# ODD2/DFD-CLIP

Hardware: AMD Instinct MI355X
Metric: 1-sec clips/sec (30x224x224 frames) ViT-B/16 (higher is better)
Workload: dtype bf16

## Files before the change

dfd-clip_amd/blocked.py:

```python
import torch

GROUP_ROWS = 16
TILE_CHANNELS = 64


def padded_rows(m):
    return (int(m) + GROUP_ROWS - 1) // GROUP_ROWS * GROUP_ROWS


def piece_offset(row, channel, ld):
    g, er = divmod(int(row), GROUP_ROWS)
    kt, c = divmod(int(channel), TILE_CHANNELS)
    chunk, e = divmod(c, 8)
    s, eq = chunk & 1, chunk >> 1
    return g * GROUP_ROWS * ld + kt * 1024 + s * 512 + er * 32 + eq * 8 + e


def pack(x, fill=0):
    m, c = x.shape
    assert c % TILE_CHANNELS == 0, "the blocked layout needs whole 64-channel K tiles"
    mp = padded_rows(m)
    xp = torch.full((mp, c), fill, dtype=x.dtype, device=x.device)
    xp[:m] = x
    v = xp.view(mp // GROUP_ROWS, GROUP_ROWS, c // TILE_CHANNELS, 4, 2, 8)
    return v.permute(0, 2, 4, 1, 3, 5).reshape(mp, c).contiguous()


def unpack(b, m=None):
    mp, c = b.shape
    assert mp % GROUP_ROWS == 0 and c % TILE_CHANNELS == 0 and b.is_contiguous()
    v = b.view(mp // GROUP_ROWS, c // TILE_CHANNELS, 2, GROUP_ROWS, 4, 8)
    x = v.permute(0, 3, 1, 4, 2, 5).reshape(mp, c)
    return x[:mp if m is None else m].contiguous()


def fc_channel_perm(n, device=None):
    assert n % TILE_CHANNELS == 0
    c = torch.arange(n, device=device)
    return (c & ~60) | ((c & 12) << 2) | ((c & 48) >> 2)


def lane_channels(eq):
    perm = fc_channel_perm(TILE_CHANNELS)
    return [[int(perm[16 * j + 4 * eq + e]) for e in range(4)] for j in range(4)]
```

dfd-clip_amd/capi.py:

```python
import ctypes
import os
from ctypes import POINTER, Structure, c_char_p, c_double, c_float, c_int, c_int32, c_int64, c_size_t, c_uint, c_uint8, c_uint32, c_uint64, c_void_p

import torch

PKG_DIR = os.path.dirname(os.path.abspath(__file__))
LIB_PATH = os.path.join(PKG_DIR, "libdfdclip_hip.so")

F32, BF16 = 0, 1
EPI_BIAS, EPI_BIAS_QUICKGELU, EPI_BIAS_RESIDUAL, EPI_PATCH_EMBED, EPI_QKV_EXPORT, EPI_RESIDUAL_POS, EPI_BIAS_GELU = range(7)
ABI_VERSION = 17

_DTYPE = {torch.float32: F32, torch.bfloat16: BF16}
FP8 = 2
FP8_MAX = 448.0
FP8_MIN_ROWS = 1024


class DfdError(RuntimeError):
    pass


GEMM_STREAM_OUT = 1
GEMM_SPARE_IF_FREE = 2
GEMM_C_BLOCKED = 4
GEMM_A_BLOCKED = 8


class GemmExtra(Structure):
    _fields_ = [("pos", c_void_p), ("cls", c_void_p), ("k_export", c_void_p), ("v_export", c_void_p),
                ("tokens", c_int32), ("frames_per_clip", c_int32), ("residual", c_void_p), ("qkv_first", c_int32),
                ("drop_rng", c_void_p), ("drop_site", c_uint32), ("drop_p", c_float), ("flags", c_uint32)]


OPTIM_SGD, OPTIM_ADAMW = 0, 1


class OptimExtra(Structure):
    _fields_ = [("kind", c_int32), ("reserved", c_int32), ("beta1", c_double), ("beta2", c_double), ("eps", c_double),
                ("step", c_int64), ("exp_avg_sq", c_void_p)]


class DropoutDesc(Structure):
    _fields_ = [("rng_state", c_void_p), ("site", c_uint32), ("p", c_float)]


class Dropout:
    __slots__ = ("rng", "site", "p")

    def __init__(self, rng, site, p):
        assert rng.is_cuda and rng.dtype == torch.int64 and rng.numel() == 2 and 0.0 <= p < 1.0
        self.rng, self.site, self.p = rng, int(site), float(p)

    def desc(self):
        return DropoutDesc(self.rng.data_ptr(), self.site, self.p)


def _drop(d):
    return ctypes.byref(d.desc()) if d is not None and d.p > 0 else None


SIGNATURES = {
    "dfd_last_error": (c_char_p, []),
    "dfd_abi_version": (c_int, []),
    "dfd_gemm_last_path": (c_int, []),
    "dfd_gemm_set_variant": (c_int, [c_int]),
    "dfd_dropout": (c_int, [c_void_p, c_int, c_void_p, c_int, c_int64, POINTER(DropoutDesc), c_void_p]),
    "dfd_device_check": (c_int, []),
    "dfd_layernorm": (c_int, [c_void_p, c_int64, c_void_p, c_void_p, c_void_p, c_int64, c_int, c_int64, c_int, c_float, c_float, c_void_p]),
    "dfd_layernorm2": (c_int, [c_void_p, c_int64, c_void_p, c_void_p, c_void_p, c_void_p, c_void_p, c_int64, c_int, c_int64, c_int, c_float,
                               c_float, c_void_p]),
    "dfd_add_layernorm": (c_int, [c_void_p, c_int64, c_void_p, c_void_p, c_int64, c_int, c_int, c_void_p, c_void_p, c_void_p, c_int64,
                                  c_int, c_int64, c_int, c_float, c_float, c_void_p]),
    "dfd_patchify": (c_int, [c_void_p, c_void_p, c_int, c_int, c_int, c_int, c_int, c_void_p]),
    "dfd_preprocess_u8": (c_int, [c_void_p, c_int, c_int, c_int, c_int, c_int, c_int, POINTER(c_float), POINTER(c_float),
                                  c_void_p, c_int, c_int, c_int, c_void_p]),
    "dfd_preprocess_geometry": (c_int, [c_int, c_int, c_int, POINTER(c_int), POINTER(c_int), POINTER(c_int), POINTER(c_int)]),
    "dfd_gemm": (c_int, [c_void_p, c_int64, c_void_p, c_int64, c_int, c_void_p, c_int64, c_int, c_void_p, c_int,
                         POINTER(GemmExtra), c_int64, c_int, c_int, c_void_p]),
# ... 123 lines not shown

SWIGLU_SIGNATURES = {
    "dfd_swiglu_fwd": (c_int, [c_void_p, c_int64, c_void_p, c_int64, c_int, c_int64, c_int, c_void_p]),
    "dfd_swiglu_last_path": (c_int, []),
}

KVGATHER_VEC16, KVGATHER_ELEMENT = 1, 2

KVGATHER_SIGNATURES = {
    "dfd_kv_gather_patches": (c_int, [c_void_p, c_void_p, c_int, c_int64, c_int64, c_int64, c_void_p, c_void_p, c_void_p, c_void_p, c_int,
                                      c_int64, c_int, c_int, c_int, c_int, c_void_p]),
    "dfd_kv_gather_last_path": (c_int, []),
}

KVFRAMES_VEC16, KVFRAMES_ELEMENT = 1, 2
KVFRAMES_SRC_ONCE = 1

KVFRAMES_SIGNATURES = {
    "dfd_kv_move_frames": (c_int, [c_void_p, c_void_p, c_void_p, c_void_p, c_int, c_int64, c_int64, c_int64, c_int64, c_int64, c_int64,
                                   c_void_p, c_void_p, c_int, c_int64, c_int, c_int, c_int, c_int, c_int, c_void_p]),
    "dfd_kv_move_last_path": (c_int, []),
}

EMA_SIGNATURES = {
    "dfd_ema_step": (c_int, [c_void_p, c_int, c_int64, c_float, c_float, c_void_p]),
}

class AttentionPlan(Structure):
    _fields_ = [("path", c_int32), ("grid", c_uint32), ("block", c_uint32), ("chunk", c_int32), ("lds", c_uint64)]


class GemmPlan(Structure):
    _fields_ = [("kernel", c_int32), ("epilogue", c_int32), ("tile_rows", c_int32), ("tiles_m", c_int32), ("ntiles", c_int64),
                ("grid", c_uint32), ("grid_y", c_uint32), ("block", c_uint32), ("c_blocked", c_int32), ("a_blocked", c_int32),
                ("dynamic", c_int32)]


class AdapterPlan(Structure):
    _fields_ = [("path", c_int32), ("grid", c_uint32), ("block", c_uint32), ("slabs", c_int32), ("groups_per_slab", c_int32)]


HOOK_SIGNATURES = {
    "dfd_adapter_norm_gelu_last_path": (c_int, []),
    "dfd_adapter_norm_gelu_plan": (c_int, [c_int, c_int, c_int, c_int, c_int, c_int, c_int, c_int, POINTER(AdapterPlan)]),
    "dfd_gemm_last_kernel": (c_int, []),
    "dfd_gemm_plan": (c_int, [c_int, c_int, c_int, c_int64, c_int, c_int, c_int64, c_int64, c_int64, c_uint32, c_int, c_int, c_int, c_uint,
                              c_uint, c_int, POINTER(GemmPlan)]),
    "dfd_attention_set_variant": (c_int, [c_int]),
    "dfd_attention_last_path": (c_int, []),
    "dfd_attention_plan": (c_int, [c_int, c_int, c_int, c_int, c_int64, c_int64, c_int, POINTER(AttentionPlan)]),
    "dfd_gemm_pair_set_variant": (c_int, [c_int]),
    "dfd_gemm_pair_plan": (c_int, [c_int64, c_int, c_int]),
    "dfd_gemm_pair_launches": (c_int64, []),
    "dfd_gemm_at_b_last_path": (c_int, []),
    "dfd_stream_policy_set": (c_uint, [c_uint]),
    "dfd_stream_policy_get": (c_uint, []),
}

(ATTN_ROWS, ATTN_ROWS_CHUNKED, ATTN_ITEM7, ATTN_ITEM9, ATTN_PERSIST7_SHORT, ATTN_PERSIST7, ATTN_XROW,
 ATTN_STREAM) = range(1, 9)

ADP_ROW256, ADP_JOINT_REG, ADP_JOINT, ADP_ROW = range(1, 5)

GEMM_GENERAL, GEMM_TILE, GEMM_PERSISTENT, GEMM_PINGPONG = range(1, 5)
(GEMM_PTR_A, GEMM_PTR_W, GEMM_PTR_C, GEMM_PTR_BIAS, GEMM_PTR_POS, GEMM_PTR_CLS, GEMM_PTR_RESIDUAL, GEMM_PTR_COL_SCALE,
 GEMM_PTR_EXPORT) = (1 << i for i in range(9))

STREAM_DECODER_KV, STREAM_DECODER_WEIGHTS, STREAM_OPTIMIZER, STREAM_ENCODER_ROWS, STREAM_ALL = 1, 2, 4, 8, 15
STREAM_DEFAULT = STREAM_DECODER_KV | STREAM_ENCODER_ROWS

_lib = None


def load_library(path=None):
    global _lib
    if _lib is not None and path is None:
        return _lib
    path = path or LIB_PATH
    if not os.path.exists(path):
        raise DfdError(f"{path} not found: the HIP kernel library is not built and there is no fallback path")
    lib = ctypes.CDLL(path)
    for name, (res, args) in {**SIGNATURES, **EXT_SIGNATURES, **EXPLAIN_SIGNATURES, **AUGMENT_SIGNATURES, **ALIGN_SIGNATURES,
                               **ELASTIC_SIGNATURES, **YUV_SIGNATURES, **SWIGLU_SIGNATURES, **KVGATHER_SIGNATURES,
                               **KVFRAMES_SIGNATURES, **EMA_SIGNATURES, **HOOK_SIGNATURES}.items():
        try:
            fn = getattr(lib, name)
        except AttributeError:
            raise DfdError(f"{path} does not export {name}")
        fn.restype = res
        fn.argtypes = args
    if lib.dfd_abi_version() != ABI_VERSION:
        raise DfdError(f"{path}: ABI version {lib.dfd_abi_version()} != {ABI_VERSION}")
    _lib = lib
    return lib


def _check(rc, what):
    if rc != 0:
        raise DfdError(f"{what} failed ({rc}): {load_library().dfd_last_error().decode()}")


def _stream():
    return c_void_p(torch._C._cuda_getCurrentRawStream(torch._C._cuda_getDevice()))


def _ptr(t):
# ... 251 lines not shown

def kv_move_frames(k, v, k_out, v_out, src_frame=None, dst_frame=None, src_once=False, src_host=None, dst_host=None):
    _dev(k, v, k_out, v_out, src_frame, dst_frame)
    assert k.dtype == v.dtype == k_out.dtype == v_out.dtype and k.dtype in _DTYPE, (k.dtype, v.dtype, k_out.dtype, v_out.dtype)
    assert k.dim() == 4 and k.shape == v.shape and k.stride() == v.stride(), "k and v are two views of one layout"
    assert k_out.dim() == 4 and k_out.shape == v_out.shape and k_out.stride() == v_out.stride(), "k_out and v_out are two views of one layout"
    L, src_frames, P, D = k.shape
    assert (k_out.shape[0], k_out.shape[2], k_out.shape[3]) == (L, P, D), (k.shape, k_out.shape)
    dst_frames = k_out.shape[1]
    assert (k.stride(3) == 1 and k_out.stride(3) == 1) or D <= 1, "rows are dense: unit column stride"
    n_src, _ = _frame_table("src_frame", src_frame, src_host, src_frames)
    n_dst, host = _frame_table("dst_frame", dst_frame, dst_host, dst_frames)
    if n_src is not None and n_dst is not None:
        assert n_src == n_dst, (n_src, n_dst)
    n = n_src if n_src is not None else n_dst
    if n is None:
        assert src_frames == dst_frames, "without a table both sides hold the same frames"
        n = src_frames
    if (src_frame is None and n > src_frames) or (dst_frame is None and n > dst_frames):
        raise DfdError(f"kv_move_frames: {n} frames under an identity table exceed that side (src {src_frames}, dst {dst_frames})")
    if host is not None and len(set(host.tolist())) != host.numel():
        raise DfdError("kv_move_frames: dst_frame names a frame twice: two moves into one frame would race")
    if L == 0 or n == 0 or P == 0 or D == 0:
        return k_out, v_out
    _check(load_library().dfd_kv_move_frames(_ptr(k), _ptr(v), _ptr(k_out), _ptr(v_out), _DTYPE[k.dtype], k.stride(0), k.stride(1),
                                             max(k.stride(2), D), k_out.stride(0), k_out.stride(1), max(k_out.stride(2), D),
                                             _ptr(src_frame), _ptr(dst_frame), L, n, src_frames, dst_frames, P, D,
                                             KVFRAMES_SRC_ONCE if src_once else 0, _stream()), "dfd_kv_move_frames")
    return k_out, v_out


def kv_move_last_path():
    return load_library().dfd_kv_move_last_path()


def profile_gemm(epilogue=None):
    _profile["epilogue"] = epilogue
    _profile["events"] = []
    _profile["base"] = None
    if epilogue is not None:
        _profile["base"] = torch.cuda.Event(enable_timing=True)
        _profile["base"].record()


def profile_gemm_collect():
    base = _profile["base"]
    spans = [(base.elapsed_time(a), base.elapsed_time(b), flops) for a, b, flops in _profile["events"]]
    profile_gemm(None)
    return spans


def gemm(a, w, c, bias=None, epilogue=EPI_BIAS, m=None, pos=None, cls=None, k_export=None, v_export=None, tokens=0,
         frames_per_clip=0, residual=None, qkv_first=0, drop=None, stream_out=False, spare_cus=0, tile_blocks=0, spare_if_free=False,
         c_blocked=False, a_blocked=False):
    _dev(a, w, c, bias, pos, cls, k_export, v_export, residual)
    assert a.dtype == w.dtype and a.stride(1) == 1 and w.stride(1) == 1 and c.stride(1) == 1
    M = a.shape[0] if m is None else m
    N, K = w.shape
    assert a.shape[1] == K
    assert residual is None or (residual.dtype == c.dtype and residual.stride(0) == c.stride(0))
    assert drop is None or epilogue == EPI_RESIDUAL_POS
    assert 0 <= epilogue <= EPI_BIAS_GELU, f"unknown epilogue {epilogue}"
    if c_blocked or a_blocked:
        blk = c if c_blocked else a
        assert blk.shape[0] >= (M + 15) // 16 * 16, "a blocked matrix needs its rows rounded up to 16"
    extra = GemmExtra(_ptr(pos).value, _ptr(cls).value, _ptr(k_export).value, _ptr(v_export).value, tokens, frames_per_clip,
                      _ptr(residual).value, qkv_first, drop.rng.data_ptr() if drop is not None and drop.p > 0 else None,
                      drop.site if drop is not None else 0, drop.p if drop is not None else 0.0, (GEMM_STREAM_OUT if stream_out else 0) | (GEMM_SPARE_IF_FREE if spare_if_free else 0) | ((int(spare_cus) & 0xff) << 8) | ((int(tile_blocks) & 0xf) << 16)
                      | (GEMM_C_BLOCKED if c_blocked else 0) | (GEMM_A_BLOCKED if a_blocked else 0))
    timed = _profile["epilogue"] == epilogue
    if timed:
        e0, e1 = torch.cuda.Event(enable_timing=True), torch.cuda.Event(enable_timing=True)
        e0.record()
    _check(load_library().dfd_gemm(_ptr(a), a.stride(0), _ptr(w), w.stride(0), _DTYPE[a.dtype], _ptr(c), c.stride(0),
                                   _DTYPE[c.dtype], _ptr(bias), epilogue, ctypes.byref(extra), M, N, K, _stream()), "dfd_gemm")
    if timed:
        e1.record()
        _profile["events"].append((e0, e1, 2.0 * M * N * K))
    return c


def gemm_fp8(a, w, c, col_scale, bias=None, epilogue=EPI_BIAS, m=None, out_inv_scale=0.0, pos=None, k_export=None, v_export=None,
             tokens=0, frames_per_clip=0, qkv_first=0, stream_out=False, spare_cus=0, spare_if_free=False):
    _dev(a, w, c, col_scale, bias, pos, k_export, v_export)
    assert a.element_size() == 1 and w.element_size() == 1 and a.stride(1) == 1 and w.stride(1) == 1 and c.stride(1) == 1
    assert col_scale.dtype == torch.float32 and col_scale.is_contiguous()
    M = a.shape[0] if m is None else m
    N, K = w.shape
    assert a.shape[1] == K and col_scale.numel() == N
    c_dtype = FP8 if c.element_size() == 1 else _DTYPE[c.dtype]
    extra = GemmExtra(_ptr(pos).value, None, _ptr(k_export).value, _ptr(v_export).value, tokens, frames_per_clip, None, qkv_first,
                      None, 0, 0.0, (GEMM_STREAM_OUT if stream_out else 0) | (GEMM_SPARE_IF_FREE if spare_if_free else 0) | ((int(spare_cus) & 0xff) << 8))
    timed = _profile["epilogue"] == epilogue
    if timed:
        e0, e1 = torch.cuda.Event(enable_timing=True), torch.cuda.Event(enable_timing=True)
        e0.record()
    _check(load_library().dfd_gemm_fp8(_ptr(a), a.stride(0), _ptr(w), w.stride(0), _ptr(c), c.stride(0), c_dtype, _ptr(col_scale),
                                       _ptr(bias), float(out_inv_scale), epilogue, ctypes.byref(extra), M, N, K, _stream()),
           "dfd_gemm_fp8")
    if timed:
        e1.record()
        _profile["events"].append((e0, e1, 2.0 * M * N * K))
    return c


def gemm_set_variant(variant):
    return load_library().dfd_gemm_set_variant(int(variant))


def gemm_pair_set_variant(variant):
    return load_library().dfd_gemm_pair_set_variant(int(variant))


def gemm_pair_plan(M, D, H):
    return bool(load_library().dfd_gemm_pair_plan(int(M), int(D), int(H)))


def gemm_pair_launches():
    return load_library().dfd_gemm_pair_launches()


def stream_policy_set(mask):
    return load_library().dfd_stream_policy_set(int(mask))


def stream_policy_get():
    return load_library().dfd_stream_policy_get()


def gemm_last_path():
    return load_library().dfd_gemm_last_path()


def gemm_last_kernel():
    return load_library().dfd_gemm_last_kernel()


def gemm_plan(ab_dtype, c_dtype, epilogue, M, N, K, lda=None, ldw=None, ldc=None, flags=0, tokens=0, frames_per_clip=0, qkv_first=0,
              has=0, misaligned=0, n_cu=256):
    out = GemmPlan()
    rc = load_library().dfd_gemm_plan(ab_dtype, c_dtype, epilogue, M, N, K, K if lda is None else lda, K if ldw is None else ldw,
                                      N if ldc is None else ldc, flags, tokens, frames_per_clip, qkv_first, has, misaligned, n_cu,
                                      ctypes.byref(out))
    if rc < 0:
        raise DfdError(f"dfd_gemm_plan failed ({rc}): {load_library().dfd_last_error().decode()}")
    return out


def gemm_at_b_workspace_bytes(R, Ma, Nb, dtype):
    return load_library().dfd_gemm_at_b_workspace(R, Ma, Nb, _DTYPE[dtype])


def gemm_at_b_last_path():
    return load_library().dfd_gemm_at_b_last_path()


def gemm_at_b(a, b, c, workspace):
    _dev(a, b, c, workspace)
    assert a.dtype == b.dtype and a.stride(1) == 1 and b.stride(1) == 1 and c.is_contiguous() and c.dtype == torch.float32
    R, Ma = a.shape
    Nb = b.shape[1]
    assert b.shape[0] == R and tuple(c.shape) == (Ma, Nb)
    assert workspace.numel() * workspace.element_size() >= gemm_at_b_workspace_bytes(R, Ma, Nb, a.dtype)
    _check(load_library().dfd_gemm_at_b(_ptr(a), a.stride(0), _ptr(b), b.stride(0), _DTYPE[a.dtype], _ptr(c), R, Ma, Nb,
                                        _ptr(workspace), _stream()), "dfd_gemm_at_b")
    return c


def adapter_norm_gelu(a, y, weight, bias, frames, patches, x, joint, eps=1e-5):
    _dev(a, y, weight, bias)
    assert (a.dtype == y.dtype or a.dtype == torch.float32) and a.is_contiguous() and y.is_contiguous()
    assert weight.is_contiguous() and bias.is_contiguous()
    _check(load_library().dfd_adapter_norm_gelu(_ptr(a), _DTYPE[a.dtype], _ptr(y), _DTYPE[y.dtype], _ptr(weight), _ptr(bias), frames,
                                                patches, x, int(joint), eps, _stream()), "dfd_adapter_norm_gelu")
    return y


def adapter_norm_gelu_bwd_workspace_bytes(frames, patches, x, joint):
    return load_library().dfd_adapter_norm_gelu_bwd_workspace(frames, patches, x, int(joint))


def adapter_norm_gelu_bwd(a, dy, da, weight, bias, dweight, dbias, workspace, frames, patches, x, joint, eps=1e-5):
    _dev(a, dy, da, weight, bias, dweight, dbias, workspace)
    assert dy.dtype == da.dtype and (a.dtype == dy.dtype or a.dtype == torch.float32)
    assert a.is_contiguous() and dy.is_contiguous() and da.is_contiguous()
    _check(load_library().dfd_adapter_norm_gelu_bwd(_ptr(a), _DTYPE[a.dtype], _ptr(dy), _ptr(da), _DTYPE[dy.dtype], _ptr(weight), _ptr(bias),
                                                    _ptr(dweight), _ptr(dbias), _ptr(workspace), frames, patches, x, int(joint),
                                                    eps, _stream()), "dfd_adapter_norm_gelu_bwd")
    return da


def attention_set_variant(variant):
    return load_library().dfd_attention_set_variant(int(variant))


def attention_last_path():
    return load_library().dfd_attention_last_path()


def attention_plan(dtype, n_frames, tokens, heads, ld_qkv=None, ld_out=None, n_cu=256):
    D = heads * 64
    plan = AttentionPlan()
    rc = load_library().dfd_attention_plan(_DTYPE[dtype], n_frames, tokens, heads, 3 * D if ld_qkv is None else ld_qkv,
                                           D if ld_out is None else ld_out, n_cu, ctypes.byref(plan))
    if rc < 0:
        raise DfdError(f"dfd_attention_plan failed ({rc}): {load_library().dfd_last_error().decode()}")
    return plan


def attention_fwd(qkv, out, n_frames, tokens, heads, head_dim=64):
    _dev(qkv, out)
    assert qkv.dtype == out.dtype and qkv.stride(1) == 1 and out.stride(1) == 1
    _check(load_library().dfd_attention_fwd(_ptr(qkv), qkv.stride(0), _ptr(out), out.stride(0), _DTYPE[qkv.dtype], n_frames,
                                            tokens, heads, head_dim, head_dim ** -0.5, _stream()), "dfd_attention_fwd")
    return out


def linear_rows(x, w, bias, y, epilogue=EPI_BIAS):
    _dev(x, w, bias, y)
    assert x.dtype == torch.float32 and w.dtype == torch.float32 and y.dtype == torch.float32
    assert x.stride(1) == 1 and y.stride(1) == 1 and w.is_contiguous()
    B, K = x.shape
    N = w.shape[0]
    _check(load_library().dfd_linear_rows(_ptr(x), x.stride(0), _ptr(w), _ptr(bias), _ptr(y), y.stride(0), epilogue, B, N, K,
                                          _stream()), "dfd_linear_rows")
    return y


def linear_rows_t_workspace_bytes(B, N, K):
    return load_library().dfd_linear_rows_t_workspace(B, N, K)


def linear_rows_t(x, wt, bias, y, workspace, epilogue=EPI_BIAS, residual=None):
    _dev(x, wt, bias, y, workspace, residual)
    assert residual is None or (residual.dtype == torch.float32 and residual.stride(1) == 1 and residual.shape == y.shape)
    assert x.dtype == torch.float32 and wt.dtype == torch.float32 and y.dtype == torch.float32
    assert x.stride(1) == 1 and y.stride(1) == 1 and wt.is_contiguous()
    B, K = x.shape
    N = wt.shape[1]
    assert wt.shape[0] == K and workspace.numel() * workspace.element_size() >= linear_rows_t_workspace_bytes(B, N, K)
    _check(load_library().dfd_linear_rows_t(_ptr(x), x.stride(0), _ptr(wt), _ptr(bias), _ptr(residual),
                                            residual.stride(0) if residual is not None else 0, _ptr(y), y.stride(0), epilogue, B, N, K,
                                            _ptr(workspace), _stream()), "dfd_linear_rows_t")
    return y


def decoder_attn_workspace_bytes(B, heads, d, splits):
    return load_library().dfd_decoder_attn_workspace(B, heads, d, splits)


class KvLayoutDesc(ctypes.Structure):
    _fields_ = [("row_stride", c_int64), ("frame_stride", c_int64), ("pos", c_void_p)]


def _kv_layout(x, other, pos, B, T, patches, D):
    if other is not None:
        assert other.dtype == x.dtype and other.shape == x.shape and other.stride() == x.stride()
    if x.is_contiguous() and pos is None:
        assert x.numel() == B * T * patches * D
        return None, None
    if x.is_contiguous():
        rs, fs = D, patches * D
    else:
        assert x.dim() == 3 and x.shape == (B * T, patches, D) and x.stride(2) == 1, "strided K/V must be [B*T, patches, D] views"
        fs, rs = x.stride(0), x.stride(1)
    if pos is not None:
# ... 308 lines not shown
```

dfd-clip_amd/csrc/attention.hip:

```cpp
#include "attention_common.hpp"

namespace {

template <typename T> struct Vec16;
template <> struct Vec16<float> { using type = f32x4; static constexpr int N = 4; };
template <> struct Vec16<bf16_t> { using type = bf16x8; static constexpr int N = 8; };

template <typename T>
__device__ __forceinline__ void attn_row_key(const float (&q)[HD], float (&acc)[HD], float& mx, float& l, const T* Kp, const T* Vp) {
  using V16 = typename Vec16<T>::type;
  constexpr int VN = Vec16<T>::N;
  constexpr int CHUNKS = HD / VN;
  float s0 = 0.f, s1 = 0.f;
#pragma unroll
  for (int ch = 0; ch < CHUNKS; ++ch) {
    const V16 kv = *reinterpret_cast<const V16*>(Kp + ch * VN);
#pragma unroll
    for (int e = 0; e < VN; e += 2) {
      s0 = fmaf(q[ch * VN + e], to_f32(kv[e]), s0);
      s1 = fmaf(q[ch * VN + e + 1], to_f32(kv[e + 1]), s1);
    }
  }
  const float s = s0 + s1;
  if (s > mx) {
// ... 77 lines not shown
  for (int qbase = 0; qbase < tokens; qbase += blockDim.x) {
    const int qi = qbase + threadIdx.x;
    const bool live = qi < tokens;
    float q[HD], acc[HD];
    const T* qp = base + (int64_t)(live ? qi : tokens - 1) * ld_qkv;
#pragma unroll
    for (int ch = 0; ch < CHUNKS; ++ch) {
      const V16 v = *reinterpret_cast<const V16*>(qp + ch * VN);
#pragma unroll
      for (int e = 0; e < VN; ++e) q[ch * VN + e] = to_f32(v[e]) * scale;
    }
#pragma unroll
    for (int c = 0; c < HD; ++c) acc[c] = 0.f;
    float mx = -INFINITY, l = 0.f;
    for (int k0 = 0; k0 < tokens; k0 += chunk) {
      const int nk = min(chunk, tokens - k0);
      __syncthreads();
      for (int c = threadIdx.x; c < nk * CHUNKS; c += blockDim.x) {
        const int row = c / CHUNKS, ch = c % CHUNKS;
        const T* src = base + (int64_t)(k0 + row) * ld_qkv + ch * VN;
        *reinterpret_cast<V16*>(Ks + row * HD + ch * VN) = *reinterpret_cast<const V16*>(src + D);
        *reinterpret_cast<V16*>(Vs + row * HD + ch * VN) = *reinterpret_cast<const V16*>(src + 2 * D);
      }
      __syncthreads();
      if (live)
        for (int j = 0; j < nk; ++j) attn_row_key<T>(q, acc, mx, l, Ks + j * HD, Vs + j * HD);
    }
    if (live) {
      const float inv = 1.0f / l;
      T* op = out + ((int64_t)frame * tokens + qi) * ld_out + head * HD;
#pragma unroll
      for (int ch = 0; ch < CHUNKS; ++ch) {
        V16 o;
#pragma unroll
        for (int e = 0; e < VN; ++e) o[e] = from_f32<T>(acc[ch * VN + e] * inv);
        *reinterpret_cast<V16*>(op + ch * VN) = o;
      }
    }
  }
}

template <typename T>
int launch_rows(const AttnPlan& p, const AttnCall& c) {
  const T* qkv = static_cast<const T*>(c.qkv);
  T* out = static_cast<T*>(c.out);
  if (p.path == ATTN_ROWS_CHUNKED)
    return attn_launch<&attn_rows_chunked_kernel<T>>("dfd_attention_fwd", p, c.st, qkv, c.ld_qkv, out, c.ld_out, c.tokens, c.heads, c.scale, p.chunk);
  return attn_launch<&attn_rows_kernel<T>>("dfd_attention_fwd", p, c.st, qkv, c.ld_qkv, out, c.ld_out, c.tokens, c.heads, c.scale);
}

thread_local int g_attn_variant = 0;
thread_local int g_attn_last_path = 0;

int checked_plan(AttnPlan* p, int dtype, int n_frames, int tokens, int heads, int64_t ld_qkv, int64_t ld_out, int n_cu) {
  DFD_REQUIRE(n_frames >= 0 && tokens > 0 && heads > 0, "dfd_attention_fwd: bad shape");
  DFD_REQUIRE(dtype == DFD_F32 || dtype == DFD_BF16, "dfd_attention_fwd: dtype=%d", dtype);
  const int esz = dtype == DFD_F32 ? 4 : 2;
  DFD_REQUIRE(ld_qkv >= 3 * heads * HD && ld_out >= heads * HD && (ld_qkv * esz) % 16 == 0 && (ld_out * esz) % 16 == 0,
              "dfd_attention_fwd: bad leading dimensions");
  *p = attn_plan(dtype, n_frames, tokens, heads, ld_qkv, ld_out, g_attn_variant, n_cu > 0 ? n_cu : dfd_cu_count());
  DFD_REQUIRE(p->path != ATTN_NONE, "dfd_attention_fwd: %lld (frame, head) items do not fit a grid", (long long)n_frames * heads);
  return DFD_OK;
}

}

extern "C" int dfd_attention_set_variant(int variant) {
  const int old = g_attn_variant;
  g_attn_variant = variant;
  return old;
}

extern "C" int dfd_attention_last_path(void) { return g_attn_last_path; }

extern "C" int dfd_attention_plan(int dtype, int n_frames, int tokens, int heads, int64_t ld_qkv, int64_t ld_out, int n_cu,
                                  dfd_attention_plan_t* out) {
  AttnPlan p;
  if (checked_plan(&p, dtype, n_frames, tokens, heads, ld_qkv, ld_out, n_cu) != DFD_OK) return -1;
  if (out) *out = dfd_attention_plan_t{p.path, p.grid, p.block, p.chunk, (uint64_t)p.lds};
  return p.path;
}

extern "C" int dfd_attention_fwd(const void* qkv, int64_t ld_qkv, void* out, int64_t ld_out, int dtype, int n_frames,
                                 int tokens, int heads, int head_dim, float scale, void* stream) {
  DFD_REQUIRE(qkv && out, "dfd_attention_fwd: null pointer");
  DFD_REQUIRE(head_dim == HD, "dfd_attention_fwd: head_dim=%d, only 64 is supported", head_dim);
  AttnPlan p;
  if (int rc = checked_plan(&p, dtype, n_frames, tokens, heads, ld_qkv, ld_out, 0)) return rc;
  DFD_REQUIRE(dfd_aligned16(qkv) && dfd_aligned16(out), "dfd_attention_fwd: pointers must be 16-byte aligned");
  if (n_frames == 0) return DFD_OK;
  const AttnCall c{qkv, ld_qkv, out, ld_out, n_frames, tokens, heads, scale, static_cast<hipStream_t>(stream)};
  int rc;
  switch (p.path) {
    case ATTN_ROWS:
    case ATTN_ROWS_CHUNKED: rc = dtype == DFD_F32 ? launch_rows<float>(p, c) : launch_rows<bf16_t>(p, c); break;
    case ATTN_XROW: rc = dfd_attn_launch_xrow(p, c); break;
    case ATTN_STREAM: rc = dfd_attn_launch_stream(p, c); break;
    default: rc = dfd_attn_launch_mfma(p, c); break;
  }
  if (rc == DFD_OK) g_attn_last_path = p.path;
  return rc;
}
```

dfd-clip_amd/csrc/attention_common.hpp:

```cpp
#pragma once
#include "common.hpp"
#include "../../include/dfdclip_hooks.h"

namespace {

constexpr int HD = 64;

typedef float f32x2v __attribute__((ext_vector_type(2)));
typedef __attribute__((address_space(3))) void* lds_ptr_t;
typedef short short4v __attribute__((ext_vector_type(4)));
typedef int v4i_t __attribute__((ext_vector_type(4)));

__device__ __forceinline__ float vmax3(float a, float b, float c) {
  float r;
  asm("v_max3_f32 %0, %1, %2, %3" : "=v"(r) : "v"(a), "v"(b), "v"(c));
  return r;
}

__device__ __forceinline__ void attn_stage_k(__amdgpu_buffer_rsrc_t srd, unsigned char* kimg, uint32_t sbase, uint32_t ldq,
                                             uint32_t Db, int lane, int np, int tokens, int p0 = 0, int dp = 1) {
  const int sub = lane >> 3, pos = lane & 7;
  const uint32_t row0 = (uint32_t)sub * ldq;
  const uint32_t k_even = row0 + Db + ((pos ^ ((sub >> 1) & 3)) << 4), k_odd = row0 + Db + ((pos ^ (((sub >> 1) & 3) | 4)) << 4);
  for (int p = p0; p < np; p += dp) {
    if (8 * p + sub < tokens)
      __builtin_amdgcn_raw_ptr_buffer_load_lds(srd, (lds_ptr_t)(kimg + p * 1024), 16, ((p & 1) ? k_odd : k_even) + p * 8 * ldq, sbase, 0, 0);
  }
}
__device__ __forceinline__ void attn_stage_v(__amdgpu_buffer_rsrc_t srd, unsigned char* vimg, uint32_t sbase, uint32_t ldq,
                                             uint32_t Db, int lane, int np, int tokens, int p0 = 0, int dp = 1) {
  const int sub = lane >> 3, pos = lane & 7;
  const uint32_t v_any = (uint32_t)sub * ldq + 2 * Db + ((pos ^ (((sub >> 1) & 1) << 2)) << 4);
  for (int p = p0; p < np; p += dp) {
    if (8 * p + sub < tokens)
      __builtin_amdgcn_raw_ptr_buffer_load_lds(srd, (lds_ptr_t)(vimg + p * 1024), 16, v_any + p * 8 * ldq, sbase, 0, 0);
  }
}

struct AttnNoTick {
  __device__ __forceinline__ void operator()(int) const {}
};
template <int NB, bool SHORT, typename Tick = AttnNoTick>
__device__ __forceinline__ float attn_softmax(f32x16 (&S)[NB], int tokens, int h, float scale_log2e, Tick tick = Tick()) {
  constexpr int LE = SHORT ? 4 : 16;
#pragma unroll
  for (int e = 0; e < LE; ++e) {
    const int key = (NB - 1) * 32 + (e & 3) + 8 * (e >> 2) + 4 * h;
    if (key >= tokens) S[NB - 1][e] = -INFINITY;
  }
  float mx = -INFINITY;
#pragma unroll
  for (int kb = 0; kb < NB; ++kb)
#pragma unroll
    for (int e = 0; e < (kb == NB - 1 ? LE : 16); e += 2) mx = vmax3(mx, S[kb][e], S[kb][e + 1]);
  mx = fmaxf(mx, __shfl_xor(mx, 32, 64));
  float sl2 = scale_log2e;
  float nmc = -mx * scale_log2e;
  asm volatile("" : "+s"(sl2));
  f32x16 lv;
#pragma unroll
  for (int e = 0; e < 16; ++e) lv[e] = 0.f;
#pragma unroll
  for (int kb = 0; kb < NB; ++kb) {
#pragma unroll
    for (int e = 0; e < (kb == NB - 1 ? LE : 16); e += 2) {
      const f32x2v t = __builtin_elementwise_fma(f32x2v{S[kb][e], S[kb][e + 1]}, f32x2v{sl2, sl2}, f32x2v{nmc, nmc});
      S[kb][e] = __builtin_amdgcn_exp2f(t[0]);
      S[kb][e + 1] = __builtin_amdgcn_exp2f(t[1]);
    }
    if (SHORT && kb == NB - 1) {
#pragma unroll
      for (int e = 0; e < 4; ++e) lv[e] += S[kb][e];
#pragma unroll
      for (int e = 4; e < 8; ++e) S[kb][e] = 0.f;
    } else {
      lv += S[kb];
    }
    tick(kb);
  }
  float l = ((lv[0] + lv[1]) + (lv[2] + lv[3])) + ((lv[4] + lv[5]) + (lv[6] + lv[7])) +
            (((lv[8] + lv[9]) + (lv[10] + lv[11])) + ((lv[12] + lv[13]) + (lv[14] + lv[15])));
  l += __shfl_xor(l, 32, 64);
  return l;
}

__device__ __forceinline__ void attn_read_v(bf16x8 (&vf)[2], const unsigned char* Vs, int lane, int step) {
  const int h = lane >> 5, tq = (lane & 15) >> 2, tp = lane & 3, rr = (lane >> 4) & 1;
  const int kbase = (step >> 1) * 32 + 16 * (step & 1) + 4 * h + tq;
// ... 15 lines not shown
struct AttnNoRider {
  __device__ __forceinline__ void operator()(const bf16x8 (&)[2], int) const {}
};
template <int NB, bool SHORT, typename Rider = AttnNoRider>
__device__ __forceinline__ void attn_pv(const f32x16 (&S)[NB], const unsigned char* Vs, int lane, f32x16 (&O)[2], Rider rider = Rider()) {
  const f32x16 zero16 = {0.f, 0.f, 0.f, 0.f, 0.f, 0.f, 0.f, 0.f, 0.f, 0.f, 0.f, 0.f, 0.f, 0.f, 0.f, 0.f};
  auto mma_v = [&](const bf16x8 (&vf)[2], int step) {
    const int kb = step >> 1, sl = step & 1;
    bf16x8 pf;
#pragma unroll
    for (int j = 0; j < 8; ++j) pf[j] = (bf16_t)S[kb][8 * sl + j];
#pragma unroll
    for (int dt = 0; dt < 2; ++dt) O[dt] = __builtin_amdgcn_mfma_f32_32x32x16_bf16(vf[dt], pf, step == 0 ? zero16 : O[dt], 0, 0, 0);
  };
  bf16x8 vfa[2], vfb[2];
  attn_read_v(vfa, Vs, lane, 0);
  __builtin_amdgcn_sched_barrier(0);
  constexpr int NS = SHORT ? 2 * NB - 1 : 2 * NB;
#pragma unroll
  for (int step = 0; step < NS; step += 2) {
    if (step + 1 < NS) attn_read_v(vfb, Vs, lane, step + 1);
    mma_v(vfa, step);
    rider(vfa, step);
    __builtin_amdgcn_sched_barrier(0);
    if (step + 2 < NS) attn_read_v(vfa, Vs, lane, step + 2);
    if (step + 1 < NS) {
      mma_v(vfb, step + 1);
      rider(vfb, step + 1);
    }
    __builtin_amdgcn_sched_barrier(0);
  }
}

__device__ __forceinline__ void attn_store_line(v4i_t d, __amdgpu_buffer_rsrc_t srd, uint32_t off) {
  __builtin_amdgcn_raw_buffer_store_b128(d, srd, off, 0, 0);
}

template <int N> __device__ __forceinline__ void attn_wait_vm() { asm volatile("s_waitcnt vmcnt(%0)" ::"n"(N) : "memory"); }

}

enum AttnPath {
  ATTN_NONE = 0, ATTN_ROWS = DFD_ATTN_ROWS, ATTN_ROWS_CHUNKED = DFD_ATTN_ROWS_CHUNKED, ATTN_ITEM7 = DFD_ATTN_ITEM7,
  ATTN_ITEM9 = DFD_ATTN_ITEM9, ATTN_PERSIST7_SHORT = DFD_ATTN_PERSIST7_SHORT, ATTN_PERSIST7 = DFD_ATTN_PERSIST7,
  ATTN_XROW = DFD_ATTN_XROW, ATTN_STREAM = DFD_ATTN_STREAM
};

struct AttnPlan {
  int path;
  unsigned grid, block;
  size_t lds;
  int chunk;
  uint32_t qkv_bytes, out_bytes;
};

constexpr size_t ATTN_LDS_MAX = 160 * 1024;
constexpr size_t attn_item_lds(int nb) { return (size_t)nb * 32 * 128 + 64 * ((size_t)nb * 64 + 8); }
constexpr size_t attn_persist_lds(int tokens, int nb) { return (size_t)4 * tokens * 128 + (size_t)2 * nb * 4096; }
constexpr size_t ATTN_XROW_LDS = 4 * 257 * 128 + 8 * 2048 + 2560;
constexpr int ATTN_STREAM_SPAN = 128;

inline AttnPlan attn_plan(int dtype, int n_frames, int tokens, int heads, int64_t ld_qkv, int64_t ld_out, int variant, int n_cu) {
  const int64_t items = (int64_t)n_frames * heads, GRID_MAX = 0x7fffffff, EXTENT_MAX = 0xfffffff0;
  const size_t esz = dtype == DFD_F32 ? 4 : 2;
  auto per_item = [&](int path, size_t lds, int chunk) {
    return AttnPlan{items <= GRID_MAX ? path : ATTN_NONE, (unsigned)items, 256u, lds, chunk, 0u, 0u};
  };
  const int nb = (tokens + 31) / 32;
  if (dtype == DFD_BF16 && (nb == 7 || nb == 9)) {
    const int64_t last_row = (int64_t)n_frames * tokens - 1;
    const int64_t qkv_bytes = last_row * ld_qkv * 2 + (int64_t)3 * heads * 128, out_bytes = last_row * ld_out * 2 + (int64_t)heads * 128;
    const unsigned grid = (unsigned)(n_cu <= 0 ? 256 : n_cu) & ~7u;
    const size_t lds = nb == 7 ? attn_persist_lds(tokens, 7) : ATTN_XROW_LDS;
    if (items >= 512 && grid >= 8 && qkv_bytes <= EXTENT_MAX && out_bytes <= EXTENT_MAX && (nb == 7 ? lds <= ATTN_LDS_MAX : tokens == 257))
      return AttnPlan{nb == 9 ? ATTN_XROW : tokens <= 6 * 32 + 8 ? ATTN_PERSIST7_SHORT : ATTN_PERSIST7, grid, 512u, lds, 0,
                      (uint32_t)qkv_bytes, (uint32_t)out_bytes};
    return per_item(nb == 7 ? ATTN_ITEM7 : ATTN_ITEM9, attn_item_lds(nb), 0);
  }
  const int64_t spans = (tokens + ATTN_STREAM_SPAN - 1) / ATTN_STREAM_SPAN;
  if (dtype == DFD_BF16 && tokens > 32 && variant != 2 && items <= GRID_MAX / spans)
    return AttnPlan{ATTN_STREAM, (unsigned)(items * spans), 256u, 0, 0, 0u, 0u};
  const size_t whole = 2 * (size_t)tokens * 64 * esz;
  const int chunk = variant == 1 ? 16 : whole > ATTN_LDS_MAX ? (int)(64 * 1024 / (2 * 64 * esz)) : 0;
  return chunk > 0 ? per_item(ATTN_ROWS_CHUNKED, 2 * (size_t)chunk * 64 * esz, chunk) : per_item(ATTN_ROWS, whole, 0);
}

template <auto Kernel, typename... A>
int attn_launch(const char* what, const AttnPlan& p, hipStream_t st, A... args) {
  static bool raised = false;
  if (p.lds > 64 * 1024 && !raised) {
    (void)hipFuncSetAttribute(reinterpret_cast<const void*>(Kernel), hipFuncAttributeMaxDynamicSharedMemorySize, (int)ATTN_LDS_MAX);
    raised = true;
  }
  hipLaunchKernelGGL(Kernel, dim3(p.grid), dim3(p.block), p.lds, st, args...);
  DFD_CHECK_LAUNCH(what);
  return DFD_OK;
}

struct AttnCall {
  const void* qkv;
  int64_t ld_qkv;
  void* out;
  int64_t ld_out;
  int n_frames, tokens, heads;
  float scale;
  hipStream_t st;
};
int dfd_attn_launch_mfma(const AttnPlan& p, const AttnCall& c);
int dfd_attn_launch_xrow(const AttnPlan& p, const AttnCall& c);
int dfd_attn_launch_stream(const AttnPlan& p, const AttnCall& c);
```

dfd-clip_amd/csrc/attention_mfma.hip:

```cpp
#include "attention_common.hpp"

namespace {

template <int NB> struct Lds {
  static constexpr int KEYS = NB * 32;
  static constexpr int VSTRIDE = KEYS * 2 + 8;
  static constexpr int K_BYTES = KEYS * 128;
  static constexpr int BYTES = K_BYTES + HD * VSTRIDE;
};

template <int NB>
__global__ __launch_bounds__(256, 2) void attn_mfma_kernel(const bf16_t* __restrict__ qkv, int64_t ld_qkv,
                                                           bf16_t* __restrict__ out, int64_t ld_out, int tokens,
                                                           int heads, float scale_log2e) {
  using L = Lds<NB>;
  extern __shared__ __attribute__((aligned(16))) unsigned char smem[];
  unsigned char* Ks = smem;
  unsigned char* Vt = smem + L::K_BYTES;
  const int tid = threadIdx.x, lane = tid & 63, wave = tid >> 6;
  const int r = lane & 31, h = lane >> 5;
  const int frame = blockIdx.x / heads, head = blockIdx.x % heads;
  const int D = heads * HD;
  const bf16_t* base = qkv + (int64_t)frame * tokens * ld_qkv + head * HD;

// ... 105 lines not shown
        const unsigned char* vp = Vt + (dt * 32 + r) * L::VSTRIDE + (kb * 32 + 16 * sl + 4 * h) * 2;
        const bf16x4 v0 = *reinterpret_cast<const bf16x4*>(vp);
        const bf16x4 v1 = *reinterpret_cast<const bf16x4*>(vp + 16);
        vf[dt] = bf16x8{v0[0], v0[1], v0[2], v0[3], v1[0], v1[1], v1[2], v1[3]};
      }
    };
    auto mma_v = [&](const bf16x8 (&vf)[2], int step) {
      const int kb = step >> 1, sl = step & 1;
      bf16x8 pf;
#pragma unroll
      for (int j = 0; j < 8; ++j) pf[j] = (bf16_t)S[kb][8 * sl + j];
#pragma unroll
      for (int dt = 0; dt < 2; ++dt) O[dt] = __builtin_amdgcn_mfma_f32_32x32x16_bf16(vf[dt], pf, O[dt], 0, 0, 0);
    };
    bf16x8 vfa[2], vfb[2];
    read_v(vfa, 0);
    __builtin_amdgcn_sched_barrier(0);
#pragma unroll
    for (int step = 0; step < 2 * NB; step += 2) {
      read_v(vfb, step + 1);
      mma_v(vfa, step);
      __builtin_amdgcn_sched_barrier(0);
      if (step + 2 < 2 * NB) read_v(vfa, step + 2);
      mma_v(vfb, step + 1);
      __builtin_amdgcn_sched_barrier(0);
    }
    if (q < tokens) {
      const float inv = 1.0f / l;
      bf16_t* op = out + ((int64_t)frame * tokens + q) * ld_out + head * HD;
#pragma unroll
      for (int dt = 0; dt < 2; ++dt)
#pragma unroll
        for (int g = 0; g < 4; ++g) {
          bf16x4 o;
#pragma unroll
          for (int e = 0; e < 4; ++e) o[e] = (bf16_t)(O[dt][4 * g + e] * inv);
          *reinterpret_cast<bf16x4*>(op + dt * 32 + 8 * g + 4 * h) = o;
        }
    }
#pragma unroll
    for (int s = 0; s < 4; ++s) qf[s] = qn[s];
  }
}

template <int NB>
__device__ __forceinline__ void attn_stage_q(__amdgpu_buffer_rsrc_t srd, unsigned char* qimg, uint32_t sbase, uint32_t ldq, int lane,
                                             int tokens) {
  const int sub = lane >> 3, pos = lane & 7;
  const uint32_t q_even = (pos ^ ((sub >> 1) & 3)) << 4, q_odd = (pos ^ (((sub >> 1) & 3) | 4)) << 4;
#pragma unroll
  for (int p = 0; p < 4 * NB; ++p) {
    const uint32_t row = (uint32_t)min(8 * p + sub, tokens - 1);
    __builtin_amdgcn_raw_ptr_buffer_load_lds(srd, (lds_ptr_t)(qimg + p * 1024), 16, row * ldq + ((p & 1) ? q_odd : q_even), sbase, 0, 0);
  }
}

__device__ __forceinline__ void wait_vm_dyn(int n) {
  switch (n < 0 ? 0 : n) {
    case 0: asm volatile("s_waitcnt vmcnt(0)" ::: "memory"); break;
    case 1: asm volatile("s_waitcnt vmcnt(1)" ::: "memory"); break;
    case 2: asm volatile("s_waitcnt vmcnt(2)" ::: "memory"); break;
    case 3: asm volatile("s_waitcnt vmcnt(3)" ::: "memory"); break;
    case 4: asm volatile("s_waitcnt vmcnt(4)" ::: "memory"); break;
    case 5: asm volatile("s_waitcnt vmcnt(5)" ::: "memory"); break;
    case 6: asm volatile("s_waitcnt vmcnt(6)" ::: "memory"); break;
    case 7: asm volatile("s_waitcnt vmcnt(7)" ::: "memory"); break;
    case 8: asm volatile("s_waitcnt vmcnt(8)" ::: "memory"); break;
    case 9: asm volatile("s_waitcnt vmcnt(9)" ::: "memory"); break;
    case 10: asm volatile("s_waitcnt vmcnt(10)" ::: "memory"); break;
    case 11: asm volatile("s_waitcnt vmcnt(11)" ::: "memory"); break;
    case 12: asm volatile("s_waitcnt vmcnt(12)" ::: "memory"); break;
    case 13: asm volatile("s_waitcnt vmcnt(13)" ::: "memory"); break;
    case 14: asm volatile("s_waitcnt vmcnt(14)" ::: "memory"); break;
    case 15: asm volatile("s_waitcnt vmcnt(15)" ::: "memory"); break;
    case 16: asm volatile("s_waitcnt vmcnt(16)" ::: "memory"); break;
    case 17: asm volatile("s_waitcnt vmcnt(17)" ::: "memory"); break;
    case 18: asm volatile("s_waitcnt vmcnt(18)" ::: "memory"); break;
    case 19: asm volatile("s_waitcnt vmcnt(19)" ::: "memory"); break;
    case 20: asm volatile("s_waitcnt vmcnt(20)" ::: "memory"); break;
    case 21: asm volatile("s_waitcnt vmcnt(21)" ::: "memory"); break;
    case 22: asm volatile("s_waitcnt vmcnt(22)" ::: "memory"); break;
    case 23: asm volatile("s_waitcnt vmcnt(23)" ::: "memory"); break;
    case 24: asm volatile("s_waitcnt vmcnt(24)" ::: "memory"); break;
    case 25: asm volatile("s_waitcnt vmcnt(25)" ::: "memory"); break;
    case 26: asm volatile("s_waitcnt vmcnt(26)" ::: "memory"); break;
    case 27: asm volatile("s_waitcnt vmcnt(27)" ::: "memory"); break;
    case 28: asm volatile("s_waitcnt vmcnt(28)" ::: "memory"); break;
    case 29: asm volatile("s_waitcnt vmcnt(29)" ::: "memory"); break;
    case 30: asm volatile("s_waitcnt vmcnt(30)" ::: "memory"); break;
    case 31: asm volatile("s_waitcnt vmcnt(31)" ::: "memory"); break;
    case 32: asm volatile("s_waitcnt vmcnt(32)" ::: "memory"); break;
    case 33: asm volatile("s_waitcnt vmcnt(33)" ::: "memory"); break;
    case 34: asm volatile("s_waitcnt vmcnt(34)" ::: "memory"); break;
    case 35: asm volatile("s_waitcnt vmcnt(35)" ::: "memory"); break;
    case 36: asm volatile("s_waitcnt vmcnt(36)" ::: "memory"); break;
    case 37: asm volatile("s_waitcnt vmcnt(37)" ::: "memory"); break;
    case 38: asm volatile("s_waitcnt vmcnt(38)" ::: "memory"); break;
    case 39: asm volatile("s_waitcnt vmcnt(39)" ::: "memory"); break;
    case 40: asm volatile("s_waitcnt vmcnt(40)" ::: "memory"); break;
    case 41: asm volatile("s_waitcnt vmcnt(41)" ::: "memory"); break;
    case 42: asm volatile("s_waitcnt vmcnt(42)" ::: "memory"); break;
    case 43: asm volatile("s_waitcnt vmcnt(43)" ::: "memory"); break;
    case 44: asm volatile("s_waitcnt vmcnt(44)" ::: "memory"); break;
    case 45: asm volatile("s_waitcnt vmcnt(45)" ::: "memory"); break;
    case 46: asm volatile("s_waitcnt vmcnt(46)" ::: "memory"); break;
    case 47: asm volatile("s_waitcnt vmcnt(47)" ::: "memory"); break;
    case 48: asm volatile("s_waitcnt vmcnt(48)" ::: "memory"); break;
    case 49: asm volatile("s_waitcnt vmcnt(49)" ::: "memory"); break;
    case 50: asm volatile("s_waitcnt vmcnt(50)" ::: "memory"); break;
    case 51: asm volatile("s_waitcnt vmcnt(51)" ::: "memory"); break;
    case 52: asm volatile("s_waitcnt vmcnt(52)" ::: "memory"); break;
    case 53: asm volatile("s_waitcnt vmcnt(53)" ::: "memory"); break;
    case 54: asm volatile("s_waitcnt vmcnt(54)" ::: "memory"); break;
    case 55: asm volatile("s_waitcnt vmcnt(55)" ::: "memory"); break;
    case 56: asm volatile("s_waitcnt vmcnt(56)" ::: "memory"); break;
    default: asm volatile("s_waitcnt vmcnt(56)" ::: "memory"); break;
  }
}

template <int NB, bool SHORT>
__global__ __launch_bounds__(512) void attn_mfma_persist_kernel(const bf16_t* __restrict__ qkv, uint32_t ldq ,
                                                                bf16_t* __restrict__ out, uint32_t ldo ,
                                                                int tokens, int heads, int n_frames, uint32_t qkv_bytes,
                                                                uint32_t out_bytes, float scale_log2e) {
  constexpr int QIMG = 32 * 128;
  extern __shared__ __attribute__((aligned(16))) unsigned char smem[];
  const int tid = threadIdx.x, wave = tid >> 6;
  int lane = tid & 63;
  asm volatile("" : "+v"(lane));
  const int r = lane & 31, h = lane >> 5;
  const uint32_t Db = (uint32_t)heads * HD * 2;
  const int ksw = (r >> 1) & 7;
  const int img = tokens * 128;
  const int np = (tokens * 8 + 63) >> 6;
  const __amdgpu_buffer_rsrc_t srdQ = __builtin_amdgcn_make_buffer_rsrc(const_cast<bf16_t*>(qkv), 0, (int)qkv_bytes, 0x00020000);
  const __amdgpu_buffer_rsrc_t srdO = __builtin_amdgcn_make_buffer_rsrc(out, 0, (int)out_bytes, 0x00020000);
  unsigned char* const qs0 = smem + 4 * img + (wave < NB ? wave : 0) * QIMG;

  for (int i = tid * 16; i < 4 * img + 2 * NB * QIMG; i += 512 * 16) *reinterpret_cast<v4i_t*>(smem + i) = v4i_t{0, 0, 0, 0};
  __syncthreads();

  const int qb = wave;
  const int xcd = blockIdx.x & 7, slot = blockIdx.x >> 3, per_xcd = gridDim.x >> 3;
  auto item_of = [&](int n, int& fr_, int& hd_) -> bool {
    const int li = n * per_xcd + slot;
    const int fl = li / heads;
    hd_ = li - fl * heads;
    fr_ = fl * 8 + xcd;
    return fr_ < n_frames;
  };
  auto barrier = [&]() { asm volatile("s_waitcnt lgkmcnt(0)\n\ts_barrier" ::: "memory"); };

  if (wave == NB) {
    int f1, h1, f2, h2;
    auto sbase_of = [&](int f, int hh) { return (uint32_t)f * tokens * ldq + hh * (HD * 2); };
    int issued = 0, mark_kq = 0, mark_v = 0;
    bool have = item_of(0, f1, h1);
    if (have) {
      attn_stage_k(srdQ, smem, sbase_of(f1, h1), ldq, Db, lane, np, tokens);
      attn_stage_q<NB>(srdQ, smem + 4 * img, sbase_of(f1, h1), ldq, lane, tokens);
      issued += np + 4 * NB;
      mark_kq = issued;
      if (item_of(1, f2, h2)) {
        attn_stage_k(srdQ, smem + 2 * img, sbase_of(f2, h2), ldq, Db, lane, np, tokens);
        issued += np;
      }
      attn_stage_v(srdQ, smem + img, sbase_of(f1, h1), ldq, Db, lane, np, tokens);
      issued += np;
      mark_v = issued;
    }
    for (int n = 0; have; ++n) {
      const int cur = n & 1;
      wait_vm_dyn(issued - mark_kq);
      barrier();
      const bool have1 = item_of(n + 1, f1, h1);
      if (have1) {
        attn_stage_q<NB>(srdQ, smem + 4 * img + (cur ^ 1) * NB * QIMG, sbase_of(f1, h1), ldq, lane, tokens);
        issued += 4 * NB;
        mark_kq = issued;
      }
      wait_vm_dyn(issued - mark_v);
      barrier();
      if (have1 && item_of(n + 2, f2, h2)) {
        attn_stage_k(srdQ, smem + cur * 2 * img, sbase_of(f2, h2), ldq, Db, lane, np, tokens);
        issued += np;
      }
      if (have1) {
        attn_stage_v(srdQ, smem + (cur ^ 1) * 2 * img + img, sbase_of(f1, h1), ldq, Db, lane, np, tokens);
        issued += np;
        mark_v = issued;
      }
      have = have1;
    }
    return;
  }
  if (wave > NB) return;

  int frame, head, nframe = 0, nhead = 0;
  bool have = item_of(0, frame, head);
  for (int n = 0; have; ++n) {
    const int cur = n & 1;
    const unsigned char* Ks = smem + cur * 2 * img;
    const unsigned char* Vs = Ks + img;
    unsigned char* Qs = qs0 + cur * NB * QIMG;
    barrier();
    const bool have_next = item_of(n + 1, nframe, nhead);
    {
    bf16x8 qf[4];
#pragma unroll
    for (int s = 0; s < 4; ++s) qf[s] = *reinterpret_cast<const bf16x8*>(Qs + r * 128 + (((2 * s + h) ^ ksw) << 4));

    f32x16 S[NB];
    const f32x16 zero16 = {0.f, 0.f, 0.f, 0.f, 0.f, 0.f, 0.f, 0.f, 0.f, 0.f, 0.f, 0.f, 0.f, 0.f, 0.f, 0.f};
    bf16x8 kfa[NB], kfb[NB];
    auto read_k = [&](bf16x8 (&kf)[NB], int s) {
#pragma unroll
      for (int kb = 0; kb < NB; ++kb)
        kf[kb] = *reinterpret_cast<const bf16x8*>(Ks + (kb * 32 + r) * 128 + (((2 * s + h) ^ ksw) << 4));
    };
    auto mma_k = [&](const bf16x8 (&kf)[NB], int s) {
#pragma unroll
      for (int kb = 0; kb < NB; ++kb)
        S[kb] = __builtin_amdgcn_mfma_f32_32x32x16_bf16(kf[kb], qf[s], s == 0 ? zero16 : S[kb], 0, 0, 0);
    };
    read_k(kfa, 0);
    __builtin_amdgcn_sched_barrier(0);
    read_k(kfb, 1);
    mma_k(kfa, 0);
    __builtin_amdgcn_sched_barrier(0);
    read_k(kfa, 2);
    mma_k(kfb, 1);
    __builtin_amdgcn_sched_barrier(0);
    read_k(kfb, 3);
    mma_k(kfa, 2);
    __builtin_amdgcn_sched_barrier(0);
    mma_k(kfb, 3);
    __builtin_amdgcn_sched_barrier(0);
    barrier();

    const float l = attn_softmax<NB, SHORT>(S, tokens, h, scale_log2e);
    f32x16 O[2];
    attn_pv<NB, SHORT>(S, Vs, lane, O);
    {
      const float inv = 1.0f / l;
#pragma unroll
      for (int dt = 0; dt < 2; ++dt)
#pragma unroll
        for (int g = 0; g < 4; ++g) {
          bf16x4 o;
#pragma unroll
          for (int e = 0; e < 4; ++e) o[e] = (bf16_t)(O[dt][4 * g + e] * inv);
          *reinterpret_cast<bf16x4*>(Qs + r * 128 + (((4 * dt + g) ^ ksw) << 4) + 8 * h) = o;
        }
      const uint32_t obase = (uint32_t)frame * tokens * ldo + head * (HD * 2);
#pragma unroll
      for (int i = 0; i < 4; ++i) {
        const int rl = 8 * i + (lane >> 3), pos = lane & 7;
        const v4i_t d = *reinterpret_cast<const v4i_t*>(Qs + rl * 128 + ((pos ^ ((rl >> 1) & 7)) << 4));
        const int qq = qb * 32 + rl;
        const uint32_t off = qq < tokens ? obase + (uint32_t)qq * ldo + pos * 16 : 0xffffffffu;
        attn_store_line(d, srdO, off);
      }
    }
    }
    have = have_next;
    frame = nframe;
    head = nhead;
  }
}

template <int NB>
int launch_item(const AttnPlan& p, const AttnCall& c) {
  static_assert(Lds<NB>::BYTES == attn_item_lds(NB), "the plan's LDS size is the kernel's layout");
  static_assert(Lds<NB>::VSTRIDE % 16 == 8, "Vt row stride must be 8 mod 16 bytes");
  return attn_launch<&attn_mfma_kernel<NB>>("dfd_attention_fwd(mfma)", p, c.st, static_cast<const bf16_t*>(c.qkv), c.ld_qkv,
                                            static_cast<bf16_t*>(c.out), c.ld_out, c.tokens, c.heads, c.scale * 1.4426950408889634f);
}

template <bool SHORT>
int launch_persist(const AttnPlan& p, const AttnCall& c) {
  return attn_launch<&attn_mfma_persist_kernel<7, SHORT>>("dfd_attention_fwd(mfma, persistent)", p, c.st, static_cast<const bf16_t*>(c.qkv),
                                                          (uint32_t)(c.ld_qkv * 2), static_cast<bf16_t*>(c.out), (uint32_t)(c.ld_out * 2),
                                                          c.tokens, c.heads, c.n_frames, p.qkv_bytes, p.out_bytes,
                                                          c.scale * 1.4426950408889634f);
}

}

int dfd_attn_launch_mfma(const AttnPlan& p, const AttnCall& c) {
  switch (p.path) {
    case ATTN_PERSIST7_SHORT: return launch_persist<true>(p, c);
    case ATTN_PERSIST7: return launch_persist<false>(p, c);
    case ATTN_ITEM7: return launch_item<7>(p, c);
    default: return launch_item<9>(p, c);
  }
}
```

dfd-clip_amd/csrc/gemm.hip:

```cpp
#include "gemm_plan.hpp"
#include "gelu.hpp"

namespace {

constexpr int BM = 128, BN = 128;
constexpr int ROW_BYTES = 64;
constexpr int ROW_STRIDE = 80;
constexpr int TILE_BYTES = BM * ROW_STRIDE;
constexpr int EPI_SPLITK_SLAB = 100;

template <typename CT> __device__ __forceinline__ void store_c(void* C, int64_t off, float v) {
  static_cast<CT*>(C)[off] = from_f32<CT>(v);
}

template <typename CT, int EPI>
__device__ __forceinline__ void epilogue_elem(const GemmArgs& a, int64_t m, int n, float acc) {
  if (m >= a.M || n >= a.N) return;
  if constexpr (EPI == DFD_EPI_BIAS) {
    store_c<CT>(a.C, m * a.ldc + n, acc + (a.bias ? a.bias[n] : 0.f));
  } else if constexpr (EPI == DFD_EPI_BIAS_QUICKGELU) {
    store_c<CT>(a.C, m * a.ldc + n, quick_gelu(acc + (a.bias ? a.bias[n] : 0.f)));
  } else if constexpr (EPI == DFD_EPI_BIAS_GELU) {
    store_c<CT>(a.C, m * a.ldc + n, gelu_erf(acc + (a.bias ? a.bias[n] : 0.f)));
  } else if constexpr (EPI == DFD_EPI_BIAS_RESIDUAL) {
// ... 188 lines not shown
  float s = 0.f;
  for (int z = 0; z < splits; ++z) s += slabs[(int64_t)z * n + i];
  out[i] = s;
}

void at_b_plan(int64_t R, int Ma, int Nb, int64_t* Rp, int* splits) {
  const int tiles = ((Ma + BM - 1) / BM) * ((Nb + BN - 1) / BN);
  int sp = (1024 + tiles - 1) / tiles;
  const int64_t steps = (R + 31) / 32;
  if (sp > steps / 8) sp = (int)(steps / 8 > 0 ? steps / 8 : 1);
  if (sp > 512) sp = 512;
  *splits = sp;
  *Rp = (R + 31) / 32 * 32;
}

template <typename T>
int launch_at_b(const void* A, int64_t lda, const void* B, int64_t ldb, float* C, int64_t R, int Ma, int Nb, void* workspace,
                hipStream_t st) {
  int64_t Rp;
  int splits;
  at_b_plan(R, Ma, Nb, &Rp, &splits);
  T* At = static_cast<T*>(workspace);
  T* Bt = At + (int64_t)Ma * Rp;
  size_t off = (size_t)(Ma + Nb) * Rp * sizeof(T);
  off = (off + 255) / 256 * 256;
  float* slabs = reinterpret_cast<float*>(static_cast<unsigned char*>(workspace) + off);
  const dim3 tb(256);
  hipLaunchKernelGGL((transpose_pad_kernel<T>), dim3((Ma + 31) / 32, (unsigned)(Rp / 32)), tb, 0, st, static_cast<const T*>(A), lda, At, R, Ma, Rp);
  hipLaunchKernelGGL((transpose_pad_kernel<T>), dim3((Nb + 31) / 32, (unsigned)(Rp / 32)), tb, 0, st, static_cast<const T*>(B), ldb, Bt, R, Nb, Rp);
  GemmArgs a{};
  a.A = At; a.W = Bt; a.C = slabs; a.lda = Rp; a.ldw = Rp; a.ldc = Nb; a.M = Ma; a.N = Nb; a.K = (int)Rp;
  const dim3 grid((Nb + BN - 1) / BN, (Ma + BM - 1) / BM, splits);
  hipLaunchKernelGGL((gemm128_kernel<T, float, EPI_SPLITK_SLAB>), grid, tb, 0, st, a);
  const int64_t n = (int64_t)Ma * Nb;
  hipLaunchKernelGGL(slab_reduce_kernel, dim3((unsigned)((n + 255) / 256)), tb, 0, st, slabs, C, n, splits);
  DFD_CHECK_LAUNCH("dfd_gemm_at_b");
  return DFD_OK;
}

}

static int fill_extra(GemmArgs& a, int epilogue, const dfd_gemm_extra* extra) {
  if (!extra) return DFD_OK;
  a.pos = extra->pos; a.cls = extra->cls; a.k_export = extra->k_export; a.v_export = extra->v_export;
  a.residual = epilogue == DFD_EPI_RESIDUAL_POS ? extra->residual : nullptr;
  a.tokens = extra->tokens; a.frames_per_clip = extra->frames_per_clip;
  a.qkv_first = epilogue == DFD_EPI_QKV_EXPORT ? extra->qkv_first : 0;
  a.stream_out = (extra->flags & DFD_GEMM_STREAM_OUT) ? 1 : 0;
  a.spare_cus = (int)((extra->flags >> DFD_GEMM_SPARE_CUS_SHIFT) & 0xff);
  a.spare_if_free = (extra->flags & DFD_GEMM_SPARE_IF_FREE) ? 1 : 0;
  a.tile_rows = 32 * (int)((extra->flags >> DFD_GEMM_TILE_BLOCKS_SHIFT) & 0xf);
  a.c_blocked = (extra->flags & DFD_GEMM_C_BLOCKED) ? 1 : 0;
  a.a_blocked = (extra->flags & DFD_GEMM_A_BLOCKED) ? 1 : 0;
  a.pair = a.c_blocked | a.a_blocked;
  DFD_REQUIRE(epilogue != DFD_EPI_QKV_EXPORT || !extra->k_export == !extra->v_export, "dfd_gemm: QKV_EXPORT needs both k_export and v_export or neither");
  if (epilogue == DFD_EPI_RESIDUAL_POS && extra->drop_rng && extra->drop_p > 0.f) {
    DFD_REQUIRE(extra->drop_p < 1.f, "dfd_gemm: drop_p=%f", (double)extra->drop_p);
    const dfd_dropout_t dd{extra->drop_rng, extra->drop_site, extra->drop_p};
    a.drop = dfd_make_drop(&dd);
  }
  return DFD_OK;
}

static thread_local int g_gemm_variant = 0;
static thread_local int g_pair_variant = 0;

static int checked_plan(GemmPlan* p, const char* who, GemmArgs& a, GemmPtrs ptrs, int ab_dtype, int c_dtype, int epilogue, int n_cu) {
  const bool f8 = ab_dtype == DFD_FP8;
  DFD_REQUIRE(a.M >= 0 && a.N > 0 && a.K > 0, "%s: bad shape M=%lld N=%d K=%d", who, (long long)a.M, a.N, a.K);
  if (f8) {
    DFD_REQUIRE(c_dtype == DFD_BF16 || c_dtype == DFD_FP8, "%s: c_dtype=%d", who, c_dtype);
    DFD_REQUIRE(epilogue == DFD_EPI_BIAS || epilogue == DFD_EPI_BIAS_QUICKGELU || epilogue == DFD_EPI_BIAS_GELU || epilogue == DFD_EPI_QKV_EXPORT,
                "%s: epilogue %d not served (BIAS, BIAS_QUICKGELU, BIAS_GELU, QKV_EXPORT)", who, epilogue);
    DFD_REQUIRE(c_dtype == DFD_BF16 || (epilogue != DFD_EPI_QKV_EXPORT && a.out_inv_scale > 0.f), "%s: fp8 output needs out_inv_scale > 0 and a plain / QuickGELU / GELU epilogue", who);
    DFD_REQUIRE(a.lda >= a.K && a.ldw >= a.K && a.ldc >= a.N, "%s: leading dimensions", who);
  } else {
    DFD_REQUIRE(ab_dtype == DFD_F32 || ab_dtype == DFD_BF16, "%s: ab_dtype=%d", who, ab_dtype);
    DFD_REQUIRE(c_dtype == DFD_F32 || c_dtype == DFD_BF16, "%s: c_dtype=%d", who, c_dtype);
    DFD_REQUIRE(!(ab_dtype == DFD_F32 && c_dtype == DFD_BF16), "%s: f32 operands with bf16 output unsupported", who);
    DFD_REQUIRE(a.K % 32 == 0, "%s: K=%d must be a multiple of 32", who, a.K);
    const int esz = ab_dtype == DFD_F32 ? 4 : 2;
    DFD_REQUIRE(a.lda >= a.K && a.ldw >= a.K && (a.lda * esz) % 16 == 0 && (a.ldw * esz) % 16 == 0, "%s: lda=%lld ldw=%lld must be >= K and 16-byte multiples", who,
                (long long)a.lda, (long long)a.ldw);
    DFD_REQUIRE(!(ptrs.misaligned & (DFD_GEMM_PTR_A | DFD_GEMM_PTR_W)), "%s: A and W must be 16-byte aligned", who);
  }
  const bool has_pos = ptrs.present & DFD_GEMM_PTR_POS;
  if (epilogue == DFD_EPI_PATCH_EMBED) {
    DFD_REQUIRE(has_pos && (ptrs.present & DFD_GEMM_PTR_CLS) && a.tokens > 1, "%s: PATCH_EMBED needs extra.pos, extra.cls, extra.tokens", who);
    DFD_REQUIRE(a.M % (a.tokens - 1) == 0, "%s: PATCH_EMBED M=%lld is not a whole number of frames", who, (long long)a.M);
    DFD_REQUIRE(c_dtype == DFD_F32 && a.ldc >= a.N, "%s: PATCH_EMBED writes an f32 token matrix", who);
  } else {
    DFD_REQUIRE(a.ldc >= a.N, "%s: ldc=%lld < N", who, (long long)a.ldc);
  }
  if (epilogue == DFD_EPI_QKV_EXPORT) {
    DFD_REQUIRE(a.tokens > 1 && (a.qkv_first == 0 || a.qkv_first == 1) && a.N % (3 - a.qkv_first) == 0,
                "%s: QKV_EXPORT needs extra.tokens, qkv_first in {0, 1} and N a multiple of the column blocks present", who);
    DFD_REQUIRE(a.M % a.tokens == 0, "%s: QKV_EXPORT M=%lld is not a whole number of frames", who, (long long)a.M);
    DFD_REQUIRE(!has_pos || a.frames_per_clip > 0, "%s: QKV_EXPORT with pos needs frames_per_clip", who);
  }
  if (epilogue == DFD_EPI_RESIDUAL_POS) {
    DFD_REQUIRE(a.tokens > 1, "%s: RESIDUAL_POS needs extra.tokens (patches per frame + 1)", who);
    DFD_REQUIRE(!has_pos || a.frames_per_clip > 0, "%s: RESIDUAL_POS with pos needs frames_per_clip", who);
  }
  DFD_REQUIRE(a.tile_rows == 0 || a.tile_rows == 224 || a.tile_rows == 256, "%s: tile blocks must be 0, 7 or 8", who);
  if (a.frames_per_clip < 1) a.frames_per_clip = 1;
  if (a.M == 0) {
    *p = GemmPlan{};
    return DFD_OK;
  }
  *p = gemm_plan(a, ptrs, ab_dtype, c_dtype, epilogue, g_gemm_variant, g_pair_variant, n_cu > 0 ? n_cu : dfd_cu_count());
  if (p->refused) {
    dfd_set_error("%s: %s%s (epilogue %d, M=%lld N=%d K=%d)", who,
                  a.pair ? "DFD_GEMM_C_BLOCKED / DFD_GEMM_A_BLOCKED: the ping-pong kernel does not serve this call: " : "call not served: ", p->refused,
                  epilogue, (long long)a.M, a.N, a.K);
    return DFD_ERR_INVALID_ARG;
  }
  if (p->tiles.grid == 0) {
    dfd_set_error("%s: cannot query the device", who);
    return DFD_ERR_LAUNCH;
  }
  return DFD_OK;
}

static thread_local int g_last_kernel = 0;
static thread_local int g_last_path = 0;
extern "C" int dfd_gemm_last_kernel(void) { return g_last_kernel; }
extern "C" int dfd_gemm_last_path(void) { return g_last_path; }
extern "C" int dfd_gemm_set_variant(int variant) {
  const int old = g_gemm_variant;
  g_gemm_variant = variant;
  return old;
}

static thread_local int64_t g_pair_launches = 0;
extern "C" int dfd_gemm_pair_set_variant(int variant) {
  const int old = g_pair_variant;
  g_pair_variant = variant;
  return old;
}
extern "C" int64_t dfd_gemm_pair_launches(void) { return g_pair_launches; }
extern "C" int dfd_gemm_pair_plan(int64_t M, int D, int H) {
  if (g_pair_variant == 1 || M < 1 || D < 1 || H < 1) return 0;
  if (M < 1024 && g_pair_variant != 2) return 0;
  GemmArgs fc{}, pr{};
  fc.M = pr.M = M; fc.pair = pr.pair = 1;
  fc.N = H; fc.K = D; fc.lda = D; fc.ldw = D; fc.ldc = H; fc.c_blocked = 1;
  pr.N = D; pr.K = H; pr.lda = H; pr.ldw = H; pr.ldc = D; pr.a_blocked = 1;
  const GemmPtrs dense{DFD_GEMM_PTR_A | DFD_GEMM_PTR_W | DFD_GEMM_PTR_C | DFD_GEMM_PTR_BIAS, 0u};
  auto blocked = [&](const GemmArgs& a, int epi) {
    return gemm_plan(a, dense, DFD_BF16, DFD_BF16, epi, g_gemm_variant, g_pair_variant, 256).kernel == DFD_GEMM_PINGPONG;
  };
  return blocked(fc, DFD_EPI_BIAS_QUICKGELU) && blocked(pr, DFD_EPI_BIAS) ? 1 : 0;
}

static int plan_and_launch(const char* who, GemmArgs& a, int ab_dtype, int c_dtype, int epilogue, void* stream) {
  GemmPlan p;
  if (const int rc = checked_plan(&p, who, a, gemm_ptrs(a), ab_dtype, c_dtype, epilogue, 0)) return rc;
  if (p.kernel == 0) return DFD_OK;
  a.c_blocked = p.c_blocked;
  a.a_blocked = p.a_blocked;
  hipStream_t st = static_cast<hipStream_t>(stream);
  const bool f8 = ab_dtype == DFD_FP8, cf8 = c_dtype == DFD_FP8;
  int rc, path;
  switch (p.kernel) {
    case DFD_GEMM_PINGPONG: rc = dfd_gemm256e_launch(p, a, f8, cf8, st); path = 257; break;
    case DFD_GEMM_PERSISTENT: rc = dfd_gemm256p_launch(p, a, f8, cf8, st); path = 256; break;
    case DFD_GEMM_TILE: rc = dfd_gemm256_launch(p, a, c_dtype, st); path = 256; break;
    default:
      rc = ab_dtype == DFD_F32 ? launch_gemm128<float, float>(p, a, st)
           : c_dtype == DFD_BF16 ? launch_gemm128<bf16_t, bf16_t>(p, a, st) : launch_gemm128<bf16_t, float>(p, a, st);
      path = 128;
  }
  if (rc != DFD_OK) return rc;
  g_last_kernel = p.kernel;
  if (!f8) g_last_path = path;
  if (p.c_blocked || p.a_blocked) ++g_pair_launches;
  return DFD_OK;
}

extern "C" int dfd_gemm_plan(int ab_dtype, int c_dtype, int epilogue, int64_t M, int N, int K, int64_t lda, int64_t ldw, int64_t ldc,
                             uint32_t flags, int tokens, int frames_per_clip, int qkv_first, unsigned has, unsigned misaligned, int n_cu,
                             dfd_gemm_plan_t* out) {
  dfd_gemm_extra extra{};
  extra.tokens = tokens; extra.frames_per_clip = frames_per_clip; extra.qkv_first = qkv_first; extra.flags = flags;
  GemmArgs a{};
  a.lda = lda; a.ldw = ldw; a.ldc = ldc; a.M = M; a.N = N; a.K = K; a.out_inv_scale = 1.f;
  (void)fill_extra(a, epilogue, &extra);
  const unsigned optional = DFD_GEMM_PTR_EXPORT | DFD_GEMM_PTR_POS | DFD_GEMM_PTR_RESIDUAL;
  GemmPtrs ptrs{((2u * DFD_GEMM_PTR_EXPORT - 1u) & ~optional) | (has & optional), 0u};
  ptrs.misaligned = misaligned & ptrs.present;
  GemmPlan p;
  if (checked_plan(&p, ab_dtype == DFD_FP8 ? "dfd_gemm_fp8" : "dfd_gemm", a, ptrs, ab_dtype, c_dtype, epilogue, n_cu) != DFD_OK) return -1;
  if (out)
    *out = dfd_gemm_plan_t{p.kernel, p.epilogue, p.tiles.rows, p.tiles.tiles_m, p.tiles.ntiles, (uint32_t)p.tiles.grid, p.grid_y, p.block,
                           p.c_blocked, p.a_blocked, p.dynamic};
  return p.kernel;
}

extern "C" int dfd_gemm(const void* A, int64_t lda, const void* W, int64_t ldw, int ab_dtype, void* C, int64_t ldc,
                        int c_dtype, const float* bias, int epilogue, const dfd_gemm_extra* extra, int64_t M, int N,
                        int K, void* stream) {
  DFD_REQUIRE(A && W && C, "dfd_gemm: null pointer");
  DFD_REQUIRE(ab_dtype != DFD_FP8, "dfd_gemm: ab_dtype=%d", ab_dtype);
  GemmArgs a{};
  a.A = A; a.W = W; a.C = C; a.bias = bias;
  a.lda = lda; a.ldw = ldw; a.ldc = ldc; a.M = M; a.N = N; a.K = K;
  if (const int rc = fill_extra(a, epilogue, extra)) return rc;
  return plan_and_launch("dfd_gemm", a, ab_dtype, c_dtype, epilogue, stream);
}

extern "C" int dfd_gemm_fp8(const void* A, int64_t lda, const void* W, int64_t ldw, void* C, int64_t ldc, int c_dtype,
                            const float* col_scale, const float* bias, float out_inv_scale, int epilogue,
                            const dfd_gemm_extra* extra, int64_t M, int N, int K, void* stream) {
  DFD_REQUIRE(A && W && C && col_scale, "dfd_gemm_fp8: null pointer");
  GemmArgs a{};
  a.A = A; a.W = W; a.C = C; a.bias = bias; a.col_scale = col_scale; a.out_inv_scale = out_inv_scale;
  a.lda = lda; a.ldw = ldw; a.ldc = ldc; a.M = M; a.N = N; a.K = K;
  if (const int rc = fill_extra(a, epilogue, extra)) return rc;
  return plan_and_launch("dfd_gemm_fp8", a, DFD_FP8, c_dtype, epilogue, stream);
}

bool dfd_gemm_tn_supported(const void* A, int64_t lda, const void* B, int64_t ldb, int Ma, int Nb);
int dfd_gemm_tn_splits(int64_t R, int Ma, int Nb);
int dfd_gemm_tn_launch(const void* A, int64_t lda, const void* B, int64_t ldb, float* C, int64_t R, int Ma, int Nb,
                       float* slabs, hipStream_t st, int* tile);

static thread_local int g_at_b_last_path = 0;
extern "C" int dfd_gemm_at_b_last_path(void) { return g_at_b_last_path; }

// ... 39 lines not shown
```

dfd-clip_amd/csrc/gemm256e.hip:

```cpp
#include <mutex>
#include <unordered_map>

#include "gemm256p_common.hpp"

namespace {

constexpr int UNIT = 128 * ROWB;
constexpr int DEPTH = 6;
constexpr int NB = 2 * (DEPTH - 1);

template <int EPI, int RB, bool F8, bool CF8, bool ABLK = false>
__global__ __launch_bounds__(512) void gemm256e_kernel(const GemmArgs a, int tiles_m, int tiles_n) {
  static_assert(!F8 || RB == 8, "fp8 form: 256-row tiles only");
  static_assert(!CF8 || (F8 && EPI != DFD_EPI_QKV_EXPORT), "fp8 output: fp8 operands, plain, QuickGELU or GELU epilogue");
  constexpr int ESZ = F8 ? 1 : 2;
  constexpr int TMU = 32 * RB;
  constexpr int WROWS = 16 * RB;
  constexpr int HB = RB - 4;
  constexpr int NCV = F8 ? 2 : 1;
  constexpr int S1 = CF8 ? RB : 2 * RB;
  constexpr int S2 = 4 * RB;
  static_assert(!ABLK || (!F8 && EPI == DFD_EPI_BIAS), "blocked A: bf16 operands, plain epilogue");
  constexpr bool C_BLK = !F8 && (EPI == DFD_EPI_BIAS_QUICKGELU || EPI == DFD_EPI_BIAS_GELU);
  constexpr bool A_BLK = ABLK;
  __shared__ __attribute__((aligned(1024))) unsigned char smem[RING + 8 * STAGE];
  const int tid = threadIdx.x;
  const int lane = tid & 63;
  const int wave = __builtin_amdgcn_readfirstlane(tid >> 6);
  const int wr = wave >> 2, wc = wave & 3;
  const int ntiles = tiles_m * tiles_n;

  const int G = gridDim.x, bid = blockIdx.x;
  const int xcd = bid & 7, q8 = G >> 3, r8 = G & 7;
  const int pos = xcd_position();

  const OperandSrds<F8, CF8, A_BLK, C_BLK> srd(a);
  const __amdgpu_buffer_rsrc_t srdA = srd.A, srdW = srd.W, srdC = srd.C;
  const v4i srdB = words(a.bias ? a.bias : reinterpret_cast<const float*>(a.W), a.bias ? a.N * 4 : 0);
  [[maybe_unused]] const v4i srdS = words(F8 ? a.col_scale : reinterpret_cast<const float*>(a.W), F8 ? a.N * 4 : 0);
  const int cnt_x = q8 + (xcd < r8 ? 1 : 0), off_x = pos - (bid >> 3);
  const v4i srdT = words(reinterpret_cast<const float*>(a.sched ? a.sched : reinterpret_cast<const uint32_t*>(a.W)), a.sched ? 8 * 128 : 0);

  const uint32_t lda2 = (uint32_t)(a.lda * ESZ), ldw2 = (uint32_t)(a.ldw * ESZ);
  const uint32_t a_last = (uint32_t)(a.M - 1) * lda2;
  constexpr bool a_blk = A_BLK;
  constexpr int a_kstep = a_blk ? (int)DFD_BLK_UNIT : ROWB;
  uint32_t vA[2][2], vW[2];
  auto set_a = [&](const Tile& t, int ha) {
    int l = lane;
    asm volatile("" : "+v"(l));
    const uint32_t pr = (uint32_t)(l >> 3), pp = (uint32_t)(l & 7);
    if constexpr (a_blk) {
      const uint32_t c0 = pp ^ (pr >> 1);
      const uint32_t r0 = (uint32_t)t.m0 + (uint32_t)(WROWS * (wave >> 2) + 64 * ha + 16 * (wave & 3)) + pr;
      const uint32_t m_last = (uint32_t)(a.M - 1);
      vA[ha][0] = dfd_blk_row(min(r0, m_last), lda2) + dfd_blk_chunk(c0);
      vA[ha][1] = dfd_blk_row(min(r0 + 8u, m_last), lda2) + dfd_blk_chunk(c0 ^ 4u);
    } else {
      const uint32_t ch0 = (pp ^ (pr >> 1)) << 4;
      const uint32_t row0 = ((uint32_t)t.m0 + (uint32_t)(WROWS * (wave >> 2) + 64 * ha + 16 * (wave & 3))) * lda2 + pr * lda2;
      vA[ha][0] = min(row0, a_last) + ch0;
      vA[ha][1] = min(row0 + 8u * lda2, a_last) + (ch0 ^ 64u);
    }
  };
  auto set_w = [&](const Tile& t, int hb) {
    int l = lane;
    asm volatile("" : "+v"(l));
    const uint32_t pr = (uint32_t)(l >> 3), pp = (uint32_t)(l & 7);
    const uint32_t ch0 = (pp ^ (pr >> 1)) << 4;
    vW[hb] = ((uint32_t)t.n0 + (uint32_t)(64 * (wave >> 1) + 32 * hb + 16 * (wave & 1))) * ldw2 + pr * ldw2 + ch0;
  };
  auto issue = [&](int kind, int kr) {
    unsigned char* d = smem + ((kind & 1) ? 0 : 4 * UNIT) + (2 * (kind >> 1) + (kr & 1)) * UNIT + wave * 16 * ROWB;
    if (kind & 1) {
      __builtin_amdgcn_raw_ptr_buffer_load_lds(srdA, (lds_ptr_t)d, 16, vA[kind >> 1][0], kr * a_kstep, 0, 0);
      __builtin_amdgcn_raw_ptr_buffer_load_lds(srdA, (lds_ptr_t)(d + 8 * ROWB), 16, vA[kind >> 1][1], kr * a_kstep, 0, 0);
// ... 192 lines not shown
      seg_tail(P2{});
      quadrant(PAR ? X : Y, 1, 1);
      if constexpr (END != 0) read_w(PAR ? X : Y, PAR ^ 1, 0);
      seg_tail(P3{});
      quadrant(PAR ? Y : X, 1, 0);
    };
    using C0 = std::integral_constant<int, 0>;
    using C1 = std::integral_constant<int, 1>;
    using C2 = std::integral_constant<int, 2>;
    using C3 = std::integral_constant<int, 3>;
    using C4 = std::integral_constant<int, 4>;
    bool short_k = false;
    if constexpr (EPI == DFD_EPI_RESIDUAL_POS) short_k = nk == 4;
    if (short_k) {
      if constexpr (EPI == DFD_EPI_RESIDUAL_POS) {
        ktile(0, C0{}, C0{}, C3{});
        ktile(1, C1{}, C1{}, C2{});
        ktile(2, C0{}, C2{}, C1{});
        ktile(3, C1{}, C2{}, C0{});
      }
    } else {
      ktile(0, C0{}, C0{}, C4{});
      ktile(1, C1{}, C1{}, C4{});
      if (dyn) {
        uint32_t n;
        const uint32_t slot_addr = (uint32_t)(uintptr_t)(lds_ptr_t)(smem + RING + 1024);
        asm volatile("ds_read_b32 %0, %1\n\ts_waitcnt lgkmcnt(0)" : "=&v"(n) : "v"(slot_addr) : "memory");
        n = (uint32_t)__builtin_amdgcn_readfirstlane((int)n) - a.sched_base[xcd];
        const uint32_t r = n / (uint32_t)cnt_x;
        has_next = r < (uint32_t)(ntiles / G + 1);
        nidx = (int)((r + 1) * (uint32_t)G + (uint32_t)off_x + (n - r * (uint32_t)cnt_x));
        has_next = has_next && nidx < ntiles;
        nxt = has_next ? decode_tile(nidx, tiles_m, tiles_n, TMU) : cur;
      }
      for (int kt = 2; kt < nk - 4; kt += 2) {
        ktile(kt, C0{}, C2{}, C4{});
        ktile(kt + 1, C1{}, C2{}, C4{});
      }
      ktile(nk - 4, C0{}, C2{}, C3{});
      ktile(nk - 3, C1{}, C2{}, C2{});
      ktile(nk - 2, C0{}, C2{}, C1{});
      ktile(nk - 1, C1{}, C2{}, C0{});
    }

    f32x4 b4[4];
    [[maybe_unused]] f32x4 cs4[4];
    const int le = opaque_lane();
#pragma unroll
    for (int j = 0; j < 4; ++j) {
      b4[j] = *reinterpret_cast<const f32x4*>(ep + (j * 16 + (le >> 4) * 4) * 4);
      if constexpr (F8) cs4[j] = *reinterpret_cast<const f32x4*>(ep + 256 + (j * 16 + (le >> 4) * 4) * 4);
    }
    asm volatile("s_waitcnt lgkmcnt(0)" ::: "memory");
    const int stores = tile_epilogue<EPI, RB, F8, CF8, C_BLK>(a, acc, b4, cs4, ep, cur, wr, wc, le, D, srdC);
    if (!has_next) break;
    s_prev = countable_stores<RB>(stores, cur, wr, a.M);
    idx = nidx;
    cur = nxt;
  }
  wait_vm<0>();
  if (wr == 0) __builtin_amdgcn_s_barrier();
}

struct SchedSlot {
  uint32_t* dev = nullptr;
  uint32_t base[8] = {0, 0, 0, 0, 0, 0, 0, 0};
};

bool sched_prepare(GemmArgs& a, hipStream_t st, int grid, int64_t ntiles) {
  static std::mutex mu;
  static std::unordered_map<hipStream_t, SchedSlot> slots;
  static uint32_t* pool = nullptr;
  static int used = 0;
  constexpr int MAX_SLOTS = 64;
  a.sched = nullptr;
  hipStreamCaptureStatus cap = hipStreamCaptureStatusNone;
  if (hipStreamIsCapturing(st, &cap) != hipSuccess || cap != hipStreamCaptureStatusNone) {
    (void)hipGetLastError();
    return true;
  }
  std::lock_guard<std::mutex> lock(mu);
  auto it = slots.find(st);
  if (it == slots.end()) {
    if (pool == nullptr) {
      if (hipMalloc(reinterpret_cast<void**>(&pool), MAX_SLOTS * 8 * 128) != hipSuccess || hipMemset(pool, 0, MAX_SLOTS * 8 * 128) != hipSuccess) {
        (void)hipGetLastError();
        pool = nullptr;
        return true;
      }
    }
    if (used >= MAX_SLOTS) return true;
    SchedSlot sl;
    sl.dev = pool + used * 8 * 32;
    ++used;
    it = slots.emplace(st, sl).first;
  }
  SchedSlot& sl = it->second;
  a.sched = sl.dev;
  const int q8 = grid >> 3, r8 = grid & 7;
  const int64_t full = ntiles / grid, rem = ntiles % grid;
  for (int x = 0; x < 8; ++x) {
    a.sched_base[x] = sl.base[x];
    const int cnt = q8 + (x < r8 ? 1 : 0);
    const int off = x < r8 ? x * (q8 + 1) : r8 * (q8 + 1) + (x - r8) * q8;
    int64_t last = rem - off;
    last = last < 0 ? 0 : (last > cnt ? cnt : last);
    sl.base[x] += (uint32_t)(full * cnt + last);
  }
  return true;
}

struct Gemm256e {
  static constexpr int kernel = DFD_GEMM_PINGPONG;
  template <int EPI, int RB, bool F8, bool CF8>
  static int run(const GemmPlan& p, hipStream_t st, const GemmArgs& a) {
    if constexpr (!F8 && EPI == DFD_EPI_BIAS) {
      if (a.a_blocked) return gemm_launch<&gemm256e_kernel<EPI, RB, F8, CF8, true>>("ping-pong", p, st, a, p.tiles.tiles_m, a.N / TN);
    }
    return gemm_launch<&gemm256e_kernel<EPI, RB, F8, CF8, false>>("ping-pong", p, st, a, p.tiles.tiles_m, a.N / TN);
  }
};

}

int dfd_gemm256e_launch(const GemmPlan& p, GemmArgs& a, bool f8, bool cf8, hipStream_t st) {
  if (p.dynamic) sched_prepare(a, st, p.tiles.grid, p.tiles.ntiles);
  else a.sched = nullptr;
  return launch_persistent<Gemm256e>(p, a, f8, cf8, st);
}
```

dfd-clip_amd/csrc/gemm256p_common.hpp:

```cpp
#pragma once
#include <type_traits>

#include "gemm_plan.hpp"

#include "gelu.hpp"
#include "gemm_blocked.hpp"

typedef int v4i_t __attribute__((ext_vector_type(4)));
typedef v4i_t v4i;
typedef int v8i __attribute__((ext_vector_type(8)));

namespace {

__device__ __forceinline__ void store_out(v4i_t d, __amdgpu_buffer_rsrc_t srd, uint32_t off, int stream_out) {
  if (stream_out) {
    __builtin_amdgcn_raw_buffer_store_b128(d, srd, off, 0, 2);
  } else {
    __builtin_amdgcn_raw_buffer_store_b128(d, srd, off, 0, 0);
  }
}

constexpr int TM = 256, TN = 256, TK = 64;
constexpr int ROWB = TK * 2;
constexpr int A_BYTES = TM * ROWB;
constexpr int SLOT = (TM + TN) * ROWB;
constexpr int RING = 2 * SLOT;
constexpr int STAGE = 4096;
typedef __attribute__((address_space(3))) void* lds_ptr_t;

struct Tile {
  int m0, n0;
};

__device__ __forceinline__ Tile decode_tile(int idx, int tiles_m, int tiles_n, int tile_rows) {
  const int ngroups = (tiles_n + 5) / 6;
  const int gcols = (tiles_n + ngroups - 1) / ngroups;
  int grp = idx / (tiles_m * gcols);
  grp = grp < ngroups - 1 ? grp : ngroups - 1;
  const int rem = idx - grp * tiles_m * gcols;
  const int cols_here = min(gcols, tiles_n - grp * gcols);
  const int tm = rem / cols_here, tn = grp * gcols + (rem - tm * cols_here);
  return Tile{tm * tile_rows, tn * TN};
}

template <int N> __device__ __forceinline__ void wait_vm() { asm volatile("s_waitcnt vmcnt(%0)" ::"n"(N) : "memory"); }

__device__ __forceinline__ int opaque_lane() {
  int l = threadIdx.x & 63;
  asm volatile("" : "+v"(l));
  return l;
}

__device__ __forceinline__ int xcd_position() {
  const int G = gridDim.x, bid = blockIdx.x;
  const int xcd = bid & 7, q8 = G >> 3, r8 = G & 7;
  return (xcd < r8 ? xcd * (q8 + 1) : r8 * (q8 + 1) + (xcd - r8) * q8) + (bid >> 3);
}

__device__ __forceinline__ __amdgpu_buffer_rsrc_t make_srd(const void* p, int64_t bytes) {
  return __builtin_amdgcn_make_buffer_rsrc(const_cast<void*>(p), 0, (int)(uint32_t)bytes, 0x00020000);
}
__device__ __forceinline__ v4i words(const float* p, int bytes) {
  const uint64_t u = reinterpret_cast<uint64_t>(p);
  return v4i{(int)(uint32_t)u, (int)((uint32_t)(u >> 32) & 0xffffu), bytes, 0x00020000};
}
template <bool F8, bool CF8, bool ABLK = false, bool CBLK = false>
struct OperandSrds {
  __amdgpu_buffer_rsrc_t A, W, C;
  __device__ __forceinline__ explicit OperandSrds(const GemmArgs& a)
      : A(make_srd(a.A, rows(a.M, ABLK && a.a_blocked) * a.lda * (F8 ? 1 : 2))), W(make_srd(a.W, (int64_t)a.N * a.ldw * (F8 ? 1 : 2))),
        C(make_srd(a.C, rows(a.M, CBLK && a.c_blocked) * a.ldc * (CF8 ? 1 : 2))) {}
  static __device__ __forceinline__ int64_t rows(int64_t M, bool blocked) { return blocked ? (M + 15) & ~(int64_t)15 : M; }
};
template <int RB> __device__ __forceinline__ int countable_stores(int stores, const Tile& t, int wr, int64_t M) {
  return (int64_t)t.m0 + (wr + 1) * 16 * RB <= M ? stores : 0;
}

template <int EPI, int RB, bool F8, bool CF8, bool BLK = false>
__device__ __forceinline__ int tile_epilogue(const GemmArgs& a, f32x4 (&acc)[RB][4], const f32x4 (&b4)[4], const f32x4 (&cs4)[4], unsigned char* const ep,
                                             const Tile& cur, int wr, int wc, int le, int D, __amdgpu_buffer_rsrc_t srdC) {
  constexpr int WROWS = 16 * RB;
  const int er = le & 15, eq = le >> 4;
  const int drow = le >> 3, dc = le & 7;
  const int nb = cur.n0 + wc * 64;
  const int64_t mrow0 = (int64_t)cur.m0 + wr * WROWS + drow;
  const int rows_left = (int)min((int64_t)0x7fffffff, a.M - mrow0);
  int which = 0;
  if constexpr (EPI == DFD_EPI_QKV_EXPORT) which = cur.n0 / D + a.qkv_first;
  const bool exporting = EPI == DFD_EPI_QKV_EXPORT && which > 0 && a.k_export != nullptr;
  int stores = 2 * RB;
#pragma unroll
  for (int i = 0; i < RB; ++i)
#pragma unroll
    for (int j = 0; j < 4; ++j) {
      if constexpr (F8) acc[i][j] = acc[i][j] * cs4[j] + b4[j];
      else acc[i][j] += b4[j];
    }
  if constexpr (EPI == DFD_EPI_QKV_EXPORT) {
    if (exporting) {
      stores = 4 * RB;
      const int ecol = nb - (which - a.qkv_first) * D + dc * 8;
      unsigned char* const parkf = ep + er * 256;
      const int64_t erows = (a.M / a.tokens) * (a.tokens - 1);
      const __amdgpu_buffer_rsrc_t srdE = make_srd(which == 2 ? a.v_export : a.k_export, erows * D * 2);
      const __amdgpu_buffer_rsrc_t srdP = make_srd(a.pos ? a.pos : reinterpret_cast<const float*>(a.W), a.pos ? a.frames_per_clip * D * 4 : 0);
#pragma unroll
      for (int i = 0; i < RB; ++i) {
        __builtin_amdgcn_sched_barrier(0);
        uint32_t eoff[2];
        f32x4 pe[2][2];
#pragma unroll
        for (int rr = 0; rr < 2; ++rr) {
          const int rloc = i * 16 + rr * 8;
          const uint32_t m = (uint32_t)min(mrow0 + rloc, a.M - 1);
          const uint32_t frame = a.div_tokens.div(m);
          const uint32_t tok = m - frame * (uint32_t)a.tokens;
          const uint32_t t = frame - a.div_frames.div(frame) * (uint32_t)a.frames_per_clip;
          eoff[rr] = (rloc < rows_left && tok > 0) ? ((frame * (uint32_t)(a.tokens - 1) + tok - 1) * (uint32_t)D + ecol) * 2 : 0xffffffffu;
          pe[rr][0] = pe[rr][1] = f32x4{0.f, 0.f, 0.f, 0.f};
          if (a.pos != nullptr) {
            const uint32_t poff = (t * (uint32_t)D + ecol) * 4;
            pe[rr][0] = __builtin_bit_cast(f32x4, __builtin_amdgcn_raw_buffer_load_b128(srdP, poff, 0, 0));
            pe[rr][1] = __builtin_bit_cast(f32x4, __builtin_amdgcn_raw_buffer_load_b128(srdP, poff, 16, 0));
          }
        }
#pragma unroll
        for (int j = 0; j < 4; ++j)
          *reinterpret_cast<f32x4*>(parkf + (((j * 4 + eq) ^ er) << 4)) = acc[i][j];
#pragma unroll
        for (int rr = 0; rr < 2; ++rr) {
          const int row = rr * 8 + drow;
// ... 73 lines not shown
      for (int rr = 0; rr < 2; ++rr) {
        const int row = rr * 8 + drow;
        const f32x4 x0 = *reinterpret_cast<const f32x4*>(ep + row * 256 + (((2 * dc) ^ row) << 4));
        const f32x4 x1 = *reinterpret_cast<const f32x4*>(ep + row * 256 + (((2 * dc + 1) ^ row) << 4));
        float dv[8];
#pragma unroll
        for (int e = 0; e < 4; ++e) {
          dv[e] = x0[e];
          dv[4 + e] = x1[e];
        }
        dfd_drop_eight(a.drop, (uint64_t)gq[b][rr] << 3, dv);
        const bf16x8 ob = __builtin_bit_cast(bf16x8, oq[b][rr]);
        bf16x8 o;
#pragma unroll
        for (int e = 0; e < 4; ++e) {
          o[e] = (bf16_t)((float)ob[e] + dv[e] + pq[b][rr][0][e]);
          o[4 + e] = (bf16_t)((float)ob[4 + e] + dv[4 + e] + pq[b][rr][1][e]);
        }
        store_out(__builtin_bit_cast(v4i, o), srdC, offq[b][rr], a.stream_out);
      }
    }
  } else if constexpr (CF8) {
    stores = RB;
    const int srow = le >> 2, sc = le & 3;
    unsigned char* const park8 = ep + er * 64 + eq * 4;
    const int psw = (er >> 1) & 3;
    const unsigned char* const dsrc8 = ep + srow * 64 + ((sc ^ ((srow >> 1) & 3)) << 4);
    const int64_t m8 = (int64_t)cur.m0 + wr * WROWS + srow;
    const int rows_left8 = (int)min((int64_t)0x7fffffff, a.M - m8);
    const uint32_t cbase8 = (uint32_t)(m8 * a.ldc + nb + sc * 16);
#pragma unroll
    for (int q = 0; q < 4; ++q) {
#pragma unroll
      for (int ii = 0; ii < 2; ++ii) {
        const int i = 2 * q + ii;
#pragma unroll
        for (int j = 0; j < 4; ++j) {
          f32x4 v = activate(acc[i][j]) * a.out_inv_scale;
#pragma unroll
          for (int e = 0; e < 4; ++e) v[e] = __builtin_fminf(__builtin_fmaxf(v[e], -448.0f), 448.0f);
          unsigned pk = __builtin_amdgcn_cvt_pk_fp8_f32(v[0], v[1], 0u, false);
          pk = __builtin_amdgcn_cvt_pk_fp8_f32(v[2], v[3], pk, true);
          *reinterpret_cast<unsigned*>(park8 + ii * 1024 + ((j ^ psw) << 4)) = pk;
        }
      }
#pragma unroll
      for (int rr = 0; rr < 2; ++rr) {
        const v4i d = *reinterpret_cast<const v4i*>(dsrc8 + rr * 1024);
        const int rloc = q * 32 + rr * 16;
        const uint32_t off = rloc < rows_left8 ? cbase8 + (uint32_t)rloc * (uint32_t)a.ldc : 0xffffffffu;
        store_out(d, srdC, off, a.stream_out);
      }
    }
  } else if (BLK && a.c_blocked) {
    const int row0 = wr * WROWS + er;
    const int rows_left_b = (int)min((int64_t)0x7fffffff, a.M - ((int64_t)cur.m0 + row0));
    const uint32_t ldc2 = (uint32_t)(a.ldc * 2);
    const uint32_t cbase = dfd_blk_row((uint32_t)cur.m0 + (uint32_t)row0, ldc2) + (uint32_t)(nb >> 6) * DFD_BLK_UNIT + (uint32_t)eq * 16u;
#pragma unroll
    for (int i = 0; i < RB; ++i) {
#pragma unroll
      for (int s = 0; s < 2; ++s) {
        const f32x4 v0 = activate(acc[i][2 * s]), v1 = activate(acc[i][2 * s + 1]);
        bf16x8 o;
#pragma unroll
        for (int e = 0; e < 4; ++e) {
          o[e] = (bf16_t)v0[e];
          o[4 + e] = (bf16_t)v1[e];
        }
        const uint32_t off = i * 16 < rows_left_b ? cbase + (uint32_t)i * (ldc2 * 16u) + (uint32_t)s * 1024u : 0xffffffffu;
        store_out(__builtin_bit_cast(v4i, o), srdC, off, a.stream_out);
      }
    }
  } else {
    unsigned char* const park = ep + er * 128 + ((eq ^ ((er & 7) << 1)) << 3);
    const unsigned char* const dsrc = ep + drow * 128 + ((dc ^ drow) << 4);
    const uint32_t cbase = (uint32_t)((mrow0 * a.ldc + nb + dc * 8) * 2);
#pragma unroll
    for (int q = 0; q < 4; ++q) {
#pragma unroll
      for (int ii = 0; ii < 2; ++ii) {
        const int i = 2 * q + ii;
        if (i >= RB) continue;
#pragma unroll
        for (int j = 0; j < 4; ++j) {
          const f32x4 v = activate(acc[i][j]);
          bf16x4 o;
#pragma unroll
          for (int e = 0; e < 4; ++e) o[e] = (bf16_t)v[e];
          typedef __attribute__((address_space(3))) bf16x4 lds_bf16x4;
          *reinterpret_cast<lds_bf16x4*>(((uint32_t)(uintptr_t)(lds_ptr_t)(park + ii * 2048)) ^ (uint32_t)(j << 5)) = o;
        }
      }
#pragma unroll
      for (int rr = 0; rr < 4; ++rr) {
        if (q * 32 + rr * 8 >= WROWS) continue;
        const v4i d = *reinterpret_cast<const v4i*>(dsrc + rr * 1024);
        const int rloc = q * 32 + rr * 8;
        uint32_t off = rloc < rows_left ? cbase + (uint32_t)rloc * (uint32_t)(a.ldc * 2) : 0xffffffffu;
        store_out(d, srdC, off, a.stream_out);
      }
    }
  }
  return stores;
}


// ... 39 lines not shown
```

dfd-clip_amd/csrc/gemm_args.hpp:

```cpp
#pragma once
#include "dropout.hpp"

struct GemmArgs {
  const void* A;
  const void* W;
  void* C;
  const float* bias;
  const float* pos;
  const float* cls;
  void* k_export;
  void* v_export;
  const void* residual;
  int64_t lda, ldw, ldc, M;
  int N, K, tokens, frames_per_clip;
  int qkv_first;
  int stream_out;
  int spare_cus;
  int spare_if_free;
  int tile_rows;
  DfdDrop drop;
  FastDiv div_tokens, div_frames;
  const float* col_scale;
  float out_inv_scale;
  uint32_t* sched;
  uint32_t sched_base[8];
  int no_dynamic;
  int c_blocked, a_blocked, pair;
};
```

dfd-clip_amd/csrc/gemm_plan.hpp:

```cpp
#pragma once
#include "gemm_args.hpp"

#include "../../include/dfdclip_hooks.h"

struct GemmPtrs {
  unsigned present, misaligned;
};
inline GemmPtrs gemm_ptrs(const GemmArgs& a) {
  const void* const ptr[] = {a.A, a.W, a.C, a.bias, a.pos, a.cls, a.residual, a.col_scale, a.k_export};
  GemmPtrs p{0u, 0u};
  for (unsigned i = 0; i < sizeof(ptr) / sizeof(ptr[0]); ++i) {
    if (ptr[i] != nullptr) p.present |= 1u << i;
    if ((reinterpret_cast<uintptr_t>(ptr[i]) & 15) != 0) p.misaligned |= 1u << i;
  }
  return p;
}

struct TilePlan {
  int rows, tiles_m;
  int64_t ntiles;
  int grid;
};

struct GemmPlan {
  int kernel;
  int epilogue;
  int c_blocked, a_blocked;
  int dynamic;
  TilePlan tiles;
  unsigned grid_y, block;
  const char* refused;
};

constexpr int GEMM_TILE_N = 256;
constexpr int64_t GEMM_EXTENT_MAX = 0xfffffff0;

constexpr bool gemm_serves(int kernel, int epi, bool f8) {
  const bool both = epi == DFD_EPI_BIAS || epi == DFD_EPI_BIAS_QUICKGELU || epi == DFD_EPI_QKV_EXPORT;
  return kernel == DFD_GEMM_PINGPONG ? both || epi == DFD_EPI_BIAS_GELU || (!f8 && epi == DFD_EPI_RESIDUAL_POS) : both || (f8 && epi == DFD_EPI_BIAS_GELU);
}

inline TilePlan plan_tiles(int64_t M, int N, int spare_cus, bool spare_if_free, int tile_rows, bool f8, bool force224, int n_cu) {
  const int tiles_n = N / GEMM_TILE_N;
  if (n_cu <= 0) return TilePlan{0, 0, 0, 0};
  int cus = n_cu - spare_cus;
  cus = cus < n_cu / 2 ? n_cu / 2 : cus;
  auto cost = [&](int rows, int c) { return (double)((((M + rows - 1) / rows) * tiles_n + c - 1) / c) * (rows == 224 ? 0.97 : 1.0); };
  if (spare_cus > 0 && spare_if_free) {
    auto best = [&](int c) { return f8 ? cost(256, c) : force224 ? cost(224, c) : (cost(224, c) < cost(256, c) ? cost(224, c) : cost(256, c)); };
    if (best(cus) > best(n_cu)) cus = n_cu;
  }
  const bool use224 = !f8 && (force224 || tile_rows == 224 || (tile_rows == 0 && cost(224, cus) < cost(256, cus)));
  TilePlan p;
  p.rows = use224 ? 224 : 256;
  p.tiles_m = (int)((M + p.rows - 1) / p.rows);
  p.ntiles = (int64_t)p.tiles_m * tiles_n;
  p.grid = (int)(p.ntiles < cus ? p.ntiles : cus);
  return p;
}

inline const char* gemm_persistent_refuses(int kernel, const GemmArgs& a, GemmPtrs p, bool f8, int c_dtype, int epi, int cb, int ab) {
  const bool pingpong = kernel == DFD_GEMM_PINGPONG, cf8 = c_dtype == DFD_FP8;
  const int esz = f8 ? 1 : 2, csz = cf8 ? 1 : 2, kshift = f8 ? 7 : 6;
  if (c_dtype != DFD_BF16 && !(f8 && cf8)) return "C must be bf16 (e4m3 operands: or e4m3)";
  if (f8 && (!(p.present & DFD_GEMM_PTR_COL_SCALE) || (p.misaligned & DFD_GEMM_PTR_COL_SCALE))) return "col_scale must be 16-byte aligned";
  if (a.N % GEMM_TILE_N != 0) return "N % 256 != 0";
  if ((a.K & ((1 << kshift) - 1)) != 0) return "a row of K is not a whole number of 128-byte steps";
  if (a.M < 1024 && !a.pair) return "M < 1024";
  if ((a.lda * esz) % 16 != 0 || (a.ldw * esz) % 16 != 0 || (a.ldc * csz) % 16 != 0) return "lda, ldw and ldc must be 16-byte multiples";
  if (p.misaligned & (DFD_GEMM_PTR_A | DFD_GEMM_PTR_W | DFD_GEMM_PTR_C | DFD_GEMM_PTR_BIAS)) return "A, W, C and bias must be 16-byte aligned";
  const int64_t Mr = a.pair ? (a.M + 15) & ~(int64_t)15 : a.M;
  if (Mr * a.lda * esz > GEMM_EXTENT_MAX || (int64_t)a.N * a.ldw * esz > GEMM_EXTENT_MAX || Mr * a.ldc * csz > GEMM_EXTENT_MAX)
    return "A, W or C exceeds the 32-bit byte offsets of a buffer descriptor";
  if ((int64_t)((a.M + 223) / 224) * (a.N / GEMM_TILE_N) > 0x3fffffff || a.M >= ((int64_t)1 << 31)) return "too many tiles or rows";
  if ((cb || ab) && (esz != 2 || csz != 2)) return "the fragment-blocked layout is bf16";
  if ((cb && a.ldc % 64 != 0) || (ab && a.lda % 64 != 0)) return "the leading dimension of a fragment-blocked matrix must be a multiple of 64";
  const int nk = a.K >> kshift;
  if (pingpong) {
    if ((nk < 6 && !(epi == DFD_EPI_RESIDUAL_POS && nk == 4)) || (nk & 1)) return "the ping-pong K loop needs an even number of 128-byte steps, at least 6";
    if ((a.ldw * esz) % 128 != 0) return "ldw must be a multiple of 128 bytes";
  } else if (nk < 2) {
    return "K is less than two 128-byte steps";
  }
  if (!gemm_serves(kernel, epi, f8)) return "the kernel has no form for this epilogue";
  if ((cb || ab) && !pingpong) return "only the ping-pong kernel knows the fragment-blocked layout";
  if (cb && epi != DFD_EPI_BIAS_QUICKGELU && epi != DFD_EPI_BIAS_GELU) return "DFD_GEMM_C_BLOCKED needs BIAS_QUICKGELU or BIAS_GELU";
  if (ab && epi != DFD_EPI_BIAS) return "DFD_GEMM_A_BLOCKED needs BIAS";
  if (epi == DFD_EPI_QKV_EXPORT) {
    const int D = a.N / (3 - a.qkv_first);
    if (cf8) return "an e4m3 C has no QKV_EXPORT form";
    if (D % GEMM_TILE_N != 0) return "a q / k / v column block is not a multiple of 256";
    if (p.misaligned & DFD_GEMM_PTR_POS) return "pos must be 16-byte aligned";
    if ((p.present & DFD_GEMM_PTR_EXPORT) && (a.M / a.tokens) * (a.tokens - 1) * (int64_t)D * 2 > GEMM_EXTENT_MAX) return "the K / V export exceeds 32-bit byte offsets";
  }
  if (epi == DFD_EPI_RESIDUAL_POS) {
    if (a.tokens < 2 || a.M * (int64_t)(a.N >> 3) >= ((int64_t)1 << 32)) return "RESIDUAL_POS needs tokens and M * N / 8 < 2^32";
    if ((p.misaligned & (DFD_GEMM_PTR_POS | DFD_GEMM_PTR_RESIDUAL)) || ((p.present & DFD_GEMM_PTR_POS) && a.frames_per_clip < 1))
      return "pos and residual must be 16-byte aligned";
  }
  return nullptr;
}

inline const char* gemm_tile_refuses(const GemmArgs& a, GemmPtrs p, int c_dtype, int epi) {
  if (a.N % GEMM_TILE_N != 0 || a.K % 64 != 0 || a.K < 128 || a.M < 1024) return "N % 256, K % 64, K >= 128, M >= 1024";
  if ((a.lda % 8) != 0 || (a.ldw % 8) != 0 || (a.ldc % 4) != 0) return "leading dimensions";
  if (p.misaligned & (DFD_GEMM_PTR_C | DFD_GEMM_PTR_BIAS)) return "C and bias must be 16-byte aligned";
  if ((int64_t)((a.M + 255) / 256) * (a.N / GEMM_TILE_N) > 0x7fffffff) return "too many tiles";
  if (a.M >= ((int64_t)1 << 31)) return "too many rows";
  const bool bf = c_dtype == DFD_BF16;
  switch (epi) {
    case DFD_EPI_BIAS:
    case DFD_EPI_BIAS_QUICKGELU:
      return nullptr;
    case DFD_EPI_QKV_EXPORT:
      return (a.N / (3 - a.qkv_first)) % GEMM_TILE_N != 0 || (p.misaligned & DFD_GEMM_PTR_POS) ? "column blocks of 256, aligned pos" : nullptr;
    case DFD_EPI_BIAS_RESIDUAL:
      return bf ? "f32 C only" : nullptr;
    case DFD_EPI_RESIDUAL_POS:
      return !bf || (a.ldc % 8) != 0 || (p.misaligned & (DFD_GEMM_PTR_POS | DFD_GEMM_PTR_RESIDUAL)) ? "bf16 C, ldc % 8, aligned pos and residual" : nullptr;
    case DFD_EPI_PATCH_EMBED:
      return bf || (p.misaligned & (DFD_GEMM_PTR_POS | DFD_GEMM_PTR_CLS)) ? "f32 C, aligned pos and cls" : nullptr;
    default:
      return "no form for this epilogue";
  }
}

inline const char* gemm_general_refuses(int c_dtype, int epi) {
  switch (epi) {
    case DFD_EPI_BIAS:
    case DFD_EPI_BIAS_QUICKGELU:
    case DFD_EPI_BIAS_GELU:
    case DFD_EPI_QKV_EXPORT:
    case DFD_EPI_RESIDUAL_POS:
      return nullptr;
    case DFD_EPI_BIAS_RESIDUAL:
    case DFD_EPI_PATCH_EMBED:
      return c_dtype == DFD_F32 ? nullptr : "the epilogue needs an f32 C";
    default:
      return "unknown epilogue";
  }
}

inline GemmPlan gemm_plan(const GemmArgs& a, GemmPtrs ptrs, int ab_dtype, int c_dtype, int epilogue, int gemm_variant, int pair_variant, int n_cu) {
  GemmPlan p{};
  p.epilogue = epilogue;
  const int cb = pair_variant == 1 ? 0 : a.c_blocked, ab = pair_variant == 1 ? 0 : a.a_blocked;
  const bool f8 = ab_dtype == DFD_FP8;
  if (ab_dtype != DFD_F32) {
    const int epi_p = epilogue == DFD_EPI_QKV_EXPORT && !(ptrs.present & DFD_GEMM_PTR_EXPORT) ? DFD_EPI_BIAS : epilogue;
    int kernel = DFD_GEMM_PINGPONG;
    const char* why = a.pair && f8                ? "the fragment-blocked layout is bf16"
                      : gemm_variant == 1 ? "dfd_gemm_set_variant(1) skips the ping-pong kernel"
                                          : gemm_persistent_refuses(kernel, a, ptrs, f8, c_dtype, epi_p, cb, ab);
    if (why && !a.pair) why = gemm_persistent_refuses(kernel = DFD_GEMM_PERSISTENT, a, ptrs, f8, c_dtype, epi_p, cb, ab);
    if (!why) {
      p.kernel = kernel; p.epilogue = epi_p; p.grid_y = 1; p.block = 512;
      p.c_blocked = cb; p.a_blocked = ab;
      p.tiles = plan_tiles(a.M, a.N, a.spare_cus, kernel == DFD_GEMM_PINGPONG && a.spare_if_free, a.tile_rows, f8, epi_p == DFD_EPI_RESIDUAL_POS, n_cu);
      p.dynamic = kernel == DFD_GEMM_PINGPONG && !f8 && a.K / 64 >= 6 && gemm_variant == 3;
      return p;
    }
    if (a.pair || f8) {
      p.refused = why;
      return p;
    }
    if (!gemm_tile_refuses(a, ptrs, c_dtype, epilogue)) {
      const int tiles_m = (int)((a.M + 255) / 256);
      const int64_t ntiles = (int64_t)tiles_m * (a.N / GEMM_TILE_N);
      p.kernel = DFD_GEMM_TILE; p.tiles = TilePlan{256, tiles_m, ntiles, (int)ntiles}; p.grid_y = 1; p.block = 512;
      return p;
    }
  }
  p.refused = gemm_general_refuses(c_dtype, epilogue);
  if (!p.refused) {
    const int tiles_m = (int)((a.M + 127) / 128), tiles_n = (a.N + 127) / 128;
    p.kernel = DFD_GEMM_GENERAL; p.tiles = TilePlan{128, tiles_m, (int64_t)tiles_m * tiles_n, tiles_n}; p.grid_y = (unsigned)tiles_m; p.block = 256;
  }
  return p;
}

template <auto Kernel, typename... A>
int gemm_launch(const char* kernel, const GemmPlan& p, hipStream_t st, const A&... args) {
  hipLaunchKernelGGL(Kernel, dim3((unsigned)p.tiles.grid, p.grid_y), dim3(p.block), 0, st, args...);
  const hipError_t e = hipGetLastError();
  if (e != hipSuccess) {
    dfd_set_error("dfd_gemm(%s): launch failed: %s", kernel, hipGetErrorString(e));
    return DFD_ERR_LAUNCH;
  }
  return DFD_OK;
}

int dfd_gemm256_launch(const GemmPlan& p, const GemmArgs& a, int c_dtype, hipStream_t st);
int dfd_gemm256p_launch(const GemmPlan& p, GemmArgs& a, bool f8, bool cf8, hipStream_t st);
int dfd_gemm256e_launch(const GemmPlan& p, GemmArgs& a, bool f8, bool cf8, hipStream_t st);
```

dfd-clip_amd/encoder.py:

```python
import contextlib

import torch
from torch import nn

from . import blocked, capi


FP8_PRESETS = ("all", "proj-bf16", "kv-bf16", "kv+proj-bf16", "edges-bf16", "none")
FP8_CONTRACT_POLICY = None
_ALL = {"qkv": "fp8", "fc": "fp8", "proj": "fp8"}
_NONE = {"qkv": "bf16", "fc": "bf16", "proj": "bf16"}


def expand_fp8_policy(policy, layers, tapped=None):
    tapped = sorted(set(range(layers) if tapped is None else (int(t) for t in tapped)))
    if any(t < 0 or t >= layers for t in tapped):
        raise ValueError(f"fp8 policy: tapped layers {tapped} outside 0..{layers - 1}")
    if policy is None:
        policy = "all"
    if isinstance(policy, str):
        if policy not in FP8_PRESETS:
            raise ValueError(f"fp8 policy: unknown preset {policy!r} (presets: {', '.join(FP8_PRESETS)})")
        kv = "kv-bf16" if policy in ("kv-bf16", "kv+proj-bf16") else "fp8"
        proj = "bf16" if policy in ("proj-bf16", "kv+proj-bf16") else "fp8"
# ... 65 lines not shown
class ResidualAttentionBlock(_Holder):
    def __init__(self, d_model, n_head):
        super().__init__()
        self.attn = _AttnParams(d_model)
        self.attn.n_head = n_head
        self.ln_1 = nn.LayerNorm(d_model)
        self.mlp = _Mlp(d_model)
        self.ln_2 = nn.LayerNorm(d_model)


class Transformer(_Holder):
    def __init__(self, width, layers, heads):
        super().__init__()
        self.width = width
        self.layers = layers
        self.resblocks = nn.Sequential(*[ResidualAttentionBlock(width, heads) for _ in range(layers)])


def _invalidate_after_load(module, incompatible_keys):
    module.invalidate()


class VisionTransformer(RuntimeStateMixin, nn.Module):
    _RUNTIME_STATE = {"_prepared": None, "_ws": {}, "_side_streams": [], "_calib": None}
    ln_eps = 1e-5
    act_epilogue = capi.EPI_BIAS_QUICKGELU
    ffn_hidden = 0

    def __init__(self, input_resolution, patch_size, width, layers, heads, output_dim, precision="bf16"):
        super().__init__()
        self.output_dim = output_dim
        self.conv1 = nn.Conv2d(3, width, kernel_size=patch_size, stride=patch_size, bias=False)
        scale = width ** -0.5
        self.class_embedding = nn.Parameter(scale * torch.randn(width))
        self.positional_embedding = nn.Parameter(scale * torch.randn((input_resolution // patch_size) ** 2 + 1, width))
        self.ln_pre = nn.LayerNorm(width)
        self.transformer = Transformer(width, layers, heads)
        self.ln_post = nn.LayerNorm(width)
        self.proj = nn.Parameter(scale * torch.randn(width, output_dim))
        self._init_runtime(input_resolution, patch_size, width, layers, heads, precision)

    def _init_runtime(self, input_resolution, patch_size, width, layers, heads, precision):
        assert width % heads == 0 and width // heads == 64, "kernels are built for 64-wide heads"
        assert precision in ("fp32", "bf16", "fp8")
        self.input_resolution = input_resolution
        self.width = width
        self.layers = layers
        self.heads = heads
        self.patch_size = patch_size
        self.precision = precision
        self.register_load_state_dict_post_hook(_invalidate_after_load)
        self._prepared = None
        self._ws = {}
        self.frame_chunk = 0
        self.streams = 1
        self._side_streams = []
        self.pixel_mean = (0.48145466, 0.4578275, 0.40821073)
        self.pixel_std = (0.26862954, 0.26130258, 0.27577711)
        self.antialias = True
        self.deferred_residual = precision in ("bf16", "fp8")
        self._fp8 = None
        self._fp8_amax = None
        self._fp8_margin = 1.0
        self._calib = None
        self._fp8_policy, self._fp8_tapped = "all", None
        self._fp8_plan = expand_fp8_policy("all", layers) if precision == "fp8" else None
        self.stream_out = {"qkv": True, "out": True, "fc": True, "proj": True}
        self.spare_cus = 0
        self.spare_layers = 0
        self.spare_gemms = {"qkv": False, "out": False, "fc": False, "proj": True}
        self.spare_window_layers = 0
        self.spare_if_free = True

    @property
    def tokens(self):
        return (self.input_resolution // self.patch_size) ** 2 + 1

    @property
    def act_dtype(self):
        return torch.float32 if self.precision == "fp32" else torch.bfloat16

    def _ensure_fp8(self, frames):
        if self.precision == "fp8" and self._fp8_amax is None and getattr(self, "_calib", None) is None:
            import logging
            logging.warning("fp8 encoder: no calibration yet, taking the activation scales from this batch "
                            "(call encoder.calibrate_fp8(frames) with representative frames to fix them beforehand)")
            self.calibrate_fp8(frames[:min(frames.shape[0], 64)])

    @torch.no_grad()
    def calibrate_fp8(self, x, margin=1.0):
        assert self.precision == "fp8"
        p = self._prepare()
        frames = self._as_frames(x)
        n = frames.shape[0]
        M = n * self.tokens
        rec = []
        self._calib = rec
        try:
            ws = self._workspace(n, 1, slot=99)
            self._embed(frames, ws, p)
            for bp in p["blocks"]:
                self._block(ws, bp, ws["qkv"][0], M, n)
        finally:
            self._ws.pop(self._ws_key(n, 1, 99), None)
            self._calib = None
        amax = torch.stack(rec).view(len(p["blocks"]), 3).float().cpu()
# ... 34 lines not shown
    def _fp8_layers(self):
        if self._fp8 is None:
            assert self._fp8_amax is not None, "fp8 encoder: not calibrated"
            p = self._prepare()
            scales = (self._fp8_amax * self._fp8_margin / capi.FP8_MAX).clamp_min(1e-12)
            layers = []
            for l, bp in enumerate(p["blocks"]):
                s1, s2, su = (float(v) for v in scales[l])
                layers.append(dict(h1_inv=1.0 / s1, h2_inv=1.0 / s2, u_inv=1.0 / su, cs_qkv=(bp["s_qkv"] * s1).contiguous(),
                                   cs_fc=(bp["s_fc"] * s2).contiguous(), cs_proj=(bp["s_proj"] * su).contiguous()))
            self._fp8 = layers
        return self._fp8

    def invalidate(self):
        self._prepared = None
        self._fp8 = None

    def _apply(self, fn, *a, **k):
        out = super()._apply(fn, *a, **k)
        self._prepared = None
        self._fp8 = None
        self._ws = {}
        return out

    def load_state_dict(self, *a, **k):
        out = super().load_state_dict(*a, **k)
        self._prepared = None
        self._fp8 = None
        return out

    def _param_device(self):
        return self.class_embedding.device

    def _prepare(self):
        if self._prepared is not None:
            return self._prepared
        dev = self._param_device()
        if dev.type != "cuda":
            raise capi.DfdError("the encoder runs on HIP kernels only: move the model to a GPU (.to('cuda'))")
        self._prepared = self._stage(dev)
        self._stage_blocked_fc(self._prepared)
        return self._prepared

    def _stage_blocked_fc(self, p):
        if self.act_dtype != torch.bfloat16:
            return
        for bp in p["blocks"]:
            if "w_fc" not in bp:
                continue
            H = bp["w_fc"].shape[0]
            if H % 64 == 0 and bp["w_proj"].shape[1] == H:
                idx = blocked.fc_channel_perm(H, device=bp["w_fc"].device)
                bp["w_fc_blk"], bp["b_fc_blk"] = bp["w_fc"][idx].contiguous(), bp["b_fc"][idx].contiguous()

    def _pair_blocked(self, bp, M, pl=_NONE):
        if "w_fc_blk" not in bp or not self.deferred_residual or pl["fc"] == "fp8" or pl["proj"] == "fp8":
            return False
        return capi.gemm_pair_plan(M, self.width, bp["w_fc"].shape[0])

    def _stage(self, dev):
        act = self.act_dtype
        kreal = 3 * self.patch_size ** 2
        kpad = (kreal + 63) // 64 * 64
        wp = torch.zeros(self.width, kpad, device=dev, dtype=torch.float32)
        wp[:, :kreal] = self.conv1.weight.detach().reshape(self.width, kreal)
        f32 = lambda t: t.detach().to(torch.float32).contiguous()
        p = dict(kpad=kpad, w_patch=wp.to(act).contiguous(), cls=f32(self.class_embedding),
                 pos=f32(self.positional_embedding), ln_pre=(f32(self.ln_pre.weight), f32(self.ln_pre.bias)), blocks=[])
        q8 = quantize_rows_e4m3
        for blk in self.transformer.resblocks:
            if self.precision == "fp8":
                f8 = dict(zip(("w_qkv8", "s_qkv"), q8(blk.attn.in_proj_weight)))
                f8.update(zip(("w_fc8", "s_fc"), q8(blk.mlp.c_fc.weight)))
                f8.update(zip(("w_proj8", "s_proj"), q8(blk.mlp.c_proj.weight)))
            else:
                f8 = {}
            p["blocks"].append(dict(f8, idx=len(p["blocks"]), 
                ln1=(f32(blk.ln_1.weight), f32(blk.ln_1.bias)), ln2=(f32(blk.ln_2.weight), f32(blk.ln_2.bias)),
                w_qkv=blk.attn.in_proj_weight.detach().to(act).contiguous(), b_qkv=f32(blk.attn.in_proj_bias),
                w_out=blk.attn.out_proj.weight.detach().to(act).contiguous(), b_out=f32(blk.attn.out_proj.bias),
                w_fc=blk.mlp.c_fc.weight.detach().to(act).contiguous(), b_fc=f32(blk.mlp.c_fc.bias),
                w_proj=blk.mlp.c_proj.weight.detach().to(act).contiguous(), b_proj=f32(blk.mlp.c_proj.bias)))
        return p

    def _ws_key(self, n, keep_layers, slot):
        return (n, self.precision, keep_layers, slot, self.ffn_hidden, self._fp8_needs(n * self.tokens))

    def _workspace(self, n, keep_layers, slot=0):
        key = self._ws_key(n, keep_layers, slot)
        need_h8, need_u8, need_u = key[-1]
        H = self.ffn_hidden
        need_u = need_u and H == 0
        ws = self._ws.get(key)
        if ws is None:
            dev = self._param_device()
            act, D = self.act_dtype, self.width
            M = n * self.tokens
            Mp = (M + 255) // 256 * 256
            P = self.tokens - 1
            Pp = (n * P + 255) // 256 * 256
            kpad = self._prepare()["kpad"]
            ws = dict(
                x=torch.zeros(Mp, D, device=dev, dtype=torch.float32), h=torch.zeros(Mp, D, device=dev, dtype=act),
                mix=torch.zeros(Mp, D, device=dev, dtype=act), u=torch.zeros(Mp, 4 * D, device=dev, dtype=act) if need_u else None,
                patches=torch.zeros(Pp, kpad, device=dev, dtype=act),
                delta=torch.zeros(Mp, D, device=dev, dtype=act) if self.deferred_residual else None,
                delta2=torch.zeros(Mp, D, device=dev, dtype=act) if self.deferred_residual else None, pending=0,
                qkv=[torch.zeros(Mp, 3 * D, device=dev, dtype=act) for _ in range(keep_layers)])
            if H:
                ws["x12"] = torch.zeros(Mp, 2 * H, device=dev, dtype=act)
                ws["hidden"] = torch.zeros(Mp, (H + 31) // 32 * 32, device=dev, dtype=act)
# ... 44 lines not shown
            else:
                capi.layernorm(x[:M], pre[0], pre[1], x[:M], eps=self.ln_eps)
                capi.layernorm(x[:M], gb[0], gb[1], h[:M], eps=self.ln_eps, out_inv_scale=inv)
        elif pend == 0:
            capi.layernorm(x[:M], gb[0], gb[1], h[:M], eps=self.ln_eps, out_inv_scale=inv)
        elif discard_x:
            capi.add_layernorm(x[:M], ws["delta"][:M], gb[0], gb[1], h[:M], delta2=ws["delta2"][:M] if pend == 2 else None,
                               store_x=False, eps=self.ln_eps, out_inv_scale=inv)
            ws["pending"] = 0
        elif not store:
            assert pend == 1
            capi.add_layernorm(x[:M], ws["delta"][:M], gb[0], gb[1], h[:M], store_x=False, eps=self.ln_eps, out_inv_scale=inv)
        else:
            capi.add_layernorm(x[:M], ws["delta"][:M], gb[0], gb[1], h[:M], delta2=ws["delta2"][:M] if pend == 2 else None,
                               eps=self.ln_eps, out_inv_scale=inv)
            ws["pending"] = 0

    def _ln_dual(self, ws, gb, M, inv, discard_x):
        x, h, h8 = ws["x"], ws["h"], ws["h8"]
        pend = ws.get("pending", 0)
        pre = ws.pop("ln_pre", None)
        if pre is not None:
            assert pend == 0
            if self.width <= 2048:
                capi.layernorm2_dual(x[:M], pre[0], pre[1], gb[0], gb[1], h[:M], h8[:M], inv, eps=self.ln_eps)
            else:
                capi.layernorm(x[:M], pre[0], pre[1], x[:M], eps=self.ln_eps)
                capi.layernorm_dual(x[:M], gb[0], gb[1], h[:M], h8[:M], inv, eps=self.ln_eps)
        elif pend == 0:
            capi.layernorm_dual(x[:M], gb[0], gb[1], h[:M], h8[:M], inv, eps=self.ln_eps)
        else:
            capi.add_layernorm_dual(x[:M], ws["delta"][:M], gb[0], gb[1], h[:M], h8[:M], inv, eps=self.ln_eps,
                                    delta2=ws["delta2"][:M] if pend == 2 else None, store_x=not discard_x)
            ws["pending"] = 0

    def _residual(self, ws, a, w, b, M, spare_cus=0, spare_if_free=False, a_blocked=False):
        if self.deferred_residual:
            pend = ws.get("pending", 0)
            assert pend < 2
            capi.gemm(a, w, ws["delta2" if pend else "delta"], b, capi.EPI_BIAS, m=M, stream_out=self.stream_out["proj" if pend else "out"],
                      spare_cus=spare_cus, spare_if_free=spare_if_free, a_blocked=a_blocked)
            ws["pending"] = pend + 1
        else:
            capi.gemm(a, w, ws["x"], b, capi.EPI_BIAS_RESIDUAL, m=M)

    def _flush(self, ws, M):
        pend = ws.get("pending", 0)
        if pend >= 1:
            ws["x"][:M] += ws["delta"][:M]
        if pend == 2:
            ws["x"][:M] += ws["delta2"][:M]
        ws["pending"] = 0

    def _block(self, ws, bp, qkv, M, n, kv_only=False, export=None):
        calib = getattr(self, "_calib", None)
        f8 = self._fp8_layers()[bp["idx"]] if self.precision == "fp8" and calib is None and M >= capi.FP8_MIN_ROWS else None
        pl = self._fp8_plan[bp["idx"]] if f8 is not None else _NONE
        so = self.stream_out
        sp = self.spare_cus if (self.spare_layers <= 0 or bp["idx"] < self.spare_layers) else 0
        sp_all = self.spare_cus if bp["idx"] < self.spare_window_layers else 0
        sg = self.spare_gemms
        sp_qkv, sp_out, sp_fc, sp_proj = (max(sp_all, sp if sg[k] else 0) for k in ("qkv", "out", "fc", "proj"))
        free = sp_all == 0 and self.spare_if_free
        D = self.width
        first = 1 if kv_only else 0
        rows = slice(D, None) if first else slice(None)
        kw = dict(m=M, tokens=self.tokens, qkv_first=first, stream_out=so["qkv"], spare_cus=sp_qkv, spare_if_free=free)
        if export is not None:
            kw.update(pos=export[2], k_export=export[0], v_export=export[1], frames_per_clip=export[3])
        if pl["qkv"] == "fp8":
            self._ln(ws, bp["ln1"], M, q=f8["h1_inv"], discard_x=kv_only)
            capi.gemm_fp8(ws["h8"], bp["w_qkv8"][rows], qkv[:, rows], f8["cs_qkv"][rows], bp["b_qkv"][rows], capi.EPI_QKV_EXPORT, **kw)
        elif pl["qkv"] == "kv-bf16" and not kv_only:
            self._ln(ws, bp["ln1"], M, q=f8["h1_inv"], dual=True)
            capi.gemm_fp8(ws["h8"], bp["w_qkv8"][:D], qkv[:, :D], f8["cs_qkv"][:D], bp["b_qkv"][:D], capi.EPI_BIAS, m=M,
                          stream_out=so["qkv"], spare_cus=sp_qkv, spare_if_free=free)
            capi.gemm(ws["h"], bp["w_qkv"][D:], qkv[:, D:], bp["b_qkv"][D:], capi.EPI_QKV_EXPORT, **dict(kw, qkv_first=1))
        else:
            self._ln(ws, bp["ln1"], M, discard_x=kv_only and calib is None)
            if calib is not None:
                calib.append(ws["h"][:M].abs().max())
            capi.gemm(ws["h"], bp["w_qkv"][rows], qkv[:, rows], bp["b_qkv"][rows], capi.EPI_QKV_EXPORT, **kw)
        if kv_only:
            return
        capi.attention_fwd(qkv, ws["mix"], n, self.tokens, self.heads)
        self._residual(ws, ws["mix"], bp["w_out"], bp["b_out"], M, spare_cus=sp_out, spare_if_free=free)
        if "w_12" in bp:
            H = self.ffn_hidden
            self._ln(ws, bp["ln2"], M, store=False)
            capi.gemm(ws["h"], bp["w_12"], ws["x12"], bp["b_12"], capi.EPI_BIAS, m=M, stream_out=so["fc"], spare_cus=sp_fc, spare_if_free=free)
            capi.swiglu_fwd(ws["x12"][:M], ws["hidden"][:M, :H])
            self._residual(ws, ws["hidden"], bp["w_3"], bp["b_3"], M, spare_cus=sp_proj, spare_if_free=free)
        elif pl["fc"] == "fp8" and pl["proj"] == "bf16":
            self._ln(ws, bp["ln2"], M, store=False, q=f8["h2_inv"])
            capi.gemm_fp8(ws["h8"], bp["w_fc8"], ws["u"], f8["cs_fc"], bp["b_fc"], self.act_epilogue, m=M,
                          stream_out=so["fc"], spare_cus=sp_fc, spare_if_free=free)
            self._residual(ws, ws["u"], bp["w_proj"], bp["b_proj"], M, spare_cus=sp_proj, spare_if_free=free)
        elif pl["fc"] == "fp8":
            self._ln(ws, bp["ln2"], M, store=False, q=f8["h2_inv"])
            capi.gemm_fp8(ws["h8"], bp["w_fc8"], ws["u8"], f8["cs_fc"], bp["b_fc"], self.act_epilogue, m=M,
                          out_inv_scale=f8["u_inv"], stream_out=so["fc"], spare_cus=sp_fc, spare_if_free=free)
            pend = ws.get("pending", 0)
            capi.gemm_fp8(ws["u8"], bp["w_proj8"], ws["delta2" if pend else "delta"], f8["cs_proj"], bp["b_proj"], capi.EPI_BIAS, m=M,
                          stream_out=so["proj"], spare_cus=sp_proj, spare_if_free=free)
            ws["pending"] = pend + 1
        else:
            self._ln(ws, bp["ln2"], M, store=False)
            if calib is not None:
                calib.append(ws["h"][:M].abs().max())
            blk = self._pair_blocked(bp, M, pl)
            w_fc, b_fc = (bp["w_fc_blk"], bp["b_fc_blk"]) if blk else (bp["w_fc"], bp["b_fc"])
            capi.gemm(ws["h"], w_fc, ws["u"], b_fc, self.act_epilogue, m=M, stream_out=so["fc"], spare_cus=sp_fc, spare_if_free=free,
                      c_blocked=blk)
            if calib is not None:
                calib.append((blocked.unpack(ws["u"][:blocked.padded_rows(M)], M) if blk else ws["u"][:M]).abs().max())
            self._residual(ws, ws["u"], bp["w_proj"], bp["b_proj"], M, spare_cus=sp_proj, spare_if_free=free, a_blocked=blk)

    @torch.no_grad()
    def forward(self, x, with_out=False, with_q=False):
        if not x.is_cuda:
            raise capi.DfdError("the encoder runs on HIP kernels only: pass device tensors")
        p = self._prepare()
        frames = self._as_frames(x)
        n = frames.shape[0]
        self._ensure_fp8(frames)
        D, H, tok = self.width, self.heads, self.tokens
        M = n * tok
        ws = self._workspace(n, self.layers)
        self._embed(frames, ws, p)
        result = []
        for l, bp in enumerate(p["blocks"]):
            qkv = ws["qkv"][l]
            self._block(ws, bp, qkv, M, n)
            t = qkv[:M].view(n, tok, 3, H, 64)
            d = {"k": t[:, :, 1], "v": t[:, :, 2]}
            if with_q:
                d["q"] = t[:, :, 0]
            if with_out:
# ... 5 lines not shown
    @torch.no_grad()
    def extract_kv(self, x, layer_indices, num_frames, temporal_pos=None, out=None, pos_ready=None, in_place=None):
        if not x.is_cuda:
            raise capi.DfdError("the encoder runs on HIP kernels only: pass device tensors")
        p = self._prepare()
        frames = self._as_frames(x)
        n = frames.shape[0]
        assert n % num_frames == 0
        self._ensure_fp8(frames)
        D, tok = self.width, self.tokens
        P = tok - 1
        L = len(layer_indices)
        if in_place is not None:
            assert in_place.shape == (L, n, tok, 3 * D) and in_place.dtype == self.act_dtype and in_place.is_contiguous()
            k_out = v_out = None
        elif out is None:
            k_out = torch.empty(L, n * P, D, device=frames.device, dtype=self.act_dtype)
            v_out = torch.empty_like(k_out)
        else:
            k_out, v_out = out
        last = max(layer_indices)
        slot = {l: i for i, l in enumerate(layer_indices)}
        clips = n // num_frames
        chunk = self.frame_chunk if self.frame_chunk > 0 else -(-clips // max(1, self.streams)) * num_frames
        chunk = max(num_frames, chunk // num_frames * num_frames)
        starts = list(range(0, n, chunk))
        n_str = min(self.streams, len(starts))
        if n_str > 1:
            cur = torch.cuda.current_stream()
            if len(self._side_streams) < n_str:
                self._side_streams = [torch.cuda.Stream() for _ in range(n_str)]
            for st in self._side_streams[:n_str]:
                st.wait_stream(cur)
        for ci, f0 in enumerate(starts):
            nf = min(chunk, n - f0)
            ctx = torch.cuda.stream(self._side_streams[ci % n_str]) if n_str > 1 else contextlib.nullcontext()
            with ctx:
                ws = self._workspace(nf, 1, slot=(ci % n_str) if n_str > 1 else 0)
                qkv = ws["qkv"][0]
                M = nf * tok
                self._embed(frames[f0:f0 + nf], ws, p)
                waited = pos_ready is None or temporal_pos is None or in_place is not None
                for l in range(last + 1):
                    exp = None
                    qkv_l = qkv
                    if l in slot and in_place is not None:
                        qkv_l = in_place[slot[l]].view(n * tok, 3 * D)[f0 * tok:(f0 + nf) * tok]
                    elif l in slot:
                        i = slot[l]
                        if not waited:
                            torch.cuda.current_stream().wait_event(pos_ready)
                            waited = True
                        exp = (k_out[i, f0 * P:(f0 + nf) * P], v_out[i, f0 * P:(f0 + nf) * P], temporal_pos, num_frames)
                    self._block(ws, p["blocks"][l], qkv_l, M, nf, kv_only=(l == last), export=exp)
        if n_str > 1:
            for st in self._side_streams[:n_str]:
                cur.wait_stream(st)
        if in_place is not None:
            return in_place[:, :, 1:, D:2 * D], in_place[:, :, 1:, 2 * D:]
        return k_out, v_out
```

include/dfdclip.h:

```cpp
#ifndef DFDCLIP_H
#define DFDCLIP_H

#include <stddef.h>
#include <stdint.h>

#ifdef __cplusplus
extern "C" {
#endif

#define DFD_ABI_VERSION 17

enum { DFD_F32 = 0, DFD_BF16 = 1, DFD_FP8 = 2  };

enum {
  DFD_OK = 0,
  DFD_ERR_INVALID_ARG = -1,
  DFD_ERR_LAUNCH = -2,
  DFD_ERR_NO_DEVICE = -3
};

enum {
  DFD_EPI_BIAS = 0,
  DFD_EPI_BIAS_QUICKGELU,
  DFD_EPI_BIAS_RESIDUAL,
  DFD_EPI_PATCH_EMBED,
  DFD_EPI_QKV_EXPORT,
  DFD_EPI_RESIDUAL_POS,
  DFD_EPI_BIAS_GELU
};

typedef struct dfd_dropout_t {
  const uint64_t* rng_state;
  uint32_t site;
  float p;
} dfd_dropout_t;

typedef struct dfd_gemm_extra {
  const float* pos;
  const float* cls;
  void* k_export;
  void* v_export;
  int32_t tokens;
  int32_t frames_per_clip;
  const void* residual;
  int32_t qkv_first;
  const uint64_t* drop_rng;
  uint32_t drop_site;
  float drop_p;
  uint32_t flags;
} dfd_gemm_extra;

enum {
  DFD_GEMM_STREAM_OUT = 1,
  DFD_GEMM_SPARE_IF_FREE = 2,
  DFD_GEMM_C_BLOCKED = 4,
  DFD_GEMM_A_BLOCKED = 8,
  DFD_GEMM_TILE_BLOCKS_SHIFT = 16,
  DFD_GEMM_SPARE_CUS_SHIFT = 8
};

const char* dfd_last_error(void);
int dfd_abi_version(void);
int dfd_device_check(void);

int dfd_layernorm(const float* x, int64_t ldx, const float* gamma, const float* beta, void* y, int64_t ldy,
                  int y_dtype, int64_t rows, int cols, float eps, float y_inv_scale, void* stream);

int dfd_layernorm2(float* x, int64_t ldx, const float* gamma_a, const float* beta_a, const float* gamma_b, const float* beta_b,
                   void* y, int64_t ldy, int y_dtype, int64_t rows, int cols, float eps, float y_inv_scale, void* stream);

int dfd_add_layernorm(float* x, int64_t ldx, const void* delta, const void* delta2, int64_t ldd, int delta_dtype,
                      int store_x, const float* gamma, const float* beta, void* y, int64_t ldy, int y_dtype, int64_t rows,
                      int cols, float eps, float y_inv_scale, void* stream);


int dfd_patchify(const float* frames, void* patches, int out_dtype, int n_frames, int res, int patch, int kpad,
                 void* stream);

int dfd_preprocess_u8(const uint8_t* frames, int n_frames, int in_h, int in_w, int res, int patch, int antialias,
                      const float* mean3, const float* std3, void* out, int out_dtype, int layout, int kpad,
                      void* stream);
int dfd_preprocess_geometry(int in_h, int in_w, int res, int* rs_h, int* rs_w, int* top, int* left);

int dfd_gemm(const void* A, int64_t lda, const void* W, int64_t ldw, int ab_dtype, void* C, int64_t ldc,
             int c_dtype, const float* bias, int epilogue, const dfd_gemm_extra* extra, int64_t M, int N, int K,
             void* stream);
int dfd_gemm_fp8(const void* A, int64_t lda, const void* W, int64_t ldw, void* C, int64_t ldc, int c_dtype,
                 const float* col_scale, const float* bias, float out_inv_scale, int epilogue,
                 const dfd_gemm_extra* extra, int64_t M, int N, int K, void* stream);

int dfd_gemm_last_path(void);

int dfd_gemm_set_variant(int variant);

size_t dfd_gemm_at_b_workspace(int64_t R, int Ma, int Nb, int dtype);
int dfd_gemm_at_b(const void* A, int64_t lda, const void* B, int64_t ldb, int dtype, float* C, int64_t R, int Ma, int Nb,
                  void* workspace, void* stream);

int dfd_attention_fwd(const void* qkv, int64_t ld_qkv, void* out, int64_t ld_out, int dtype, int n_frames,
                      int tokens, int heads, int head_dim, float scale, void* stream);

int dfd_linear_rows(const float* x, int64_t ldx, const float* W, const float* bias, float* y, int64_t ldy,
                    int epilogue, int B, int N, int K, void* stream);

size_t dfd_linear_rows_t_workspace(int B, int N, int K);
int dfd_linear_rows_t(const float* x, int64_t ldx, const float* Wt, const float* bias, const float* residual, int64_t ldr,
                      float* y, int64_t ldy, int epilogue, int B, int N, int K, void* workspace, void* stream);

typedef struct {
// ... 100 lines not shown
```

include/dfdclip_hooks.h:

```cpp
#ifndef DFDCLIP_HOOKS_H
#define DFDCLIP_HOOKS_H

#include <stdint.h>

#ifdef __cplusplus
extern "C" {
#endif

enum {
  DFD_ATTN_ROWS = 1,
  DFD_ATTN_ROWS_CHUNKED = 2,
  DFD_ATTN_ITEM7 = 3,
  DFD_ATTN_ITEM9 = 4,
  DFD_ATTN_PERSIST7_SHORT = 5,
  DFD_ATTN_PERSIST7 = 6,
  DFD_ATTN_XROW = 7,
  DFD_ATTN_STREAM = 8
};
typedef struct {
  int32_t path;
  uint32_t grid, block;
  int32_t chunk;
  uint64_t lds;
} dfd_attention_plan_t;

int dfd_attention_last_path(void);
int dfd_attention_plan(int dtype, int n_frames, int tokens, int heads, int64_t ld_qkv, int64_t ld_out, int n_cu,
                       dfd_attention_plan_t* out);

int dfd_attention_set_variant(int variant);

enum { DFD_GEMM_GENERAL = 1,
       DFD_GEMM_TILE = 2,
       DFD_GEMM_PERSISTENT = 3,
       DFD_GEMM_PINGPONG = 4  };
enum { DFD_GEMM_PTR_A = 1, DFD_GEMM_PTR_W = 2, DFD_GEMM_PTR_C = 4, DFD_GEMM_PTR_BIAS = 8, DFD_GEMM_PTR_POS = 16, DFD_GEMM_PTR_CLS = 32,
       DFD_GEMM_PTR_RESIDUAL = 64, DFD_GEMM_PTR_COL_SCALE = 128, DFD_GEMM_PTR_EXPORT = 256  };
typedef struct {
  int32_t kernel;
  int32_t epilogue;
  int32_t tile_rows, tiles_m;
  int64_t ntiles;
  uint32_t grid, grid_y, block;
  int32_t c_blocked, a_blocked;
  int32_t dynamic;
} dfd_gemm_plan_t;

int dfd_gemm_last_kernel(void);
int dfd_gemm_plan(int ab_dtype, int c_dtype, int epilogue, int64_t M, int N, int K, int64_t lda, int64_t ldw, int64_t ldc,
                  uint32_t flags, int tokens, int frames_per_clip, int qkv_first, unsigned has, unsigned misaligned, int n_cu,
                  dfd_gemm_plan_t* out);

int dfd_gemm_pair_set_variant(int variant);
int dfd_gemm_pair_plan(int64_t M, int D, int H);
int64_t dfd_gemm_pair_launches(void);

int dfd_gemm_at_b_last_path(void);

enum { DFD_ADP_ROW256 = 1,
       DFD_ADP_JOINT_REG = 2,
       DFD_ADP_JOINT = 3,
       DFD_ADP_ROW = 4         };
typedef struct {
  int32_t path;
  uint32_t grid, block;
  int32_t slabs, groups_per_slab;
} dfd_adapter_plan_t;

int dfd_adapter_norm_gelu_last_path(void);
int dfd_adapter_norm_gelu_plan(int frames, int patches, int x, int joint, int a_dtype, int dtype, int misaligned, int backward,
                               dfd_adapter_plan_t* out);

enum {
  DFD_STREAM_DECODER_KV = 1,
  DFD_STREAM_DECODER_WEIGHTS = 2,
  DFD_STREAM_OPTIMIZER = 4,
  DFD_STREAM_ENCODER_ROWS = 8,
  DFD_STREAM_ALL = 15
};
#define DFD_STREAM_DEFAULT 9
unsigned dfd_stream_policy_set(unsigned mask);
unsigned dfd_stream_policy_get(void);

#ifdef __cplusplus
}
#endif
#endif
```

Before: 906.5.

## Write QKV GEMM output in fragment-blocked layout read directly by persistent attention

Adds a QKV_BLOCKED mode in which the ping-pong GEMM stores q|k|v in the 16-row fragment-blocked layout, using permuted QKV weights and bias. The persistent attention kernel gains blocked staging paths that load Q/K/V tiles from that layout straight into LDS. The aim is to make attention staging loads more contiguous and cheaper. It is gated on bf16, 193..208 tokens, a private qkv buffer and no export or calibration. This adds planner complexity and a second attention kernel instantiation, and it also lets variant 3 force the persistent path with fewer items.

```diff
diff --git a/dfd-clip_amd/blocked.py b/dfd-clip_amd/blocked.py
--- a/dfd-clip_amd/blocked.py
+++ b/dfd-clip_amd/blocked.py
@@ -43,3 +43,31 @@
 def lane_channels(eq):
     perm = fc_channel_perm(TILE_CHANNELS)
     return [[int(perm[16 * j + 4 * eq + e]) for e in range(4)] for j in range(4)]
+
+
+
+def qkv_channel_perm(heads, device=None):
+    return fc_channel_perm(3 * heads * TILE_CHANNELS, device=device)
+
+
+def qkv_unit(third, head, heads):
+    assert 0 <= third < 3 and 0 <= head < heads
+    return third * heads + head
+
+
+def qkv_offset(row, third, head, d, heads, ld=None):
+    return piece_offset(row, qkv_unit(third, head, heads) * TILE_CHANNELS + d, 3 * heads * TILE_CHANNELS if ld is None else ld)
+
+
+def qkv_pack(qkv, fill=0):
+    return pack(qkv, fill)
+
+
+def qkv_unpack(b, m=None):
+    return unpack(b, m)
+
+
+def qkv_item_units(frame, tokens, third, head, heads, ld=None):
+    ld = 3 * heads * TILE_CHANNELS if ld is None else ld
+    g0, g1 = (frame * tokens) // GROUP_ROWS, (frame * tokens + tokens - 1) // GROUP_ROWS
+    return [g * GROUP_ROWS * ld + qkv_unit(third, head, heads) * 1024 for g in range(g0, g1 + 1)]
diff --git a/dfd-clip_amd/capi.py b/dfd-clip_amd/capi.py
--- a/dfd-clip_amd/capi.py
+++ b/dfd-clip_amd/capi.py
@@ -25,6 +25,7 @@
 GEMM_SPARE_IF_FREE = 2
 GEMM_C_BLOCKED = 4
 GEMM_A_BLOCKED = 8
+GEMM_QKV_BLOCKED = 16
 
 
 class GemmExtra(Structure):
@@ -254,6 +255,11 @@
     "dfd_gemm_pair_set_variant": (c_int, [c_int]),
     "dfd_gemm_pair_plan": (c_int, [c_int64, c_int, c_int]),
     "dfd_gemm_pair_launches": (c_int64, []),
+    "dfd_gemm_qkv_set_variant": (c_int, [c_int]),
+    "dfd_gemm_qkv_plan": (c_int, [c_int64, c_int]),
+    "dfd_gemm_qkv_launches": (c_int64, []),
+    "dfd_attention_fwd_blocked": (c_int, [c_void_p, c_int64, c_void_p, c_int64, c_int, c_int, c_int, c_int, c_int, c_float, c_void_p]),
+    "dfd_attention_plan_blocked": (c_int, [c_int, c_int, c_int, c_int, c_int64, c_int64, c_int, POINTER(AttentionPlan)]),
     "dfd_gemm_at_b_last_path": (c_int, []),
     "dfd_stream_policy_set": (c_uint, [c_uint]),
     "dfd_stream_policy_get": (c_uint, []),
@@ -611,7 +617,7 @@
 
 def gemm(a, w, c, bias=None, epilogue=EPI_BIAS, m=None, pos=None, cls=None, k_export=None, v_export=None, tokens=0,
          frames_per_clip=0, residual=None, qkv_first=0, drop=None, stream_out=False, spare_cus=0, tile_blocks=0, spare_if_free=False,
-         c_blocked=False, a_blocked=False):
+         c_blocked=False, a_blocked=False, qkv_blocked=False):
     _dev(a, w, c, bias, pos, cls, k_export, v_export, residual)
     assert a.dtype == w.dtype and a.stride(1) == 1 and w.stride(1) == 1 and c.stride(1) == 1
     M = a.shape[0] if m is None else m
@@ -620,13 +626,13 @@
     assert residual is None or (residual.dtype == c.dtype and residual.stride(0) == c.stride(0))
     assert drop is None or epilogue == EPI_RESIDUAL_POS
     assert 0 <= epilogue <= EPI_BIAS_GELU, f"unknown epilogue {epilogue}"
-    if c_blocked or a_blocked:
-        blk = c if c_blocked else a
+    if c_blocked or a_blocked or qkv_blocked:
+        blk = a if a_blocked else c
         assert blk.shape[0] >= (M + 15) // 16 * 16, "a blocked matrix needs its rows rounded up to 16"
     extra = GemmExtra(_ptr(pos).value, _ptr(cls).value, _ptr(k_export).value, _ptr(v_export).value, tokens, frames_per_clip,
                       _ptr(residual).value, qkv_first, drop.rng.data_ptr() if drop is not None and drop.p > 0 else None,
                       drop.site if drop is not None else 0, drop.p if drop is not None else 0.0, (GEMM_STREAM_OUT if stream_out else 0) | (GEMM_SPARE_IF_FREE if spare_if_free else 0) | ((int(spare_cus) & 0xff) << 8) | ((int(tile_blocks) & 0xf) << 16)
-                      | (GEMM_C_BLOCKED if c_blocked else 0) | (GEMM_A_BLOCKED if a_blocked else 0))
+                      | (GEMM_C_BLOCKED if c_blocked else 0) | (GEMM_A_BLOCKED if a_blocked else 0) | (GEMM_QKV_BLOCKED if qkv_blocked else 0))
     timed = _profile["epilogue"] == epilogue
     if timed:
         e0, e1 = torch.cuda.Event(enable_timing=True), torch.cuda.Event(enable_timing=True)
@@ -679,6 +685,18 @@
     return load_library().dfd_gemm_pair_launches()
 
 
+def gemm_qkv_set_variant(variant):
+    return load_library().dfd_gemm_qkv_set_variant(int(variant))
+
+
+def gemm_qkv_plan(M, D):
+    return bool(load_library().dfd_gemm_qkv_plan(int(M), int(D)))
+
+
+def gemm_qkv_launches():
+    return load_library().dfd_gemm_qkv_launches()
+
+
 def stream_policy_set(mask):
     return load_library().dfd_stream_policy_set(int(mask))
 
@@ -757,20 +775,23 @@
     return load_library().dfd_attention_last_path()
 
 
-def attention_plan(dtype, n_frames, tokens, heads, ld_qkv=None, ld_out=None, n_cu=256):
+def attention_plan(dtype, n_frames, tokens, heads, ld_qkv=None, ld_out=None, n_cu=256, blocked=False):
     D = heads * 64
     plan = AttentionPlan()
-    rc = load_library().dfd_attention_plan(_DTYPE[dtype], n_frames, tokens, heads, 3 * D if ld_qkv is None else ld_qkv,
+    fn = load_library().dfd_attention_plan_blocked if blocked else load_library().dfd_attention_plan
+    rc = fn(_DTYPE[dtype], n_frames, tokens, heads, 3 * D if ld_qkv is None else ld_qkv,
                                            D if ld_out is None else ld_out, n_cu, ctypes.byref(plan))
     if rc < 0:
         raise DfdError(f"dfd_attention_plan failed ({rc}): {load_library().dfd_last_error().decode()}")
     return plan
 
 
-def attention_fwd(qkv, out, n_frames, tokens, heads, head_dim=64):
+def attention_fwd(qkv, out, n_frames, tokens, heads, head_dim=64, blocked=False):
     _dev(qkv, out)
     assert qkv.dtype == out.dtype and qkv.stride(1) == 1 and out.stride(1) == 1
-    _check(load_library().dfd_attention_fwd(_ptr(qkv), qkv.stride(0), _ptr(out), out.stride(0), _DTYPE[qkv.dtype], n_frames,
+    assert not blocked or qkv.shape[0] >= (n_frames * tokens + 15) // 16 * 16, "a blocked matrix needs its rows rounded up to 16"
+    fn = load_library().dfd_attention_fwd_blocked if blocked else load_library().dfd_attention_fwd
+    _check(fn(_ptr(qkv), qkv.stride(0), _ptr(out), out.stride(0), _DTYPE[qkv.dtype], n_frames,
                                             tokens, heads, head_dim, head_dim ** -0.5, _stream()), "dfd_attention_fwd")
     return out
 
diff --git a/dfd-clip_amd/csrc/attention.hip b/dfd-clip_amd/csrc/attention.hip
--- a/dfd-clip_amd/csrc/attention.hip
+++ b/dfd-clip_amd/csrc/attention.hip
@@ -153,13 +153,14 @@
 thread_local int g_attn_variant = 0;
 thread_local int g_attn_last_path = 0;
 
-int checked_plan(AttnPlan* p, int dtype, int n_frames, int tokens, int heads, int64_t ld_qkv, int64_t ld_out, int n_cu) {
+int checked_plan(AttnPlan* p, int dtype, int n_frames, int tokens, int heads, int64_t ld_qkv, int64_t ld_out, int n_cu, int blocked = 0) {
   DFD_REQUIRE(n_frames >= 0 && tokens > 0 && heads > 0, "dfd_attention_fwd: bad shape");
   DFD_REQUIRE(dtype == DFD_F32 || dtype == DFD_BF16, "dfd_attention_fwd: dtype=%d", dtype);
   const int esz = dtype == DFD_F32 ? 4 : 2;
   DFD_REQUIRE(ld_qkv >= 3 * heads * HD && ld_out >= heads * HD && (ld_qkv * esz) % 16 == 0 && (ld_out * esz) % 16 == 0,
               "dfd_attention_fwd: bad leading dimensions");
-  *p = attn_plan(dtype, n_frames, tokens, heads, ld_qkv, ld_out, g_attn_variant, n_cu > 0 ? n_cu : dfd_cu_count());
+  *p = attn_plan(dtype, n_frames, tokens, heads, ld_qkv, ld_out, g_attn_variant, n_cu > 0 ? n_cu : dfd_cu_count(), blocked);
+  DFD_REQUIRE(!p->refused, "dfd_attention_fwd_blocked: no kernel reads this fragment-blocked q|k|v: %s", p->refused);
   DFD_REQUIRE(p->path != ATTN_NONE, "dfd_attention_fwd: %lld (frame, head) items do not fit a grid", (long long)n_frames * heads);
   return DFD_OK;
 }
@@ -182,12 +183,20 @@
   return p.path;
 }
 
-extern "C" int dfd_attention_fwd(const void* qkv, int64_t ld_qkv, void* out, int64_t ld_out, int dtype, int n_frames,
-                                 int tokens, int heads, int head_dim, float scale, void* stream) {
+extern "C" int dfd_attention_plan_blocked(int dtype, int n_frames, int tokens, int heads, int64_t ld_qkv, int64_t ld_out, int n_cu,
+                                          dfd_attention_plan_t* out) {
+  AttnPlan p;
+  if (checked_plan(&p, dtype, n_frames, tokens, heads, ld_qkv, ld_out, n_cu, 1) != DFD_OK) return -1;
+  if (out) *out = dfd_attention_plan_t{p.path, p.grid, p.block, p.chunk, (uint64_t)p.lds};
+  return p.path;
+}
+
+static int attention_fwd(const void* qkv, int64_t ld_qkv, void* out, int64_t ld_out, int dtype, int n_frames, int tokens, int heads,
+                         int head_dim, float scale, void* stream, int blocked) {
   DFD_REQUIRE(qkv && out, "dfd_attention_fwd: null pointer");
   DFD_REQUIRE(head_dim == HD, "dfd_attention_fwd: head_dim=%d, only 64 is supported", head_dim);
   AttnPlan p;
-  if (int rc = checked_plan(&p, dtype, n_frames, tokens, heads, ld_qkv, ld_out, 0)) return rc;
+  if (int rc = checked_plan(&p, dtype, n_frames, tokens, heads, ld_qkv, ld_out, 0, blocked)) return rc;
   DFD_REQUIRE(dfd_aligned16(qkv) && dfd_aligned16(out), "dfd_attention_fwd: pointers must be 16-byte aligned");
   if (n_frames == 0) return DFD_OK;
   const AttnCall c{qkv, ld_qkv, out, ld_out, n_frames, tokens, heads, scale, static_cast<hipStream_t>(stream)};
@@ -202,3 +211,13 @@
   if (rc == DFD_OK) g_attn_last_path = p.path;
   return rc;
 }
+
+extern "C" int dfd_attention_fwd(const void* qkv, int64_t ld_qkv, void* out, int64_t ld_out, int dtype, int n_frames,
+                                 int tokens, int heads, int head_dim, float scale, void* stream) {
+  return attention_fwd(qkv, ld_qkv, out, ld_out, dtype, n_frames, tokens, heads, head_dim, scale, stream, 0);
+}
+
+extern "C" int dfd_attention_fwd_blocked(const void* qkv, int64_t ld_qkv, void* out, int64_t ld_out, int dtype, int n_frames,
+                                         int tokens, int heads, int head_dim, float scale, void* stream) {
+  return attention_fwd(qkv, ld_qkv, out, ld_out, dtype, n_frames, tokens, heads, head_dim, scale, stream, 1);
+}
diff --git a/dfd-clip_amd/csrc/attention_common.hpp b/dfd-clip_amd/csrc/attention_common.hpp
--- a/dfd-clip_amd/csrc/attention_common.hpp
+++ b/dfd-clip_amd/csrc/attention_common.hpp
@@ -1,5 +1,6 @@
 #pragma once
 #include "common.hpp"
+#include "gemm_blocked.hpp"
 #include "../../include/dfdclip_hooks.h"
 
 namespace {
@@ -34,6 +35,27 @@
   for (int p = p0; p < np; p += dp) {
     if (8 * p + sub < tokens)
       __builtin_amdgcn_raw_ptr_buffer_load_lds(srd, (lds_ptr_t)(vimg + p * 1024), 16, v_any + p * 8 * ldq, sbase, 0, 0);
+  }
+}
+
+__device__ __forceinline__ void attn_stage_k_blk(__amdgpu_buffer_rsrc_t srd, unsigned char* kimg, uint32_t frow, uint32_t sunit,
+                                                 uint32_t ldq, int lane, int np, int tokens) {
+  const int sub = lane >> 3, pos = lane & 7;
+  const uint32_t r0 = frow + (uint32_t)sub;
+  const uint32_t k_even = dfd_blk_chunk((uint32_t)(pos ^ ((sub >> 1) & 3))), k_odd = dfd_blk_chunk((uint32_t)(pos ^ (((sub >> 1) & 3) | 4)));
+  for (int p = 0; p < np; ++p) {
+    if (8 * p + sub < tokens)
+      __builtin_amdgcn_raw_ptr_buffer_load_lds(srd, (lds_ptr_t)(kimg + p * 1024), 16, dfd_blk_row(r0 + 8u * p, ldq) + ((p & 1) ? k_odd : k_even), sunit, 0, 0);
+  }
+}
+__device__ __forceinline__ void attn_stage_v_blk(__amdgpu_buffer_rsrc_t srd, unsigned char* vimg, uint32_t frow, uint32_t sunit,
+                                                 uint32_t ldq, int lane, int np, int tokens) {
+  const int sub = lane >> 3, pos = lane & 7;
+  const uint32_t r0 = frow + (uint32_t)sub;
+  const uint32_t v_any = dfd_blk_chunk((uint32_t)(pos ^ (((sub >> 1) & 1) << 2)));
+  for (int p = 0; p < np; ++p) {
+    if (8 * p + sub < tokens)
+      __builtin_amdgcn_raw_ptr_buffer_load_lds(srd, (lds_ptr_t)(vimg + p * 1024), 16, dfd_blk_row(r0 + 8u * p, ldq) + v_any, sunit, 0, 0);
   }
 }
 
@@ -155,6 +177,8 @@
   size_t lds;
   int chunk;
   uint32_t qkv_bytes, out_bytes;
+  int blocked;
+  const char* refused;
 };
 
 constexpr size_t ATTN_LDS_MAX = 160 * 1024;
@@ -163,9 +187,23 @@
 constexpr size_t ATTN_XROW_LDS = 4 * 257 * 128 + 8 * 2048 + 2560;
 constexpr int ATTN_STREAM_SPAN = 128;
 
-inline AttnPlan attn_plan(int dtype, int n_frames, int tokens, int heads, int64_t ld_qkv, int64_t ld_out, int variant, int n_cu) {
+inline AttnPlan attn_plan(int dtype, int n_frames, int tokens, int heads, int64_t ld_qkv, int64_t ld_out, int variant, int n_cu, int blocked = 0) {
   const int64_t items = (int64_t)n_frames * heads, GRID_MAX = 0x7fffffff, EXTENT_MAX = 0xfffffff0;
   const size_t esz = dtype == DFD_F32 ? 4 : 2;
+  if (blocked) {
+    auto refuse = [](const char* why) { return AttnPlan{ATTN_NONE, 0u, 0u, 0, 0, 0u, 0u, 1, why}; };
+    if (dtype != DFD_BF16) return refuse("the fragment-blocked layout is bf16");
+    if (ld_qkv % 64 != 0) return refuse("the leading dimension of a fragment-blocked matrix must be a multiple of 64");
+    if (tokens < 193 || tokens > 208) return refuse("only the persistent kernel for 193..208 tokens reads a fragment-blocked q|k|v");
+    const int64_t rows = ((int64_t)n_frames * tokens + 15) & ~(int64_t)15;
+    const int64_t qkv_bytes = rows * ld_qkv * 2, out_bytes = ((int64_t)n_frames * tokens - 1) * ld_out * 2 + (int64_t)heads * 128;
+    const unsigned grid = (unsigned)(n_cu <= 0 ? 256 : n_cu) & ~7u;
+    const size_t lds = attn_persist_lds(tokens, 7);
+    if (grid < 8 || lds > ATTN_LDS_MAX) return refuse("the persistent kernel needs 8 compute units and its images in LDS");
+    if (qkv_bytes > EXTENT_MAX || out_bytes > EXTENT_MAX || (int64_t)n_frames * tokens > GRID_MAX)
+      return refuse("q|k|v or out exceeds the 32-bit byte offsets of a buffer descriptor");
+    return AttnPlan{tokens <= 6 * 32 + 8 ? ATTN_PERSIST7_SHORT : ATTN_PERSIST7, grid, 512u, lds, 0, (uint32_t)qkv_bytes, (uint32_t)out_bytes, 1, nullptr};
+  }
   auto per_item = [&](int path, size_t lds, int chunk) {
     return AttnPlan{items <= GRID_MAX ? path : ATTN_NONE, (unsigned)items, 256u, lds, chunk, 0u, 0u};
   };
@@ -175,7 +213,7 @@
     const int64_t qkv_bytes = last_row * ld_qkv * 2 + (int64_t)3 * heads * 128, out_bytes = last_row * ld_out * 2 + (int64_t)heads * 128;
     const unsigned grid = (unsigned)(n_cu <= 0 ? 256 : n_cu) & ~7u;
     const size_t lds = nb == 7 ? attn_persist_lds(tokens, 7) : ATTN_XROW_LDS;
-    if (items >= 512 && grid >= 8 && qkv_bytes <= EXTENT_MAX && out_bytes <= EXTENT_MAX && (nb == 7 ? lds <= ATTN_LDS_MAX : tokens == 257))
+    if ((items >= 512 || variant == 3) && grid >= 8 && qkv_bytes <= EXTENT_MAX && out_bytes <= EXTENT_MAX && (nb == 7 ? lds <= ATTN_LDS_MAX : tokens == 257))
       return AttnPlan{nb == 9 ? ATTN_XROW : tokens <= 6 * 32 + 8 ? ATTN_PERSIST7_SHORT : ATTN_PERSIST7, grid, 512u, lds, 0,
                       (uint32_t)qkv_bytes, (uint32_t)out_bytes};
     return per_item(nb == 7 ? ATTN_ITEM7 : ATTN_ITEM9, attn_item_lds(nb), 0);
diff --git a/dfd-clip_amd/csrc/attention_mfma.hip b/dfd-clip_amd/csrc/attention_mfma.hip
--- a/dfd-clip_amd/csrc/attention_mfma.hip
+++ b/dfd-clip_amd/csrc/attention_mfma.hip
@@ -181,6 +181,18 @@
   for (int p = 0; p < 4 * NB; ++p) {
     const uint32_t row = (uint32_t)min(8 * p + sub, tokens - 1);
     __builtin_amdgcn_raw_ptr_buffer_load_lds(srd, (lds_ptr_t)(qimg + p * 1024), 16, row * ldq + ((p & 1) ? q_odd : q_even), sbase, 0, 0);
+  }
+}
+
+template <int NB>
+__device__ __forceinline__ void attn_stage_q_blk(__amdgpu_buffer_rsrc_t srd, unsigned char* qimg, uint32_t frow, uint32_t sunit, uint32_t ldq,
+                                                 int lane, int tokens) {
+  const int sub = lane >> 3, pos = lane & 7;
+  const uint32_t q_even = dfd_blk_chunk((uint32_t)(pos ^ ((sub >> 1) & 3))), q_odd = dfd_blk_chunk((uint32_t)(pos ^ (((sub >> 1) & 3) | 4)));
+#pragma unroll
+  for (int p = 0; p < 4 * NB; ++p) {
+    const uint32_t row = frow + (uint32_t)min(8 * p + sub, tokens - 1);
+    __builtin_amdgcn_raw_ptr_buffer_load_lds(srd, (lds_ptr_t)(qimg + p * 1024), 16, dfd_blk_row(row, ldq) + ((p & 1) ? q_odd : q_even), sunit, 0, 0);
   }
 }
 
@@ -247,7 +259,7 @@
   }
 }
 
-template <int NB, bool SHORT>
+template <int NB, bool SHORT, bool BLK = false>
 __global__ __launch_bounds__(512) void attn_mfma_persist_kernel(const bf16_t* __restrict__ qkv, uint32_t ldq ,
                                                                 bf16_t* __restrict__ out, uint32_t ldo ,
                                                                 int tokens, int heads, int n_frames, uint32_t qkv_bytes,
@@ -283,18 +295,31 @@
   if (wave == NB) {
     int f1, h1, f2, h2;
     auto sbase_of = [&](int f, int hh) { return (uint32_t)f * tokens * ldq + hh * (HD * 2); };
+    [[maybe_unused]] auto blk_k = [&](unsigned char* dst, int f, int hh) {
+      attn_stage_k_blk(srdQ, dst, (uint32_t)f * tokens, (uint32_t)(heads + hh) * DFD_BLK_UNIT, ldq, lane, np, tokens);
+    };
+    [[maybe_unused]] auto blk_v = [&](unsigned char* dst, int f, int hh) {
+      attn_stage_v_blk(srdQ, dst, (uint32_t)f * tokens, (uint32_t)(2 * heads + hh) * DFD_BLK_UNIT, ldq, lane, np, tokens);
+    };
+    [[maybe_unused]] auto blk_q = [&](unsigned char* dst, int f, int hh) {
+      attn_stage_q_blk<NB>(srdQ, dst, (uint32_t)f * tokens, (uint32_t)hh * DFD_BLK_UNIT, ldq, lane, tokens);
+    };
     int issued = 0, mark_kq = 0, mark_v = 0;
     bool have = item_of(0, f1, h1);
     if (have) {
-      attn_stage_k(srdQ, smem, sbase_of(f1, h1), ldq, Db, lane, np, tokens);
-      attn_stage_q<NB>(srdQ, smem + 4 * img, sbase_of(f1, h1), ldq, lane, tokens);
+      if constexpr (BLK) blk_k(smem, f1, h1);
+      else attn_stage_k(srdQ, smem, sbase_of(f1, h1), ldq, Db, lane, np, tokens);
+      if constexpr (BLK) blk_q(smem + 4 * img, f1, h1);
+      else attn_stage_q<NB>(srdQ, smem + 4 * img, sbase_of(f1, h1), ldq, lane, tokens);
       issued += np + 4 * NB;
       mark_kq = issued;
       if (item_of(1, f2, h2)) {
-        attn_stage_k(srdQ, smem + 2 * img, sbase_of(f2, h2), ldq, Db, lane, np, tokens);
+        if constexpr (BLK) blk_k(smem + 2 * img, f2, h2);
+        else attn_stage_k(srdQ, smem + 2 * img, sbase_of(f2, h2), ldq, Db, lane, np, tokens);
         issued += np;
       }
-      attn_stage_v(srdQ, smem + img, sbase_of(f1, h1), ldq, Db, lane, np, tokens);
+      if constexpr (BLK) blk_v(smem + img, f1, h1);
+      else attn_stage_v(srdQ, smem + img, sbase_of(f1, h1), ldq, Db, lane, np, tokens);
       issued += np;
       mark_v = issued;
     }
@@ -304,18 +329,21 @@
       barrier();
       const bool have1 = item_of(n + 1, f1, h1);
       if (have1) {
-        attn_stage_q<NB>(srdQ, smem + 4 * img + (cur ^ 1) * NB * QIMG, sbase_of(f1, h1), ldq, lane, tokens);
+        if constexpr (BLK) blk_q(smem + 4 * img + (cur ^ 1) * NB * QIMG, f1, h1);
+        else attn_stage_q<NB>(srdQ, smem + 4 * img + (cur ^ 1) * NB * QIMG, sbase_of(f1, h1), ldq, lane, tokens);
         issued += 4 * NB;
         mark_kq = issued;
       }
       wait_vm_dyn(issued - mark_v);
       barrier();
       if (have1 && item_of(n + 2, f2, h2)) {
-        attn_stage_k(srdQ, smem + cur * 2 * img, sbase_of(f2, h2), ldq, Db, lane, np, tokens);
+        if constexpr (BLK) blk_k(smem + cur * 2 * img, f2, h2);
+        else attn_stage_k(srdQ, smem + cur * 2 * img, sbase_of(f2, h2), ldq, Db, lane, np, tokens);
         issued += np;
       }
       if (have1) {
-        attn_stage_v(srdQ, smem + (cur ^ 1) * 2 * img + img, sbase_of(f1, h1), ldq, Db, lane, np, tokens);
+        if constexpr (BLK) blk_v(smem + (cur ^ 1) * 2 * img + img, f1, h1);
+        else attn_stage_v(srdQ, smem + (cur ^ 1) * 2 * img + img, sbase_of(f1, h1), ldq, Db, lane, np, tokens);
         issued += np;
         mark_v = issued;
       }
@@ -406,9 +434,9 @@
                                             static_cast<bf16_t*>(c.out), c.ld_out, c.tokens, c.heads, c.scale * 1.4426950408889634f);
 }
 
-template <bool SHORT>
+template <bool SHORT, bool BLK>
 int launch_persist(const AttnPlan& p, const AttnCall& c) {
-  return attn_launch<&attn_mfma_persist_kernel<7, SHORT>>("dfd_attention_fwd(mfma, persistent)", p, c.st, static_cast<const bf16_t*>(c.qkv),
+  return attn_launch<&attn_mfma_persist_kernel<7, SHORT, BLK>>("dfd_attention_fwd(mfma, persistent)", p, c.st, static_cast<const bf16_t*>(c.qkv),
                                                           (uint32_t)(c.ld_qkv * 2), static_cast<bf16_t*>(c.out), (uint32_t)(c.ld_out * 2),
                                                           c.tokens, c.heads, c.n_frames, p.qkv_bytes, p.out_bytes,
                                                           c.scale * 1.4426950408889634f);
@@ -418,8 +446,8 @@
 
 int dfd_attn_launch_mfma(const AttnPlan& p, const AttnCall& c) {
   switch (p.path) {
-    case ATTN_PERSIST7_SHORT: return launch_persist<true>(p, c);
-    case ATTN_PERSIST7: return launch_persist<false>(p, c);
+    case ATTN_PERSIST7_SHORT: return p.blocked ? launch_persist<true, true>(p, c) : launch_persist<true, false>(p, c);
+    case ATTN_PERSIST7: return p.blocked ? launch_persist<false, true>(p, c) : launch_persist<false, false>(p, c);
     case ATTN_ITEM7: return launch_item<7>(p, c);
     default: return launch_item<9>(p, c);
   }
diff --git a/dfd-clip_amd/csrc/gemm.hip b/dfd-clip_amd/csrc/gemm.hip
--- a/dfd-clip_amd/csrc/gemm.hip
+++ b/dfd-clip_amd/csrc/gemm.hip
@@ -264,7 +264,8 @@
   a.tile_rows = 32 * (int)((extra->flags >> DFD_GEMM_TILE_BLOCKS_SHIFT) & 0xf);
   a.c_blocked = (extra->flags & DFD_GEMM_C_BLOCKED) ? 1 : 0;
   a.a_blocked = (extra->flags & DFD_GEMM_A_BLOCKED) ? 1 : 0;
-  a.pair = a.c_blocked | a.a_blocked;
+  a.qkv_blocked = (extra->flags & DFD_GEMM_QKV_BLOCKED) ? 1 : 0;
+  a.pair = a.c_blocked | a.a_blocked | a.qkv_blocked;
   DFD_REQUIRE(epilogue != DFD_EPI_QKV_EXPORT || !extra->k_export == !extra->v_export, "dfd_gemm: QKV_EXPORT needs both k_export and v_export or neither");
   if (epilogue == DFD_EPI_RESIDUAL_POS && extra->drop_rng && extra->drop_p > 0.f) {
     DFD_REQUIRE(extra->drop_p < 1.f, "dfd_gemm: drop_p=%f", (double)extra->drop_p);
@@ -276,6 +277,7 @@
 
 static thread_local int g_gemm_variant = 0;
 static thread_local int g_pair_variant = 0;
+static thread_local int g_qkv_variant = 0;
 
 static int checked_plan(GemmPlan* p, const char* who, GemmArgs& a, GemmPtrs ptrs, int ab_dtype, int c_dtype, int epilogue, int n_cu) {
   const bool f8 = ab_dtype == DFD_FP8;
@@ -320,10 +322,12 @@
     *p = GemmPlan{};
     return DFD_OK;
   }
-  *p = gemm_plan(a, ptrs, ab_dtype, c_dtype, epilogue, g_gemm_variant, g_pair_variant, n_cu > 0 ? n_cu : dfd_cu_count());
+  DFD_REQUIRE(!a.qkv_blocked || ab_dtype != DFD_F32, "%s: DFD_GEMM_QKV_BLOCKED: the fragment-blocked layout is bf16", who);
+  *p = gemm_plan(a, ptrs, ab_dtype, c_dtype, epilogue, g_gemm_variant, g_pair_variant, n_cu > 0 ? n_cu : dfd_cu_count(), g_qkv_variant);
   if (p->refused) {
     dfd_set_error("%s: %s%s (epilogue %d, M=%lld N=%d K=%d)", who,
-                  a.pair ? "DFD_GEMM_C_BLOCKED / DFD_GEMM_A_BLOCKED: the ping-pong kernel does not serve this call: " : "call not served: ", p->refused,
+                  a.qkv_blocked ? "DFD_GEMM_QKV_BLOCKED: the ping-pong kernel does not serve this call: "
+                  : a.pair      ? "DFD_GEMM_C_BLOCKED / DFD_GEMM_A_BLOCKED: the ping-pong kernel does not serve this call: " : "call not served: ", p->refused,
                   epilogue, (long long)a.M, a.N, a.K);
     return DFD_ERR_INVALID_ARG;
   }
@@ -365,12 +369,31 @@
   return blocked(fc, DFD_EPI_BIAS_QUICKGELU) && blocked(pr, DFD_EPI_BIAS) ? 1 : 0;
 }
 
+static thread_local int64_t g_qkv_launches = 0;
+extern "C" int dfd_gemm_qkv_set_variant(int variant) {
+  const int old = g_qkv_variant;
+  g_qkv_variant = variant;
+  return old;
+}
+extern "C" int64_t dfd_gemm_qkv_launches(void) { return g_qkv_launches; }
+extern "C" int dfd_gemm_qkv_plan(int64_t M, int D) {
+  if ((g_qkv_variant != 2 && g_qkv_variant != 3) || M < 1 || D < 1) return 0;
+  if (M < 1024 && g_qkv_variant != 2) return 0;
+  GemmArgs a{};
+  a.M = M; a.pair = a.qkv_blocked = 1;
+  a.N = 3 * D; a.K = D; a.lda = D; a.ldw = D; a.ldc = 3 * D;
+  const GemmPtrs dense{DFD_GEMM_PTR_A | DFD_GEMM_PTR_W | DFD_GEMM_PTR_C | DFD_GEMM_PTR_BIAS, 0u};
+  const GemmPlan p = gemm_plan(a, dense, DFD_BF16, DFD_BF16, DFD_EPI_BIAS, g_gemm_variant, g_pair_variant, 256, g_qkv_variant);
+  return p.kernel == DFD_GEMM_PINGPONG && p.qkv_blocked ? 1 : 0;
+}
+
 static int plan_and_launch(const char* who, GemmArgs& a, int ab_dtype, int c_dtype, int epilogue, void* stream) {
   GemmPlan p;
   if (const int rc = checked_plan(&p, who, a, gemm_ptrs(a), ab_dtype, c_dtype, epilogue, 0)) return rc;
   if (p.kernel == 0) return DFD_OK;
   a.c_blocked = p.c_blocked;
   a.a_blocked = p.a_blocked;
+  a.qkv_blocked = p.qkv_blocked;
   hipStream_t st = static_cast<hipStream_t>(stream);
   const bool f8 = ab_dtype == DFD_FP8, cf8 = c_dtype == DFD_FP8;
   int rc, path;
@@ -386,7 +409,8 @@
   if (rc != DFD_OK) return rc;
   g_last_kernel = p.kernel;
   if (!f8) g_last_path = path;
-  if (p.c_blocked || p.a_blocked) ++g_pair_launches;
+  if (p.qkv_blocked) ++g_qkv_launches;
+  else if (p.c_blocked || p.a_blocked) ++g_pair_launches;
   return DFD_OK;
 }
 
diff --git a/dfd-clip_amd/csrc/gemm256e.hip b/dfd-clip_amd/csrc/gemm256e.hip
--- a/dfd-clip_amd/csrc/gemm256e.hip
+++ b/dfd-clip_amd/csrc/gemm256e.hip
@@ -9,7 +9,7 @@
 constexpr int DEPTH = 6;
 constexpr int NB = 2 * (DEPTH - 1);
 
-template <int EPI, int RB, bool F8, bool CF8, bool ABLK = false>
+template <int EPI, int RB, bool F8, bool CF8, bool ABLK = false, bool QBLK = false>
 __global__ __launch_bounds__(512) void gemm256e_kernel(const GemmArgs a, int tiles_m, int tiles_n) {
   static_assert(!F8 || RB == 8, "fp8 form: 256-row tiles only");
   static_assert(!CF8 || (F8 && EPI != DFD_EPI_QKV_EXPORT), "fp8 output: fp8 operands, plain, QuickGELU or GELU epilogue");
@@ -21,7 +21,8 @@
   constexpr int S1 = CF8 ? RB : 2 * RB;
   constexpr int S2 = 4 * RB;
   static_assert(!ABLK || (!F8 && EPI == DFD_EPI_BIAS), "blocked A: bf16 operands, plain epilogue");
-  constexpr bool C_BLK = !F8 && (EPI == DFD_EPI_BIAS_QUICKGELU || EPI == DFD_EPI_BIAS_GELU);
+  static_assert(!QBLK || (!F8 && !ABLK && EPI == DFD_EPI_BIAS), "blocked C of the plain epilogue: bf16 operands, row-major A");
+  constexpr bool C_BLK = !F8 && (QBLK || EPI == DFD_EPI_BIAS_QUICKGELU || EPI == DFD_EPI_BIAS_GELU);
   constexpr bool A_BLK = ABLK;
   __shared__ __attribute__((aligned(1024))) unsigned char smem[RING + 8 * STAGE];
   const int tid = threadIdx.x;
@@ -320,7 +321,7 @@
       if constexpr (F8) cs4[j] = *reinterpret_cast<const f32x4*>(ep + 256 + (j * 16 + (le >> 4) * 4) * 4);
     }
     asm volatile("s_waitcnt lgkmcnt(0)" ::: "memory");
-    const int stores = tile_epilogue<EPI, RB, F8, CF8, C_BLK>(a, acc, b4, cs4, ep, cur, wr, wc, le, D, srdC);
+    const int stores = tile_epilogue<EPI, RB, F8, CF8, QBLK ? 2 : C_BLK ? 1 : 0>(a, acc, b4, cs4, ep, cur, wr, wc, le, D, srdC);
     if (!has_next) break;
     s_prev = countable_stores<RB>(stores, cur, wr, a.M);
     idx = nidx;
@@ -384,6 +385,7 @@
   static int run(const GemmPlan& p, hipStream_t st, const GemmArgs& a) {
     if constexpr (!F8 && EPI == DFD_EPI_BIAS) {
       if (a.a_blocked) return gemm_launch<&gemm256e_kernel<EPI, RB, F8, CF8, true>>("ping-pong", p, st, a, p.tiles.tiles_m, a.N / TN);
+      if (p.qkv_blocked) return gemm_launch<&gemm256e_kernel<EPI, RB, F8, CF8, false, true>>("ping-pong", p, st, a, p.tiles.tiles_m, a.N / TN);
     }
     return gemm_launch<&gemm256e_kernel<EPI, RB, F8, CF8, false>>("ping-pong", p, st, a, p.tiles.tiles_m, a.N / TN);
   }
diff --git a/dfd-clip_amd/csrc/gemm256p_common.hpp b/dfd-clip_amd/csrc/gemm256p_common.hpp
--- a/dfd-clip_amd/csrc/gemm256p_common.hpp
+++ b/dfd-clip_amd/csrc/gemm256p_common.hpp
@@ -76,7 +76,7 @@
   return (int64_t)t.m0 + (wr + 1) * 16 * RB <= M ? stores : 0;
 }
 
-template <int EPI, int RB, bool F8, bool CF8, bool BLK = false>
+template <int EPI, int RB, bool F8, bool CF8, int BLK = 0>
 __device__ __forceinline__ int tile_epilogue(const GemmArgs& a, f32x4 (&acc)[RB][4], const f32x4 (&b4)[4], const f32x4 (&cs4)[4], unsigned char* const ep,
                                              const Tile& cur, int wr, int wc, int le, int D, __amdgpu_buffer_rsrc_t srdC) {
   constexpr int WROWS = 16 * RB;
@@ -256,7 +256,7 @@
         store_out(d, srdC, off, a.stream_out);
       }
     }
-  } else if (BLK && a.c_blocked) {
+  } else if (BLK == 2 || (BLK == 1 && a.c_blocked)) {
     const int row0 = wr * WROWS + er;
     const int rows_left_b = (int)min((int64_t)0x7fffffff, a.M - ((int64_t)cur.m0 + row0));
     const uint32_t ldc2 = (uint32_t)(a.ldc * 2);
diff --git a/dfd-clip_amd/csrc/gemm_args.hpp b/dfd-clip_amd/csrc/gemm_args.hpp
--- a/dfd-clip_amd/csrc/gemm_args.hpp
+++ b/dfd-clip_amd/csrc/gemm_args.hpp
@@ -24,6 +24,6 @@
   float out_inv_scale;
   uint32_t* sched;
   uint32_t sched_base[8];
-  int no_dynamic;
+  int qkv_blocked;
   int c_blocked, a_blocked, pair;
 };
diff --git a/dfd-clip_amd/csrc/gemm_plan.hpp b/dfd-clip_amd/csrc/gemm_plan.hpp
--- a/dfd-clip_amd/csrc/gemm_plan.hpp
+++ b/dfd-clip_amd/csrc/gemm_plan.hpp
@@ -26,6 +26,7 @@
   int kernel;
   int epilogue;
   int c_blocked, a_blocked;
+  int qkv_blocked;
   int dynamic;
   TilePlan tiles;
   unsigned grid_y, block;
@@ -59,7 +60,7 @@
   return p;
 }
 
-inline const char* gemm_persistent_refuses(int kernel, const GemmArgs& a, GemmPtrs p, bool f8, int c_dtype, int epi, int cb, int ab) {
+inline const char* gemm_persistent_refuses(int kernel, const GemmArgs& a, GemmPtrs p, bool f8, int c_dtype, int epi, int cb, int ab, int qb = 0) {
   const bool pingpong = kernel == DFD_GEMM_PINGPONG, cf8 = c_dtype == DFD_FP8;
   const int esz = f8 ? 1 : 2, csz = cf8 ? 1 : 2, kshift = f8 ? 7 : 6;
   if (c_dtype != DFD_BF16 && !(f8 && cf8)) return "C must be bf16 (e4m3 operands: or e4m3)";
@@ -73,8 +74,8 @@
   if (Mr * a.lda * esz > GEMM_EXTENT_MAX || (int64_t)a.N * a.ldw * esz > GEMM_EXTENT_MAX || Mr * a.ldc * csz > GEMM_EXTENT_MAX)
     return "A, W or C exceeds the 32-bit byte offsets of a buffer descriptor";
   if ((int64_t)((a.M + 223) / 224) * (a.N / GEMM_TILE_N) > 0x3fffffff || a.M >= ((int64_t)1 << 31)) return "too many tiles or rows";
-  if ((cb || ab) && (esz != 2 || csz != 2)) return "the fragment-blocked layout is bf16";
-  if ((cb && a.ldc % 64 != 0) || (ab && a.lda % 64 != 0)) return "the leading dimension of a fragment-blocked matrix must be a multiple of 64";
+  if ((cb || ab || qb) && (esz != 2 || csz != 2)) return "the fragment-blocked layout is bf16";
+  if (((cb || qb) && a.ldc % 64 != 0) || (ab && a.lda % 64 != 0)) return "the leading dimension of a fragment-blocked matrix must be a multiple of 64";
   const int nk = a.K >> kshift;
   if (pingpong) {
     if ((nk < 6 && !(epi == DFD_EPI_RESIDUAL_POS && nk == 4)) || (nk & 1)) return "the ping-pong K loop needs an even number of 128-byte steps, at least 6";
@@ -83,9 +84,11 @@
     return "K is less than two 128-byte steps";
   }
   if (!gemm_serves(kernel, epi, f8)) return "the kernel has no form for this epilogue";
-  if ((cb || ab) && !pingpong) return "only the ping-pong kernel knows the fragment-blocked layout";
+  if ((cb || ab || qb) && !pingpong) return "only the ping-pong kernel knows the fragment-blocked layout";
+  if (qb && (cb || ab)) return "DFD_GEMM_QKV_BLOCKED does not combine with DFD_GEMM_C_BLOCKED / DFD_GEMM_A_BLOCKED";
   if (cb && epi != DFD_EPI_BIAS_QUICKGELU && epi != DFD_EPI_BIAS_GELU) return "DFD_GEMM_C_BLOCKED needs BIAS_QUICKGELU or BIAS_GELU";
   if (ab && epi != DFD_EPI_BIAS) return "DFD_GEMM_A_BLOCKED needs BIAS";
+  if (qb && epi != DFD_EPI_BIAS) return "DFD_GEMM_QKV_BLOCKED needs BIAS, or QKV_EXPORT without export buffers";
   if (epi == DFD_EPI_QKV_EXPORT) {
     const int D = a.N / (3 - a.qkv_first);
     if (cf8) return "an e4m3 C has no QKV_EXPORT form";
@@ -141,21 +144,23 @@
   }
 }
 
-inline GemmPlan gemm_plan(const GemmArgs& a, GemmPtrs ptrs, int ab_dtype, int c_dtype, int epilogue, int gemm_variant, int pair_variant, int n_cu) {
+inline GemmPlan gemm_plan(const GemmArgs& a, GemmPtrs ptrs, int ab_dtype, int c_dtype, int epilogue, int gemm_variant, int pair_variant, int n_cu,
+                          int qkv_variant = 0) {
   GemmPlan p{};
   p.epilogue = epilogue;
   const int cb = pair_variant == 1 ? 0 : a.c_blocked, ab = pair_variant == 1 ? 0 : a.a_blocked;
+  const int qb = qkv_variant == 1 ? 0 : a.qkv_blocked;
   const bool f8 = ab_dtype == DFD_FP8;
   if (ab_dtype != DFD_F32) {
     const int epi_p = epilogue == DFD_EPI_QKV_EXPORT && !(ptrs.present & DFD_GEMM_PTR_EXPORT) ? DFD_EPI_BIAS : epilogue;
     int kernel = DFD_GEMM_PINGPONG;
     const char* why = a.pair && f8                ? "the fragment-blocked layout is bf16"
                       : gemm_variant == 1 ? "dfd_gemm_set_variant(1) skips the ping-pong kernel"
-                                          : gemm_persistent_refuses(kernel, a, ptrs, f8, c_dtype, epi_p, cb, ab);
-    if (why && !a.pair) why = gemm_persistent_refuses(kernel = DFD_GEMM_PERSISTENT, a, ptrs, f8, c_dtype, epi_p, cb, ab);
+                                          : gemm_persistent_refuses(kernel, a, ptrs, f8, c_dtype, epi_p, cb, ab, qb);
+    if (why && !a.pair) why = gemm_persistent_refuses(kernel = DFD_GEMM_PERSISTENT, a, ptrs, f8, c_dtype, epi_p, cb, ab, qb);
     if (!why) {
       p.kernel = kernel; p.epilogue = epi_p; p.grid_y = 1; p.block = 512;
-      p.c_blocked = cb; p.a_blocked = ab;
+      p.c_blocked = cb | qb; p.a_blocked = ab; p.qkv_blocked = qb;
       p.tiles = plan_tiles(a.M, a.N, a.spare_cus, kernel == DFD_GEMM_PINGPONG && a.spare_if_free, a.tile_rows, f8, epi_p == DFD_EPI_RESIDUAL_POS, n_cu);
       p.dynamic = kernel == DFD_GEMM_PINGPONG && !f8 && a.K / 64 >= 6 && gemm_variant == 3;
       return p;
diff --git a/dfd-clip_amd/encoder.py b/dfd-clip_amd/encoder.py
--- a/dfd-clip_amd/encoder.py
+++ b/dfd-clip_amd/encoder.py
@@ -141,6 +141,7 @@
         self.register_load_state_dict_post_hook(_invalidate_after_load)
         self._prepared = None
         self._ws = {}
+        self._qkv_reader = {}
         self.frame_chunk = 0
         self.streams = 1
         self._side_streams = []
@@ -281,11 +282,29 @@
             if H % 64 == 0 and bp["w_proj"].shape[1] == H:
                 idx = blocked.fc_channel_perm(H, device=bp["w_fc"].device)
                 bp["w_fc_blk"], bp["b_fc_blk"] = bp["w_fc"][idx].contiguous(), bp["b_fc"][idx].contiguous()
+            if self.width % 64 == 0:
+                idx = blocked.fc_channel_perm(3 * self.width, device=bp["w_qkv"].device)
+                bp["w_qkv_blk"], bp["b_qkv_blk"] = bp["w_qkv"][idx].contiguous(), bp["b_qkv"][idx].contiguous()
 
     def _pair_blocked(self, bp, M, pl=_NONE):
         if "w_fc_blk" not in bp or not self.deferred_residual or pl["fc"] == "fp8" or pl["proj"] == "fp8":
             return False
         return capi.gemm_pair_plan(M, self.width, bp["w_fc"].shape[0])
+
+    def _qkv_blocked(self, bp, M, n, pl=_NONE):
+        if "w_qkv_blk" not in bp or pl["qkv"] != "bf16" or not capi.gemm_qkv_plan(M, self.width):
+            return False
+        reads = self._qkv_reader.get(n)
+        if reads is None:
+            try:
+                capi.attention_plan(self.act_dtype, n, self.tokens, self.heads, n_cu=0, blocked=True)
+                reads = True
+            except capi.DfdError:
+                reads = False
+            if len(self._qkv_reader) > 64:
+                self._qkv_reader.clear()
+            self._qkv_reader[n] = reads
+        return reads
 
     def _stage(self, dev):
         act = self.act_dtype
@@ -436,7 +455,7 @@
             ws["x"][:M] += ws["delta2"][:M]
         ws["pending"] = 0
 
-    def _block(self, ws, bp, qkv, M, n, kv_only=False, export=None):
+    def _block(self, ws, bp, qkv, M, n, kv_only=False, export=None, private_qkv=False):
         calib = getattr(self, "_calib", None)
         f8 = self._fp8_layers()[bp["idx"]] if self.precision == "fp8" and calib is None and M >= capi.FP8_MIN_ROWS else None
         pl = self._fp8_plan[bp["idx"]] if f8 is not None else _NONE
@@ -447,6 +466,7 @@
         sp_qkv, sp_out, sp_fc, sp_proj = (max(sp_all, sp if sg[k] else 0) for k in ("qkv", "out", "fc", "proj"))
         free = sp_all == 0 and self.spare_if_free
         D = self.width
+        qblk = False
         first = 1 if kv_only else 0
         rows = slice(D, None) if first else slice(None)
         kw = dict(m=M, tokens=self.tokens, qkv_first=first, stream_out=so["qkv"], spare_cus=sp_qkv, spare_if_free=free)
@@ -464,10 +484,12 @@
             self._ln(ws, bp["ln1"], M, discard_x=kv_only and calib is None)
             if calib is not None:
                 calib.append(ws["h"][:M].abs().max())
-            capi.gemm(ws["h"], bp["w_qkv"][rows], qkv[:, rows], bp["b_qkv"][rows], capi.EPI_QKV_EXPORT, **kw)
+            qblk = private_qkv and not kv_only and export is None and calib is None and self._qkv_blocked(bp, M, n, pl)
+            w_qkv, b_qkv = (bp["w_qkv_blk"], bp["b_qkv_blk"]) if qblk else (bp["w_qkv"], bp["b_qkv"])
+            capi.gemm(ws["h"], w_qkv[rows], qkv[:, rows], b_qkv[rows], capi.EPI_QKV_EXPORT, qkv_blocked=qblk, **kw)
         if kv_only:
             return
-        capi.attention_fwd(qkv, ws["mix"], n, self.tokens, self.heads)
+        capi.attention_fwd(qkv, ws["mix"], n, self.tokens, self.heads, blocked=qblk)
         self._residual(ws, ws["mix"], bp["w_out"], bp["b_out"], M, spare_cus=sp_out, spare_if_free=free)
         if "w_12" in bp:
             H = self.ffn_hidden
@@ -579,7 +601,7 @@
                             torch.cuda.current_stream().wait_event(pos_ready)
                             waited = True
                         exp = (k_out[i, f0 * P:(f0 + nf) * P], v_out[i, f0 * P:(f0 + nf) * P], temporal_pos, num_frames)
-                    self._block(ws, p["blocks"][l], qkv_l, M, nf, kv_only=(l == last), export=exp)
+                    self._block(ws, p["blocks"][l], qkv_l, M, nf, kv_only=(l == last), export=exp, private_qkv=l not in slot)
         if n_str > 1:
             for st in self._side_streams[:n_str]:
                 cur.wait_stream(st)
diff --git a/include/dfdclip.h b/include/dfdclip.h
--- a/include/dfdclip.h
+++ b/include/dfdclip.h
@@ -55,6 +55,7 @@
   DFD_GEMM_SPARE_IF_FREE = 2,
   DFD_GEMM_C_BLOCKED = 4,
   DFD_GEMM_A_BLOCKED = 8,
+  DFD_GEMM_QKV_BLOCKED = 16,
   DFD_GEMM_TILE_BLOCKS_SHIFT = 16,
   DFD_GEMM_SPARE_CUS_SHIFT = 8
 };
diff --git a/include/dfdclip_hooks.h b/include/dfdclip_hooks.h
--- a/include/dfdclip_hooks.h
+++ b/include/dfdclip_hooks.h
@@ -28,6 +28,11 @@
 int dfd_attention_plan(int dtype, int n_frames, int tokens, int heads, int64_t ld_qkv, int64_t ld_out, int n_cu,
                        dfd_attention_plan_t* out);
 
+int dfd_attention_fwd_blocked(const void* qkv, int64_t ld_qkv, void* out, int64_t ld_out, int dtype, int n_frames, int tokens,
+                              int heads, int head_dim, float scale, void* stream);
+int dfd_attention_plan_blocked(int dtype, int n_frames, int tokens, int heads, int64_t ld_qkv, int64_t ld_out, int n_cu,
+                               dfd_attention_plan_t* out);
+
 int dfd_attention_set_variant(int variant);
 
 enum { DFD_GEMM_GENERAL = 1,
@@ -54,6 +59,10 @@
 int dfd_gemm_pair_set_variant(int variant);
 int dfd_gemm_pair_plan(int64_t M, int D, int H);
 int64_t dfd_gemm_pair_launches(void);
+
+int dfd_gemm_qkv_set_variant(int variant);
+int dfd_gemm_qkv_plan(int64_t M, int D);
+int64_t dfd_gemm_qkv_launches(void);
 
 int dfd_gemm_at_b_last_path(void);
 
```

Result: no change. 908.1 (median of 4 runs) (+0.2%).
